# EmilioOlivastri/IPC

Measured on AMD Instinct MI355X. Metric: candidate-pairs/s (consistency matrix + set-max), higher is better.
Workload: dtype f64; 1 GPU; C2: INTEL-like SE2 synthetic (V=1228, 256 true loops) + 1000 injected outliers; N=1256 candidates, 789396 cells (i<=j), 531545 solved on rank 0, s=10, fast 6.251/50, slow 11.345/100; parallelism=1 GPU

## Files before the change

### include/ipc_amd.h

```cpp
#ifndef IPC_AMD_H
#define IPC_AMD_H

#include <stddef.h>
#include <stdint.h>

#ifdef __cplusplus
extern "C" {
#endif

typedef struct ipc_engine ipc_engine_t;

typedef enum {
    IPC_OK = 0,
    IPC_ERR_ARG = -1,
    IPC_ERR_HIP = -2,
    IPC_ERR_STATE = -3,
    IPC_ERR_LIMIT = -4
} ipc_status;

typedef struct {
    double fast_reject_th;
    int    fast_reject_iter_base;
    double slow_reject_th;
    int    slow_reject_iter_base;
    double s_factor;
} ipc_params_t;

typedef struct {
    int    i, j;
    int    lo, hi;
    double max_chi2;
    double chi2_total;
    int    iterations;
    int    tries;
    int    flags;
    int    evals;
} ipc_cell_info_t;

const char* ipc_last_error(void);

int ipc_create(int dim, int n_vertices, const double* odom_meas, const double* odom_info,
               const ipc_params_t* params, int device, ipc_engine_t** out);

int ipc_destroy(ipc_engine_t* h);

int ipc_set_candidates(ipc_engine_t* h, int n, const int* ids, const double* meas,
                       const double* info);

int ipc_append_candidate(ipc_engine_t* h, const int* ids, const double* meas, const double* info, int* index_out);

int ipc_append_odometry(ipc_engine_t* h, int n_edges, const double* meas, const double* info);
int ipc_reserve_vertices(ipc_engine_t* h, int capacity);
int ipc_vertex_count(ipc_engine_t* h, int* n_vertices);

int ipc_candidate_order(ipc_engine_t* h, int* order_out);

int ipc_initial_poses(ipc_engine_t* h, double* poses_out);


int ipc_rows_per_rank(int n, int world);

int ipc_row_assignment(int n, const int* ids, int world, int policy, int* slot_out);

int ipc_solve_rows(ipc_engine_t* h, int rank, int world, uint64_t* d_upper, void* stream);

typedef struct {
    int cells;
    int long_cells;
    int failed_cells;
    int capped_cells;
    int nan_cells;
    int damped_cells;
    int literal_cells;
} ipc_solve_report_t;
int ipc_solve_report(ipc_engine_t* h, ipc_solve_report_t* out);

int ipc_assemble_matrix(ipc_engine_t* h, const uint64_t* d_gathered, int world,
                        uint64_t* d_bits, void* stream);

int ipc_set_max(ipc_engine_t* h, const uint64_t* d_bits, uint8_t* d_accepted, void* stream);

int ipc_run(ipc_engine_t* h, uint64_t* bits_out, uint8_t* accepted_out);

int ipc_run_set_only(ipc_engine_t* h, uint8_t* accepted_out, int* solved_cells_out);

int ipc_run_sharded(ipc_engine_t** engines, int n_engines, uint64_t* bits_out, uint8_t* accepted_out);

typedef struct {
    int covered_before, covered_after;
    int cells;
    int long_cells, literal_cells, damped_cells;
    int set_max_resumed;
    int grew;
} ipc_online_report_t;
int ipc_run_online(ipc_engine_t* h, uint64_t* bits_out, uint8_t* accepted_out, ipc_online_report_t* report);
int ipc_online_covered(ipc_engine_t* h, int* m);
int ipc_online_reset(ipc_engine_t* h);
int ipc_reserve_candidates(ipc_engine_t* h, int capacity);

int ipc_cell_count(ipc_engine_t* h, int* n_cells);
int ipc_cell_info(ipc_engine_t* h, ipc_cell_info_t* out, int capacity);

int ipc_solver_time_ms(ipc_engine_t* h, double* ms, int* launches);

int ipc_synchronize(ipc_engine_t* h);


typedef struct {
    int    lo, hi;
    int    n_cluster_loops;
    int    iterations, tries, flags;
    double max_chi2;
    double chi2_total;
    double chi2_initial;
} ipc_check_info_t;

int ipc_incremental_reset(ipc_engine_t* h);

int ipc_incremental_prepare(ipc_engine_t* h);

int ipc_agreement_check(ipc_engine_t* h, int k, int* agrees, ipc_check_info_t* info);

typedef struct {
    long host_solver_fallbacks, lost_launches, relaunches, literal_band_solves;
} ipc_incremental_counters_t;
int ipc_incremental_counters(ipc_engine_t* h, ipc_incremental_counters_t* out);

int ipc_consensus_size(ipc_engine_t* h, int* n);
int ipc_consensus_set(ipc_engine_t* h, int* out);

int ipc_remove_from_consensus(ipc_engine_t* h, int k, int* removed);
int ipc_add_to_consensus(ipc_engine_t* h, int k);

int ipc_current_poses(ipc_engine_t* h, double* poses_out);

int ipc_incremental_set_state(ipc_engine_t* h, const double* poses, const int* cns, int n_cns, int resume_position);

int ipc_final_optimize(ipc_engine_t* h, const uint8_t* accepted, int iterations, double* poses_out,
                       ipc_check_info_t* info);

int ipc_debug_dense_solve(int n, const double* system, int mode, int workgroups, double* x_out, int* info_out);

int ipc_debug_band_solve(int nb, int m, int W, const double* system, int workgroups, double* x_out, int* info_out);
int ipc_debug_absorbed_edges(int klo, int khi, int n, const int* lo, const int* hi, int sweep, int* members_out, int* n_members_out,
                             int* lo_out, int* hi_out);
int ipc_debug_band_plan(int d, int nl, const int* a, const int* b, int min_n, int* use_out, int* nlb_out, int* bwb_out,
                        int* order_out);

#ifdef __cplusplus
}
#endif
#endif
```

### ipc_amd/capi.py

```python
import ctypes as C
import os

import numpy as np



def export_recommended_environment():
    os.environ.setdefault("GPU_MAX_HW_QUEUES", "24")


_HERE = os.path.dirname(os.path.abspath(__file__))
LIB_PATH = os.environ.get("IPC_AMD_LIB") or os.path.join(_HERE, "libipc_amd.so")

SYMBOLS = [
    "ipc_last_error", "ipc_create", "ipc_destroy", "ipc_set_candidates", "ipc_candidate_order",
    "ipc_initial_poses", "ipc_rows_per_rank", "ipc_solve_rows", "ipc_assemble_matrix", "ipc_set_max",
    "ipc_run", "ipc_cell_count", "ipc_cell_info", "ipc_solve_report", "ipc_solver_time_ms", "ipc_synchronize",
    "ipc_incremental_reset", "ipc_incremental_prepare", "ipc_agreement_check", "ipc_consensus_size", "ipc_consensus_set",
    "ipc_remove_from_consensus", "ipc_add_to_consensus", "ipc_current_poses", "ipc_final_optimize",
    "ipc_debug_dense_solve", "ipc_debug_band_solve", "ipc_debug_band_plan", "ipc_debug_absorbed_edges", "ipc_append_candidate", "ipc_incremental_set_state", "ipc_incremental_counters", "ipc_row_assignment", "ipc_run_sharded", "ipc_run_set_only",
    "ipc_append_odometry", "ipc_reserve_vertices", "ipc_vertex_count",
    "ipc_run_online", "ipc_online_covered", "ipc_online_reset", "ipc_reserve_candidates",
]


class Params(C.Structure):
    _fields_ = [("fast_reject_th", C.c_double), ("fast_reject_iter_base", C.c_int),
                ("slow_reject_th", C.c_double), ("slow_reject_iter_base", C.c_int),
                ("s_factor", C.c_double)]


class CellInfo(C.Structure):
    _fields_ = [("i", C.c_int), ("j", C.c_int), ("lo", C.c_int), ("hi", C.c_int),
                ("max_chi2", C.c_double), ("chi2_total", C.c_double),
                ("iterations", C.c_int), ("tries", C.c_int), ("flags", C.c_int), ("evals", C.c_int)]


class CheckInfo(C.Structure):
    _fields_ = [("lo", C.c_int), ("hi", C.c_int), ("n_cluster_loops", C.c_int), ("iterations", C.c_int),
                ("tries", C.c_int), ("flags", C.c_int), ("max_chi2", C.c_double), ("chi2_total", C.c_double),
                ("chi2_initial", C.c_double)]


class IncrementalCounters(C.Structure):
    _fields_ = [("host_solver_fallbacks", C.c_long), ("lost_launches", C.c_long), ("relaunches", C.c_long),
                ("literal_band_solves", C.c_long)]


class SolveReport(C.Structure):
    _fields_ = [("cells", C.c_int), ("long_cells", C.c_int), ("failed_cells", C.c_int), ("capped_cells", C.c_int),
                ("nan_cells", C.c_int), ("damped_cells", C.c_int), ("literal_cells", C.c_int)]


class OnlineReport(C.Structure):
    _fields_ = [("covered_before", C.c_int), ("covered_after", C.c_int), ("cells", C.c_int), ("long_cells", C.c_int),
                ("literal_cells", C.c_int), ("damped_cells", C.c_int), ("set_max_resumed", C.c_int), ("grew", C.c_int)]


CELL_DTYPE = np.dtype([("i", "<i4"), ("j", "<i4"), ("lo", "<i4"), ("hi", "<i4"), ("max_chi2", "<f8"),
                       ("chi2_total", "<f8"), ("iterations", "<i4"), ("tries", "<i4"), ("flags", "<i4"),
                       ("evals", "<i4")])

_lib = None


class IpcError(RuntimeError):
    pass


def load():
    global _lib
    if _lib is not None:
        return _lib
    if not os.path.exists(LIB_PATH):
        raise IpcError("libipc_amd.so is not built (%s); run `python -c 'import __graft_entry__ as g; "
                       "g.build()'` -- there is no CPU fallback" % LIB_PATH)
    try:
        import torch
    except ImportError:
        pass
    lib = C.CDLL(LIB_PATH)
    lib.ipc_last_error.restype = C.c_char_p
    vp, ip, dp = C.c_void_p, C.c_int, C.c_double
    lib.ipc_create.argtypes = [ip, ip, vp, vp, C.POINTER(Params), ip, C.POINTER(vp)]
    lib.ipc_destroy.argtypes = [vp]
    lib.ipc_set_candidates.argtypes = [vp, ip, vp, vp, vp]
    lib.ipc_append_candidate.argtypes = [vp, vp, vp, vp, C.POINTER(ip)]
    lib.ipc_append_odometry.argtypes = [vp, ip, vp, vp]
    lib.ipc_reserve_vertices.argtypes = [vp, ip]
    lib.ipc_vertex_count.argtypes = [vp, C.POINTER(ip)]
    lib.ipc_candidate_order.argtypes = [vp, vp]
    lib.ipc_initial_poses.argtypes = [vp, vp]
    lib.ipc_rows_per_rank.argtypes = [ip, ip]
    lib.ipc_row_assignment.argtypes = [ip, vp, ip, ip, vp]
    lib.ipc_solve_rows.argtypes = [vp, ip, ip, vp, vp]
    lib.ipc_assemble_matrix.argtypes = [vp, vp, ip, vp, vp]
    lib.ipc_set_max.argtypes = [vp, vp, vp, vp]
    lib.ipc_run.argtypes = [vp, vp, vp]
    lib.ipc_run_online.argtypes = [vp, vp, vp, C.POINTER(OnlineReport)]
    lib.ipc_online_covered.argtypes = [vp, C.POINTER(ip)]
    lib.ipc_online_reset.argtypes = [vp]
    lib.ipc_reserve_candidates.argtypes = [vp, ip]
    lib.ipc_run_sharded.argtypes = [C.POINTER(vp), ip, vp, vp]
    lib.ipc_run_set_only.argtypes = [vp, vp, C.POINTER(ip)]
    lib.ipc_cell_count.argtypes = [vp, C.POINTER(ip)]
    lib.ipc_cell_info.argtypes = [vp, vp, ip]
    lib.ipc_solve_report.argtypes = [vp, C.POINTER(SolveReport)]
    lib.ipc_solver_time_ms.argtypes = [vp, C.POINTER(dp), C.POINTER(ip)]
    lib.ipc_synchronize.argtypes = [vp]
    lib.ipc_incremental_reset.argtypes = [vp]
    lib.ipc_incremental_prepare.argtypes = [vp]
    lib.ipc_agreement_check.argtypes = [vp, ip, C.POINTER(ip), C.POINTER(CheckInfo)]
    lib.ipc_consensus_size.argtypes = [vp, C.POINTER(ip)]
    lib.ipc_consensus_set.argtypes = [vp, vp]
    lib.ipc_remove_from_consensus.argtypes = [vp, ip, C.POINTER(ip)]
    lib.ipc_add_to_consensus.argtypes = [vp, ip]
    lib.ipc_current_poses.argtypes = [vp, vp]
    lib.ipc_incremental_set_state.argtypes = [vp, vp, vp, ip, ip]
    lib.ipc_incremental_counters.argtypes = [vp, C.POINTER(IncrementalCounters)]
    lib.ipc_final_optimize.argtypes = [vp, vp, ip, vp, C.POINTER(CheckInfo)]
    lib.ipc_debug_dense_solve.argtypes = [ip, vp, ip, ip, vp, C.POINTER(ip)]
    lib.ipc_debug_band_solve.argtypes = [ip, ip, ip, vp, ip, vp, C.POINTER(ip)]
    lib.ipc_debug_absorbed_edges.argtypes = [ip, ip, ip, vp, vp, ip, vp, C.POINTER(ip), C.POINTER(ip), C.POINTER(ip)]
    lib.ipc_debug_band_plan.argtypes = [ip, ip, vp, vp, ip, C.POINTER(ip), C.POINTER(ip), C.POINTER(ip), vp]
    assert C.sizeof(CellInfo) == CELL_DTYPE.itemsize
    _lib = lib
    return lib


def check(rc):
    if rc != 0:
        raise IpcError("ipc_amd error %d: %s" % (rc, load().ipc_last_error().decode()))
```

### ipc_amd/csrc/cell_kernels.hpp

```cpp
#pragma once
#include <hip/hip_runtime.h>

#include "se2_cell.hpp"
#include "se3_cell.hpp"

namespace ipc {

struct CellOut {
    double* max_chi2;
    double* chi2_total;
    int4* meta;
};

struct Variant { int W, M; };
static const Variant kVariants[] = {
    {1, 1}, {2, 1}, {3, 1}, {4, 1}, {5, 1}, {6, 1}, {7, 1}, {8, 1}, {10, 1}, {12, 1}, {14, 1}, {16, 1},
    {4, 2}, {5, 2}, {6, 2}, {7, 2}, {8, 2}, {10, 2}, {12, 2}, {16, 2},
    {5, 3}, {6, 3}, {7, 3}, {8, 3},
    {4, 4}, {6, 4}, {8, 4}, {16, 4}, {16, 8}, {16, 16},
    {2, 3}, {2, 4}, {2, 5}, {2, 6},
    {3, 4}, {3, 5}, {3, 6}, {4, 3}, {4, 5},
};
constexpr int kNumVariants = sizeof(kVariants) / sizeof(kVariants[0]);
static const Variant kVariants3[] = { {1, 1}, {2, 1}, {4, 1}, {8, 1}, {16, 1}, {16, 2}, {16, 4},
                                      {4, 2}, {4, 4}, {8, 2}, {8, 4}, {4, 8}, {8, 5},
                                      {1, 2}, {2, 2}, {1, 4}, {2, 4}, {1, 3}, {2, 3} };
constexpr int kNumVariants3 = sizeof(kVariants3) / sizeof(kVariants3[0]);

hipError_t launch_se2_block(int nl, int variant, int n, hipStream_t st, const Se2View& P, const int2* cells,
                            SolveParams prm, CellOut out);
hipError_t launch_se3_block(int nl, int variant, int n, hipStream_t st, const Se3View& P, const int2* cells,
                            SolveParams prm, CellOut out);

struct LdsVariant { int W, M; };
static const LdsVariant kLdsVariants3[] = { {1, 1}, {1, 2}, {1, 3}, {1, 4}, {1, 6}, {1, 8},
                                            {4, 2}, {4, 3}, {4, 4}, {4, 5}, {4, 6}, {4, 7}, {4, 8}, {4, 9}, {4, 10} };
constexpr int kNumLdsVariants3 = sizeof(kLdsVariants3) / sizeof(kLdsVariants3[0]);
constexpr int kLdsVariantBase3 = 400;
#define IPC_SE3_LDS_DECL(WW, MM)                                                                                \
    hipError_t launch_se3_lds_##WW##_##MM(int nl, int n, hipStream_t st, const Se3View& P, const int2* cells,   \
                                          SolveParams prm, CellOut out, unsigned* counter, int n_cu);
IPC_SE3_LDS_DECL(1, 1) IPC_SE3_LDS_DECL(1, 2) IPC_SE3_LDS_DECL(1, 3) IPC_SE3_LDS_DECL(1, 4) IPC_SE3_LDS_DECL(1, 6)
IPC_SE3_LDS_DECL(1, 8) IPC_SE3_LDS_DECL(4, 2) IPC_SE3_LDS_DECL(4, 3) IPC_SE3_LDS_DECL(4, 4) IPC_SE3_LDS_DECL(4, 5)
IPC_SE3_LDS_DECL(4, 6) IPC_SE3_LDS_DECL(4, 7) IPC_SE3_LDS_DECL(4, 8) IPC_SE3_LDS_DECL(4, 9) IPC_SE3_LDS_DECL(4, 10)
#undef IPC_SE3_LDS_DECL

static const int kWaveM[] = {1, 3, 5, 7, 9, 11, 13};
constexpr int kNumWaveM = sizeof(kWaveM) / sizeof(kWaveM[0]);
constexpr int kWaveVariantBase = 100;

hipError_t launch_se2_wave(int nl, int M, int n, hipStream_t st, const Se2View& P, const int2* cells,
                           SolveParams prm, CellOut out, unsigned* counter, int n_cu);

static const int kPairM[] = {5, 7, 9, 11};
constexpr int kNumPairM = sizeof(kPairM) / sizeof(kPairM[0]);
constexpr int kPairVariantBase = 200;
hipError_t launch_se2_pair(int nl, int M, int n, hipStream_t st, const Se2View& P, const int2* cells,
                           SolveParams prm, CellOut out, unsigned* counter, int n_cu);

static const int kQuadM[] = {7, 9, 11, 13};
constexpr int kNumQuadM = sizeof(kQuadM) / sizeof(kQuadM[0]);
constexpr int kQuadVariantBase = 300;
hipError_t launch_se2_quad(int nl, int M, int n, hipStream_t st, const Se2View& P, const int2* cells,
                           SolveParams prm, CellOut out, unsigned* counter, int n_cu);

}
```

### ipc_amd/csrc/engine.hip

```cpp
#include <hip/hip_runtime.h>

#include <algorithm>
#include <cstdarg>
#include <cstdlib>
#include <utility>
#include <cstdio>
#include <cstring>
#include <numeric>
#include <map>
#include <mutex>
#include <string>
#include <chrono>
#include <thread>
#include <vector>

#include "../../include/ipc_amd.h"
#include "cell_kernels.hpp"
#include "cluster_se2.hpp"
#include "cluster_se3.hpp"
#include "cluster_persist.hpp"

using namespace ipc;

static thread_local std::string g_err;
// ... 334 lines not shown
        }
        if (vr) bits[(size_t)ir * words + w] = mine;
    }
}

__global__ __launch_bounds__(256) void k_assemble_delta(int N, int M, int stride, const int* lo, const int* hi,
                                                        const unsigned long long* upper, unsigned long long* bits)
{
    const int lane = threadIdx.x & 63, wave = threadIdx.x >> 6;
    const int w = blockIdx.x;
    auto U = [&](int a, int c) -> unsigned {
        const unsigned long long word = upper[(size_t)a * stride + (c >> 6)];
        return (unsigned)((word >> (c & 63)) & 1ull);
    };
    const int w0 = M >> 6, w1 = (N - 1) >> 6;
    const bool neww = w >= w0;
    const unsigned long long keep = (w == w0 && (M & 63)) ? (1ull << (M & 63)) - 1ull : 0ull;
    const int j = w * 64 + lane;
    const bool vj = j < N;
    const int loj = vj ? lo[j] : 0, hij = vj ? hi[j] : 0;
    const unsigned long long Dword = __ballot(vj && U(j, j));
    for (int rb = (neww ? 0 : w0) + blockIdx.y * 4 + wave; rb <= w1; rb += gridDim.y * 4) {
        const int ir = rb * 64 + lane;
        const bool vr = ir < N;
        const int lor = vr ? lo[ir] : 0, hir = vr ? hi[ir] : 0;
        const unsigned long long dmask = __ballot(vr && U(ir, ir));
        const int nrows = min(64, N - rb * 64);
        unsigned long long mine = 0ull;
        for (int r = 0; r < nrows; ++r) {
            const int i = rb * 64 + r;
            if (i < M && !neww) continue;
            const int loi = __builtin_amdgcn_readlane(lor, r), hii = __builtin_amdgcn_readlane(hir, r);
            unsigned long long word = ((dmask >> r) & 1ull) ? Dword : 0ull;
            const bool ov = vj && j != i && (min(hii, hij) - max(loi, loj) > 0);
            const unsigned long long ovmask = __ballot(ov);
            if (ovmask) {
                const bool bit = ov && U(min(i, j), max(i, j));
                word = (word & ~ovmask) | __ballot(bit);
            }
            if (lane == r) mine = word;
        }
        if (vr) {
            unsigned long long* dst = bits + (size_t)ir * stride + w;
            if (ir >= M) *dst = mine;
            else if (neww) *dst = keep ? ((*dst & keep) | (mine & ~keep)) : mine;
        }
    }
}

__global__ __launch_bounds__(1024) void k_set_max(int N, int words, int stride, const int* order,
                                                  const unsigned long long* bits, unsigned char* accepted, int* live,
                                                  int first = 0, unsigned long long* mask = nullptr, int* nlive_io = nullptr)
{
    constexpr int CPW = 4, RC = 16 * CPW;
    extern __shared__ unsigned long long acc[];
    __shared__ int okflag[RC];
    __shared__ unsigned long long conf[RC];
    __shared__ int kk[RC];
    __shared__ int wcount[16];
    __shared__ int nlive_s;
    const int tid = threadIdx.x, wave = tid >> 6, lane = tid & 63;
    for (int w = tid; w < words; w += blockDim.x) acc[w] = first ? mask[w] : 0ull;
    if (first) { for (int q = first + tid; q < N; q += blockDim.x) accepted[order[q]] = 0; }
    else { for (int k = tid; k < N; k += blockDim.x) accepted[k] = 0; }
    if (tid == 0) nlive_s = first ? *nlive_io : 0;
    __syncthreads();
    const int nlive0 = nlive_s;
    for (int base = first; base < N; base += 1024) {
        const int pos = base + tid;
        const int k = pos < N ? order[pos] : -1;
        const bool keep = k >= 0 && ((bits[(size_t)k * stride + (k >> 6)] >> (k & 63)) & 1ull);
        const unsigned long long m = __ballot(keep);
        if (lane == 0) wcount[wave] = __popcll(m);
        __syncthreads();
        int off = nlive_s;
        for (int v = 0; v < wave; ++v) off += wcount[v];
        if (keep) live[off + __popcll(m & ((1ull << lane) - 1ull))] = k;
        __syncthreads();
        if (tid == 0) { int t = 0; for (int v = 0; v < 16; ++v) t += wcount[v]; nlive_s += t; }
        __syncthreads();
    }
    __threadfence_block();
    const int nlive = nlive_s;
    for (int base = nlive0; base < nlive; base += RC) {
        int k[CPW];
        bool bad[CPW];
#pragma unroll
        for (int c = 0; c < CPW; ++c) {
            const int pos = base + c * 16 + wave;
            k[c] = pos < nlive ? live[pos] : -1;
            bad[c] = false;
        }
        for (int w = lane; w < words; w += 64) {
            const unsigned long long a = acc[w];
#pragma unroll
            for (int c = 0; c < CPW; ++c) {
                const unsigned long long r = k[c] >= 0 ? bits[(size_t)k[c] * stride + w] : ~0ull;
                bad[c] = bad[c] || (r & a) != a;
            }
        }
#pragma unroll
        for (int c = 0; c < CPW; ++c) {
            const bool ok = k[c] >= 0 && __ballot(bad[c]) == 0ull;
            if (lane == 0) { okflag[c * 16 + wave] = ok ? 1 : 0; kk[c * 16 + wave] = k[c]; }
        }
        __syncthreads();
#pragma unroll
        for (int c = 0; c < CPW; ++c) {
            if (k[c] < 0) continue;
            unsigned m = 0;
            if (lane < RC && kk[lane] >= 0) {
                const int o = kk[lane];
                m = (unsigned)((bits[(size_t)k[c] * stride + (o >> 6)] >> (o & 63)) & 1ull);
            }
            const unsigned long long bal = __ballot(m != 0);
            if (lane == 0) conf[c * 16 + wave] = bal;
        }
        __syncthreads();
        if (tid == 0) {
            unsigned long long taken = 0;
            for (int w = 0; w < RC; ++w) {
                if (kk[w] < 0 || !okflag[w]) continue;
                if ((conf[w] & taken) != taken) continue;
                taken |= 1ull << w;
                acc[kk[w] >> 6] |= 1ull << (kk[w] & 63);
                accepted[kk[w]] = 1;
            }
        }
        __syncthreads();
    }
    if (mask) {
        for (int w = tid; w < words; w += blockDim.x) mask[w] = acc[w];
        if (tid == 0) *nlive_io = nlive;
    }
}

struct BinPlan {
    BinCaps caps;
    int variant[kMaxBins];
    int latency_variant[kMaxBins];
    int latency_below[kMaxBins];
};
static const char* kDefaultPolicy = "w1,w3,w5,w7,w9,w11,w13,p7,p9,p11,q7,q9,q11,q13,16x4,16x8,16x16";
static const int kDefaultSideStreams2 = 7, kDefaultSideStreams3 = 7;
static const char* kDefaultPolicy3 = "w1,w2,w3,w4,w6,w8,g3,g4,g5,g6,g7,g8,g9,g10,16x4";
static const char* kBlockPolicy3 = "1x1,1x2,1x3,2x2,2x3,4x2,4x4,8x4,8x5,16x4";
static const char* kDefaultLatencyPolicy3 = "1x1,2x1,4x1,4x2,4x4,8x4,8x5,16x4";
static bool make_plan(BinPlan& bp, int dim, std::string& err)
{
    const char* env = getenv(dim == 2 ? "IPC_SE2_POLICY" : "IPC_SE3_POLICY");
    std::string pol = env && *env ? env : (dim == 2 ? kDefaultPolicy : kDefaultPolicy3);
    if (dim == 3 && pol == "block") pol = kBlockPolicy3;
    const Variant* table = dim == 2 ? kVariants : kVariants3;
    const int ntable = dim == 2 ? kNumVariants : kNumVariants3;
    std::vector<std::pair<int, int>> items;
    size_t pos = 0;
    while (pos < pol.size()) {
        size_t e = pol.find(',', pos);
        if (e == std::string::npos) e = pol.size();
        int w = 0, m = 0;
        const std::string tok = pol.substr(pos, e - pos);
        int v = -1;
        if (dim == 2 && sscanf(tok.c_str(), "w%d", &m) == 1) {
            w = 1;
            for (int k = 0; k < kNumWaveM; ++k) if (kWaveM[k] == m) v = kWaveVariantBase + m;
        } else if (dim == 2 && sscanf(tok.c_str(), "p%d", &m) == 1) {
            w = 2;
            for (int k = 0; k < kNumPairM; ++k) if (kPairM[k] == m) v = kPairVariantBase + m;
        } else if (dim == 2 && sscanf(tok.c_str(), "q%d", &m) == 1) {
            w = 4;
            for (int k = 0; k < kNumQuadM; ++k) if (kQuadM[k] == m) v = kQuadVariantBase + m;
        } else if (dim == 3 && (sscanf(tok.c_str(), "w%d", &m) == 1 || sscanf(tok.c_str(), "g%d", &m) == 1)) {
            w = tok[0] == 'w' ? 1 : 4;
            for (int k = 0; k < kNumLdsVariants3; ++k)
                if (kLdsVariants3[k].W == w && kLdsVariants3[k].M == m) v = kLdsVariantBase3 + k;
        } else {
            if (sscanf(tok.c_str(), "%dx%d", &w, &m) != 2) { err = "bad IPC_SE2_POLICY token"; return false; }
            for (int k = 0; k < ntable; ++k) if (table[k].W == w && table[k].M == m) v = k;
        }
        if (v < 0) { err = "IPC_SE*_POLICY names a variant that is not compiled: " + tok; return false; }
        items.push_back({64 * w * m, v});
        pos = e + 1;
    }
    std::sort(items.begin(), items.end());
    if (items.empty() || (int)items.size() > kMaxBins) { err = "IPC_SE2_POLICY: 1..32 variants"; return false; }
    bp.caps.n = (int)items.size();
    for (int b = 0; b < kMaxBins; ++b) {
        bp.caps.cap[b] = b < bp.caps.n ? items[b].first : 0;
        bp.variant[b] = b < bp.caps.n ? items[b].second : -1;
        bp.latency_variant[b] = -1;
        bp.latency_below[b] = 0;
    }
    if (dim == 3) {
        const char* lenv = getenv("IPC_SE3_LATENCY_POLICY");
        const std::string lpol = lenv && *lenv ? lenv : kDefaultLatencyPolicy3;
        if (lpol != "none") {
            size_t lp = 0;
            std::vector<std::pair<int, int>> lat;
            while (lp < lpol.size()) {
                size_t e = lpol.find(',', lp);
                if (e == std::string::npos) e = lpol.size();
                int w = 0, m = 0, v = -1;
                if (sscanf(lpol.substr(lp, e - lp).c_str(), "%dx%d", &w, &m) != 2) { err = "bad IPC_SE3_LATENCY_POLICY token"; return false; }
                for (int k = 0; k < ntable; ++k) if (table[k].W == w && table[k].M == m) v = k;
                if (v < 0) { err = "IPC_SE3_LATENCY_POLICY names a variant that is not compiled"; return false; }
                lat.push_back({64 * w * m, v});
                lp = e + 1;
            }
            std::sort(lat.begin(), lat.end());
            for (int b = 0; b < bp.caps.n; ++b) {
                if (bp.variant[b] >= kLdsVariantBase3) continue;
                const int wt = table[bp.variant[b]].W;
                for (const auto& lv : lat) {
                    if (lv.first < bp.caps.cap[b]) continue;
                    if (table[lv.second].W > wt) {
                        bp.latency_variant[b] = lv.second;
                        bp.latency_below[b] = wt <= 4 ? 4 / wt : 1;
                    }
                    break;
                }
            }
        }
    }
    return true;
}

static hipError_t launch_se3_lds(int nl, int idx, int n, hipStream_t st, const Se3View& P, const int2* cells,
                                 SolveParams prm, CellOut out, unsigned* counter, int n_cu)
{
#define IPC_LCASE(i, WW, MM) case i: return launch_se3_lds_##WW##_##MM(nl, n, st, P, cells, prm, out, counter, n_cu);
    switch (idx) {
        IPC_LCASE(0, 1, 1) IPC_LCASE(1, 1, 2) IPC_LCASE(2, 1, 3) IPC_LCASE(3, 1, 4) IPC_LCASE(4, 1, 6) IPC_LCASE(5, 1, 8)
        IPC_LCASE(6, 4, 2) IPC_LCASE(7, 4, 3) IPC_LCASE(8, 4, 4) IPC_LCASE(9, 4, 5) IPC_LCASE(10, 4, 6) IPC_LCASE(11, 4, 7)
        IPC_LCASE(12, 4, 8) IPC_LCASE(13, 4, 9) IPC_LCASE(14, 4, 10)
        default: return hipErrorInvalidValue;
    }
#undef IPC_LCASE
}

struct ipc_engine {
    int dim = 2, V = 0, N = 0, device = 0;
    int vcap = 0;
    double* h_stage = nullptr; double* d_stage = nullptr; size_t stage_cap = 0;
    hipEvent_t ev_stage = nullptr; bool stage_used = false;
    long chain_growths = 0;
    ipc_params_t prm{};
    double term_eps = 1e-13;
    BinPlan plan{};
    hipStream_t own_stream = nullptr;
    double* d_chain = nullptr; int estride = 0;
    double* d_chain_rec = nullptr;
    double2* d_chain_blk = nullptr;
    double* d_pose0 = nullptr;
    double* d_cand = nullptr; int cstride = 0;
    int *d_from = nullptr, *d_to = nullptr, *d_lo = nullptr, *d_hi = nullptr, *d_order = nullptr;
    int* d_live = nullptr;
    int* d_rowperm = nullptr;
    std::vector<int> row_group_off;
    bool order_stale = false;
    std::vector<void*> retired;
    hipEvent_t ev_cand = nullptr; bool cand_event = false;
    std::vector<int> order, h_lo, h_hi;
    std::vector<int> h_cand_ids; std::vector<double> h_cand_meas, h_cand_info;
    unsigned* d_counters = nullptr;
    unsigned* d_offsets = nullptr;
    unsigned* d_wave_ctr = nullptr;
    int n_cu = 256;
    int2* d_cells = nullptr; size_t cells_cap = 0;
    double *d_chi = nullptr, *d_chitot = nullptr; int4* d_meta = nullptr;
    bool plan_cached = false; int plan_rank = -1, plan_world = 0; size_t plan_total = 0;
    int slow_first_iterations = 96;
    std::vector<unsigned> plan_counts, plan_offsets;
    int2* d_lit_cells = nullptr; int* d_lit_idx = nullptr; double *d_lit_chi = nullptr, *d_lit_chitot = nullptr; int4* d_lit_meta = nullptr;
    unsigned* d_slot_off = nullptr;
    int* d_recount = nullptr; int* h_recount = nullptr;
    int last_cells = 0, last_long_cells = 0;
    hipEvent_t ev0 = nullptr, ev1 = nullptr; bool ev_valid = false; int last_launches = 0;
    static constexpr int kMaxSide = 7;
    int n_side = 0;
    bool side_forced = false;
    hipStream_t side[kMaxSide] = {};
    hipEvent_t ev_fork = nullptr, ev_join[kMaxSide] = {}, ev_join_own = nullptr;
    unsigned long long *d_upper = nullptr, *d_bits = nullptr; unsigned char* d_acc = nullptr; size_t run_cap = 0;
    int on_cov = 0, on_ccap = 0, on_wcap = 0, reserved_cands = 0;
    unsigned long long *d_on_upper = nullptr, *d_on_bits = nullptr;
    unsigned long long* d_on_mask = nullptr;
    unsigned char* d_on_acc = nullptr;
    int* d_on_live = nullptr;
    long online_growths = 0;
    std::vector<double> h_odom_meas, h_odom_info;
    std::vector<int> h_from, h_to, cns;
    double* d_chain1 = nullptr;
    double* d_open = nullptr;
    double* d_cur = nullptr;
    ClusterSolver2* cluster = nullptr;
    ClusterSolver3* cluster3 = nullptr;
    bool persist = true;
    bool last_persist = false;
    int* d_slot = nullptr; int slot_world = 0; int row_policy = 1;
    int* d_failed = nullptr; int failed_cap = 0; int last_lm_cells = 0;
    bool lm_retry = true;
    double borderline_band = -1.0;
    int last_literal_cells = 0;
    long lm_fallbacks = 0;
    long persist_timeouts = 0;
    long persist_relaunches = 0;
    bool cns_dups = false;
    PersistSolver<PersistSe2>* persist2 = nullptr;
    PersistSolver<PersistSe3>* persist3 = nullptr;
    unsigned long long* d_prof = nullptr;
    int max_helpers = -1;
    PersistKnobs knobs;
    int literal_band_min_n = 3072;
    struct SpecSlot {
        PersistSolver<PersistSe2>* s2 = nullptr;
        PersistSolver<PersistSe3>* s3 = nullptr;
        hipStream_t st = nullptr;
        hipEvent_t done = nullptr;
        int cand = -1, pos = -1;
        int state = -1;
        int launch_id = 0;
        int busy_wgs = 0;
        int expect = -1;
        std::chrono::steady_clock::time_point t_launch;
        int lo = 0, hi = 0, nclu = 0;
        double th = 0.0;
        double pred_ratio = -1.0;
    };
    struct SpecState {
        double* d_poses = nullptr;
        bool owned = false;
        hipEvent_t ready = nullptr;
        bool has_ready = false;
        std::vector<int> cns;
        int pos = -1;
        int users = 0;
        bool live = false;
        double* d_pred = nullptr; double* h_pred = nullptr; int pred_cap = 0, pred_n = 0;
        hipEvent_t pred_ev = nullptr; bool has_pred = false, pred_ready = false;
    };
    struct SpecResult {
        bool valid = false, agree = false, retry_host = false;
        int state = -1, child = -1;
        int lo = 0, hi = 0, nclu = 0;
        ClusterOut o;
    };
    std::vector<SpecSlot> slots;
    std::vector<SpecState> spec_states;
    std::vector<int> tent;
    std::vector<SpecResult> spec_res;
    int committed_state = -1;
    std::vector<int> porder, ppos;
    std::vector<char> handed;
    int spec_head = -1;
    int spec_window = 4, spec_ahead = 256;
    bool window_forced = false;
    int stream_concurrency = 0;
    int spec_active = 0;
    double accept_rate = 0.5;
    std::vector<char> pred_accept;
    double pred_k = 30.0;
    std::vector<double> pred_last;
    int spec_behind = 1;
    double uncertain_from = 0.0;
    int xcd_cus = 0;
    int spec_hedge = 0;
    int helper_limit_reject = 8;
    double gate_release_ms = 0.0;
    int helper_limit = 39;
    double st_acc_s = 0, st_rej_s = 0; long st_acc_it = 0, st_rej_it = 0, st_acc_n = 0, st_rej_n = 0;
    double st_acc_dev_s = 0, st_rej_dev_s = 0;
    unsigned long long commit_count = 0;
    hipEvent_t ev_commit = nullptr;
    int* h_abort = nullptr;
    int* d_abort = nullptr;
    int next_launch_id = 1;
    long spec_hits = 0, spec_launches = 0, spec_wasted = 0, spec_tentative = 0, spec_promoted = 0;
    double spec_t_launch = 0, spec_t_tent = 0, spec_t_total = 0;
    unsigned long long idle_why[5] = {0, 0, 0, 0, 0};
    hipStream_t pred_stream = nullptr;
    FILE* spec_log = nullptr;
    std::chrono::steady_clock::time_point spec_log_t0;
    long pred_conf[3][2] = {{0, 0}, {0, 0}, {0, 0}};
};

static int spec_quiesce(ipc_engine* h, bool state_changes);
static int spec_reset(ipc_engine* h);
struct DevicePipeline {
    ipc_engine* active = nullptr;
    std::vector<ipc_engine*> engines;
    std::recursive_mutex run_mu;
};
static std::mutex g_pipeline_mu;
static std::map<int, DevicePipeline*> g_device_pipeline;
static DevicePipeline& device_pipeline(int device)
{
    std::lock_guard<std::mutex> lk(g_pipeline_mu);
    DevicePipeline*& p = g_device_pipeline[device];
    if (!p) p = new DevicePipeline();
    return *p;
}
static std::map<int, std::vector<hipStream_t>> g_slot_streams;
static hipError_t pipeline_stream(int device, int q, hipStream_t* out)
{
    std::lock_guard<std::mutex> lk(g_pipeline_mu);
    std::vector<hipStream_t>& pool = g_slot_streams[device];
    while ((int)pool.size() <= q) {
        hipStream_t st = nullptr;
        const hipError_t e = hipStreamCreateWithFlags(&st, hipStreamNonBlocking);
        if (e != hipSuccess) return e;
        pool.push_back(st);
    }
    *out = pool[q];
    return hipSuccess;
}

static hipError_t copy_d2d_now(ipc_engine* h, void* dst, const void* src, size_t bytes)
{
    hipError_t e = hipMemcpyAsync(dst, src, bytes, hipMemcpyDeviceToDevice, h->own_stream);
    return e != hipSuccess ? e : hipStreamSynchronize(h->own_stream);
}
constexpr int kPoseTrail = 16;
static int reset_current(ipc_engine* h)
{
    const size_t n = (h->dim == 2 ? 5 : 12) * (size_t)h->vcap;
    HIPCHK(hipMemcpyAsync(h->d_cur, h->d_open, sizeof(double) * n, hipMemcpyDeviceToDevice, h->own_stream));
    HIPCHK(hipMemsetAsync(h->d_cur + n, 0, sizeof(double) * kPoseTrail, h->own_stream));
    HIPCHK(hipStreamSynchronize(h->own_stream));
    return IPC_OK;
}
extern "C" int ipc_rows_per_rank(int n, int world) { return world > 0 ? (n + world - 1) / world : 0; }

extern "C" int ipc_row_assignment(int n, const int* ids, int world, int policy, int* slot_out)
{
    if (n < 0 || world < 1 || (n > 0 && (!ids || !slot_out))) return fail(IPC_ERR_ARG, "ipc_row_assignment: bad argument");
    const int rpr = ipc_rows_per_rank(n, world);
    if (policy == 0 || world == 1) {
        for (int i = 0; i < n; ++i) slot_out[i] = (i % world) * rpr + i / world;
        return IPC_OK;
    }
    std::vector<int> lo(n), hi(n);
    for (int i = 0; i < n; ++i) { lo[i] = std::min(ids[2 * i], ids[2 * i + 1]); hi[i] = std::max(ids[2 * i], ids[2 * i + 1]); }
    std::vector<long long> cost(n);
    for (int i = 0; i < n; ++i) cost[i] = hi[i] - lo[i];
    {
        std::vector<int> ord(n);
        std::iota(ord.begin(), ord.end(), 0);
        std::sort(ord.begin(), ord.end(), [&](int a, int b) { return lo[a] != lo[b] ? lo[a] < lo[b] : a < b; });
        for (int p = 0; p < n; ++p) {
            const int a = ord[p], loa = lo[a], hia = hi[a];
            for (int q = p + 1; q < n && lo[ord[q]] < hia; ++q) {
                const int b = ord[q];
                if (std::min(hia, hi[b]) - lo[b] > 0) cost[std::min(a, b)] += std::max(hia, hi[b]) - loa;
            }
        }
    }
    std::vector<int> rows(n);
    std::iota(rows.begin(), rows.end(), 0);
    std::stable_sort(rows.begin(), rows.end(), [&](int a, int b) { return cost[a] > cost[b]; });
    std::vector<long long> load(world, 0);
    std::vector<int> used(world, 0);
    for (int i : rows) {
        int best = -1;
        for (int r = 0; r < world; ++r)
            if (used[r] < rpr && (best < 0 || load[r] < load[best])) best = r;
        slot_out[i] = best * rpr + used[best];
        ++used[best];
        load[best] += cost[i];
    }
    return IPC_OK;
}

extern "C" int ipc_create(int dim, int n_vertices, const double* odom_meas, const double* odom_info,
                          const ipc_params_t* params, int device, ipc_engine_t** out)
{
    if (!out) return fail(IPC_ERR_ARG, "ipc_create: out is NULL");
    *out = nullptr;
    if (dim != 2 && dim != 3) return fail(IPC_ERR_ARG, "ipc_create: dim must be 2 (SE2) or 3 (SE3), got %d", dim);
    if (n_vertices < 2 || !odom_meas || !odom_info || !params)
        return fail(IPC_ERR_ARG, "ipc_create: need >= 2 vertices and non-NULL arrays");
    if (!(params->s_factor > 0)) return fail(IPC_ERR_ARG, "ipc_create: s_factor must be > 0");
    int ndev = 0;
    HIPCHK(hipGetDeviceCount(&ndev));
    if (device < 0 || device >= ndev) return fail(IPC_ERR_ARG, "ipc_create: device %d of %d", device, ndev);
    HIPCHK(hipSetDevice(device));
    ipc_engine* h = new ipc_engine();
    h->dim = dim; h->V = h->vcap = n_vertices; h->prm = *params; h->device = device;
    {
        std::string perr;
        if (!make_plan(h->plan, dim, perr)) { delete h; return fail(IPC_ERR_ARG, "%s", perr.c_str()); }
    }
    if (const char* te = getenv("IPC_TERMINATE_EPS")) {
        if (*te) {
            char* end = nullptr;
            h->term_eps = strtod(te, &end);
            while (end && (*end == ' ' || *end == '\t')) ++end;
            if (end == te || (end && *end)) { delete h; return fail(IPC_ERR_ARG, "IPC_TERMINATE_EPS: '%s' is not a number", te); }
        }
        if (!(h->term_eps >= 0) || h->term_eps > 1e-6) { delete h; return fail(IPC_ERR_ARG, "IPC_TERMINATE_EPS must be in [0, 1e-6]"); }
    }
    if (const char* pp = getenv("IPC_PERSIST_PROF")) {
        if (*pp && strcmp(pp, "0")) {
            if (hipMalloc(&h->d_prof, sizeof(unsigned long long) * kProfN) != hipSuccess) h->d_prof = nullptr;
            else hipMemset(h->d_prof, 0, sizeof(unsigned long long) * kProfN);
            hipStreamSynchronize(nullptr);
        }
    }
    if (const char* mh = getenv("IPC_PERSIST_HELPERS")) { if (*mh) h->max_helpers = atoi(mh); }
    if (const char* lm = getenv("IPC_LM_RETRY")) { if (*lm) h->lm_retry = atoi(lm) != 0; }
    h->knobs = PersistKnobs::from_env();
    if (const char* e = getenv("IPC_LITERAL_BAND_MIN_N")) { if (*e) h->literal_band_min_n = atoi(e); }
    if (const char* bb = getenv("IPC_BORDERLINE_BAND")) {
        if (*bb) {
            char* end = nullptr;
            h->borderline_band = strtod(bb, &end);
            if (end == bb || *end || !(h->borderline_band >= 0) || h->borderline_band > 0.5) {
                delete h;
                return fail(IPC_ERR_ARG, "IPC_BORDERLINE_BAND must be a number in [0, 0.5]");
            }
        }
    }
    if (const char* sf = getenv("IPC_SLOW_FIRST")) { if (*sf) h->slow_first_iterations = std::max(0, atoi(sf)); }
    if (const char* rb = getenv("IPC_ROW_BALANCE")) {
        if (!strcmp(rb, "cyclic")) h->row_policy = 0;
        else if (*rb && strcmp(rb, "cost")) { delete h; return fail(IPC_ERR_ARG, "IPC_ROW_BALANCE must be 'cost' or 'cyclic'"); }
    }
    {
        const char* q = getenv("GPU_MAX_HW_QUEUES");
        const int nq = q ? atoi(q) : 4;
        h->spec_window = nq >= 24 ? 16 : (nq >= 13 ? 10 : (nq >= 9 ? 8 : 4));
    }
    if (const char* sw = getenv("IPC_SPEC_WINDOW")) { if (*sw) { h->spec_window = std::max(1, std::min(32, atoi(sw))); h->window_forced = true; } }
    if (const char* sa = getenv("IPC_SPEC_AHEAD")) { if (*sa) h->spec_ahead = std::max(1, std::min(1024, atoi(sa))); }
    if (const char* pk = getenv("IPC_SPEC_PREDICT")) { if (*pk) h->pred_k = std::max(0.0, atof(pk)); }
    if (const char* hr = getenv("IPC_PERSIST_HELPERS_REJECT")) { if (*hr) h->helper_limit_reject = std::max(0, atoi(hr)); }
    if (const char* sb = getenv("IPC_SPEC_BEHIND")) { if (*sb) h->spec_behind = std::max(0, std::min(64, atoi(sb))); }
    if (const char* lg = getenv("IPC_SPEC_LOG")) { if (*lg) { h->spec_log = fopen(lg, "w"); h->spec_log_t0 = std::chrono::steady_clock::now(); } }
    if (const char* un = getenv("IPC_SPEC_UNCERTAIN")) { if (*un) h->uncertain_from = std::max(0.0, atof(un)); }
    if (const char* xc = getenv("IPC_SPEC_XCD_CUS")) { if (*xc) h->xcd_cus = std::max(0, atoi(xc)); }
    if (const char* hg = getenv("IPC_SPEC_HEDGE")) { if (*hg) h->spec_hedge = std::max(-1, std::min(8, atoi(hg))); }
    if (const char* gr = getenv("IPC_SPEC_GATE_MS")) { if (*gr) h->gate_release_ms = std::max(0.0, atof(gr)); }
    if (const char* cm = getenv("IPC_CLUSTER_MODE")) {
        if (!strcmp(cm, "host")) h->persist = false;
        else if (*cm && strcmp(cm, "persist")) { delete h; return fail(IPC_ERR_ARG, "IPC_CLUSTER_MODE must be 'persist' or 'host'"); }
    }
    const int E = n_vertices - 1;
    const int ms = dim == 2 ? 3 : 7, is = dim == 2 ? 6 : 21, nf = dim == 2 ? (int)F_NFIELDS : (int)G_NFIELDS;
    const int ps = dim == 2 ? 3 : 12;
    h->estride = (E + 63) & ~63;
    HIPCHK(hipStreamCreateWithFlags(&h->own_stream, hipStreamNonBlocking));
    HIPCHK(hipEventCreate(&h->ev0));
    HIPCHK(hipEventCreate(&h->ev1));
    {
        const char* env = getenv("IPC_SIDE_STREAMS");
        h->n_side = env && *env ? atoi(env) : (h->dim == 2 ? kDefaultSideStreams2 : kDefaultSideStreams3);
        h->side_forced = env && *env;
        if (h->n_side < 0) h->n_side = 0;
        if (h->n_side > ipc_engine::kMaxSide) h->n_side = ipc_engine::kMaxSide;
        HIPCHK(hipEventCreateWithFlags(&h->ev_fork, hipEventDisableTiming));
        HIPCHK(hipEventCreateWithFlags(&h->ev_join_own, hipEventDisableTiming));
        for (int k = 0; k < h->n_side; ++k) {
            HIPCHK(pipeline_stream(device, k, &h->side[k]));
            HIPCHK(hipEventCreateWithFlags(&h->ev_join[k], hipEventDisableTiming));
        }
    }
    HIPCHK(hipMalloc(&h->d_chain, sizeof(double) * (nf * (size_t)h->estride + 64)));
    HIPCHK(hipMalloc(&h->d_pose0, sizeof(double) * ps * (size_t)n_vertices));
    HIPCHK(hipMalloc(&h->d_counters, sizeof(unsigned) * 2 * (kMaxBins + 1) * kPlanSub));
    HIPCHK(hipMalloc(&h->d_offsets, sizeof(unsigned) * 2 * (kMaxBins + 1) * kPlanSub));
    HIPCHK(hipMalloc(&h->d_wave_ctr, sizeof(unsigned) * 2 * (kMaxBins + 1)));
    {
        hipDeviceProp_t prop;
        HIPCHK(hipGetDeviceProperties(&prop, device));
        h->n_cu = prop.multiProcessorCount > 0 ? prop.multiProcessorCount : 256;
    }
    double *d_m = nullptr, *d_i = nullptr;
    HIPCHK(hipMalloc(&d_m, sizeof(double) * ms * E));
    HIPCHK(hipMalloc(&d_i, sizeof(double) * is * E));
    HIPCHK(hipMemcpy(d_m, odom_meas, sizeof(double) * ms * E, hipMemcpyHostToDevice));
    HIPCHK(hipMemcpy(d_i, odom_info, sizeof(double) * is * E, hipMemcpyHostToDevice));
    HIPCHK(hipStreamSynchronize(nullptr));
    HIPCHK(hipMemsetAsync(h->d_chain, 0, sizeof(double) * (nf * (size_t)h->estride + 64), h->own_stream));
    if (dim == 2) {
        hipLaunchKernelGGL(k_se2_prep, dim3((E + 255) / 256), dim3(256), 0, h->own_stream, E, d_m, d_i,
                           params->s_factor, h->d_chain, h->estride);
        hipLaunchKernelGGL(k_se2_propagate, dim3(1), dim3(64), 0, h->own_stream, n_vertices, h->d_chain, h->estride,
                           h->d_pose0, h->vcap);
        HIPCHK(hipMalloc(&h->d_chain_rec, sizeof(double) * (size_t)F_NFIELDS * (h->estride + 64)));
        HIPCHK(hipMemsetAsync(h->d_chain_rec, 0, sizeof(double) * (size_t)F_NFIELDS * (h->estride + 64), h->own_stream));
        hipLaunchKernelGGL(k_records, dim3((E + 255) / 256), dim3(256), 0, h->own_stream, E, (int)F_NFIELDS, h->d_chain,
                           h->estride, h->d_chain_rec);
    } else {
        hipLaunchKernelGGL(k_se3_prep, dim3((E + 63) / 64), dim3(64), 0, h->own_stream, E, d_m, d_i,
                           params->s_factor, h->d_chain, h->estride);
        hipLaunchKernelGGL(k_se3_propagate, dim3(1), dim3(64), 0, h->own_stream, n_vertices, h->d_chain, h->estride,
                           h->d_pose0, h->vcap);
        HIPCHK(hipMalloc(&h->d_chain_rec, sizeof(double) * (size_t)G_NFIELDS * (h->estride + 64)));
        HIPCHK(hipMemsetAsync(h->d_chain_rec, 0, sizeof(double) * (size_t)G_NFIELDS * (h->estride + 64), h->own_stream));
        hipLaunchKernelGGL(k_records, dim3((E + 255) / 256), dim3(256), 0, h->own_stream, E, (int)G_NFIELDS, h->d_chain,
                           h->estride, h->d_chain_rec);
        const size_t nblk = (size_t)h->estride / 64 + 2;
        HIPCHK(hipMalloc(&h->d_chain_blk, sizeof(double2) * nblk * kSe3BlkPairs * 64));
        HIPCHK(hipMemsetAsync(h->d_chain_blk, 0, sizeof(double2) * nblk * kSe3BlkPairs * 64, h->own_stream));
        hipLaunchKernelGGL(k_se3_blocks, dim3((E + 255) / 256), dim3(256), 0, h->own_stream, E, h->d_chain, h->estride,
                           h->d_chain_blk);
    }
    HIPCHK(hipGetLastError());
    HIPCHK(hipStreamSynchronize(h->own_stream));
    HIPCHK(hipFree(d_m));
    HIPCHK(hipFree(d_i));
    h->h_odom_meas.assign(odom_meas, odom_meas + (size_t)ms * E);
    h->h_odom_info.assign(odom_info, odom_info + (size_t)is * E);
    *out = h;
    return IPC_OK;
}

static void free_candidates(ipc_engine* h)
{
    hipFree(h->d_cand); hipFree(h->d_from); hipFree(h->d_to); hipFree(h->d_lo); hipFree(h->d_hi); hipFree(h->d_order); hipFree(h->d_live);
    hipFree(h->d_rowperm); h->d_rowperm = nullptr;
    hipFree(h->d_slot); h->d_slot = nullptr; h->slot_world = 0;
    for (void* q : h->retired) hipFree(q);
    h->retired.clear();
    h->d_cand = nullptr; h->d_from = h->d_to = h->d_lo = h->d_hi = h->d_order = h->d_live = nullptr;
    h->N = 0; h->cstride = 0; h->order_stale = false; h->cand_event = false;
    h->on_cov = 0;
}

static int alloc_candidates(ipc_engine* h, int cap)
{
    const int nf = h->dim == 2 ? (int)F_NFIELDS : (int)G_NFIELDS;
    HIPCHK(hipMalloc(&h->d_cand, sizeof(double) * nf * (size_t)cap));
    HIPCHK(hipMalloc(&h->d_from, sizeof(int) * cap));
    HIPCHK(hipMalloc(&h->d_to, sizeof(int) * cap));
    HIPCHK(hipMalloc(&h->d_lo, sizeof(int) * cap));
    HIPCHK(hipMalloc(&h->d_hi, sizeof(int) * cap));
    HIPCHK(hipMalloc(&h->d_order, sizeof(int) * cap));
    HIPCHK(hipMalloc(&h->d_live, sizeof(int) * cap));
    HIPCHK(hipMalloc(&h->d_rowperm, sizeof(int) * cap));
    HIPCHK(hipMemsetAsync(h->d_cand, 0, sizeof(double) * nf * (size_t)cap, h->own_stream));
    h->cstride = cap;
    return IPC_OK;
}

static int grow_candidates(ipc_engine* h, int need)
{
    const int nf = h->dim == 2 ? (int)F_NFIELDS : (int)G_NFIELDS;
    int cap = std::max(std::max(64, h->cstride), h->reserved_cands);
    while (cap < need) cap *= 2;
    double* o_cand = h->d_cand; const int o_stride = h->cstride;
    int *o_from = h->d_from, *o_to = h->d_to, *o_lo = h->d_lo, *o_hi = h->d_hi, *o_order = h->d_order, *o_live = h->d_live, *o_perm = h->d_rowperm;
    if (int rc = alloc_candidates(h, cap)) return rc;
    if (h->N > 0) {
        HIPCHK(hipMemcpy2DAsync(h->d_cand, sizeof(double) * cap, o_cand, sizeof(double) * o_stride, sizeof(double) * h->N, nf,
                                hipMemcpyDeviceToDevice, h->own_stream));
        HIPCHK(hipMemcpyAsync(h->d_from, o_from, sizeof(int) * h->N, hipMemcpyDeviceToDevice, h->own_stream));
        HIPCHK(hipMemcpyAsync(h->d_to, o_to, sizeof(int) * h->N, hipMemcpyDeviceToDevice, h->own_stream));
        HIPCHK(hipMemcpyAsync(h->d_lo, o_lo, sizeof(int) * h->N, hipMemcpyDeviceToDevice, h->own_stream));
        HIPCHK(hipMemcpyAsync(h->d_hi, o_hi, sizeof(int) * h->N, hipMemcpyDeviceToDevice, h->own_stream));
        if (!h->ev_cand) HIPCHK(hipEventCreateWithFlags(&h->ev_cand, hipEventDisableTiming));
        HIPCHK(hipEventRecord(h->ev_cand, h->own_stream));
        h->cand_event = true;
        h->slot_world = 0;
        h->plan_cached = false;
    }
    for (void* q : {(void*)o_cand, (void*)o_from, (void*)o_to, (void*)o_lo, (void*)o_hi, (void*)o_order, (void*)o_live, (void*)o_perm})
        if (q) h->retired.push_back(q);
    h->order_stale = true;
    return IPC_OK;
}

extern "C" int ipc_destroy(ipc_engine_t* h)
{
    if (!h) return IPC_OK;
    hipSetDevice(h->device);
    DevicePipeline& dp = device_pipeline(h->device);
    std::lock_guard<std::recursive_mutex> run_lk(dp.run_mu);
    spec_quiesce(h, true);
    {
        std::lock_guard<std::mutex> lk(g_pipeline_mu);
        if (dp.active == h) dp.active = nullptr;
        dp.engines.erase(std::remove(dp.engines.begin(), dp.engines.end(), h), dp.engines.end());
    }
    free_candidates(h);
    hipFree(h->d_chain); hipFree(h->d_chain_rec); hipFree(h->d_chain_blk); hipFree(h->d_pose0); hipFree(h->d_counters); hipFree(h->d_offsets); hipFree(h->d_wave_ctr);
    hipFree(h->d_cells); hipFree(h->d_chi); hipFree(h->d_chitot); hipFree(h->d_meta);
    hipFree(h->d_upper); hipFree(h->d_bits); hipFree(h->d_acc); hipFree(h->d_failed);
    hipFree(h->d_on_upper); hipFree(h->d_on_bits); hipFree(h->d_on_mask); hipFree(h->d_on_acc); hipFree(h->d_on_live);
    hipFree(h->d_lit_cells); hipFree(h->d_lit_idx); hipFree(h->d_lit_chi); hipFree(h->d_lit_chitot); hipFree(h->d_lit_meta);
    hipFree(h->d_slot_off); hipFree(h->d_recount); if (h->h_recount) hipHostFree(h->h_recount);
    if (h->h_stage) hipHostFree(h->h_stage);
    if (h->ev_stage) hipEventDestroy(h->ev_stage);
    hipFree(h->d_chain1); if (h->d_open != h->d_pose0) hipFree(h->d_open); hipFree(h->d_cur);
    delete h->cluster;
    delete h->cluster3;
    if (h->d_prof) {
        unsigned long long p[kProfN] = {};
        hipDeviceSynchronize();
        hipMemcpy(p, h->d_prof, sizeof(p), hipMemcpyDeviceToHost);
        static const char* names[kProfN] = {"total", "pre", "handoff", "assemble", "factor", "factor_work", "factor_wait", "backsolve",
                                            "post", "trial", "rest", "iterations", "steps", "help_dt", "help_solve", "help_update", "help_wait",
                                            "look_load", "look_solve", "look_fill", "look_potrf", "look_publish", "bs_dots", "bs_prefetch", "bs_sync", "bs_triangle",
                                            "start_skew", "start_skew_of_launches_over_1_ms", "band_launches", "tile_block", "tile_select", "tile_trsm", "tile_store"};
        fprintf(stderr, "{\"persist_profile_us\": {");
        for (int k = 0; k < kProfN; ++k)
            fprintf(stderr, "%s\"%s\": %.1f", k ? ", " : "", names[k], (k == kProfIterations || k == kProfSteps || k == kProfStartLaunches) ? (double)p[k] : p[k] * 0.01);
        fprintf(stderr, "}}\n");
        hipFree(h->d_prof);
    }
    for (auto& sl : h->slots) {
        if (sl.st) hipStreamSynchronize(sl.st);
        delete sl.s2; delete sl.s3;
        if (sl.done) hipEventDestroy(sl.done);
    }
    for (auto& stt : h->spec_states) {
        if (stt.owned) hipFree(stt.d_poses);
        if (stt.ready) hipEventDestroy(stt.ready);
        if (stt.h_pred) hipHostFree(stt.h_pred);
        if (stt.pred_ev) hipEventDestroy(stt.pred_ev);
    }
    if (h->d_prof || getenv("IPC_SPEC_STATS"))
        fprintf(stderr, "{\"speculation\": {\"window\": %d, \"slots_in_use\": %d, \"streams_abreast\": %d, \"persist_timeouts\": %ld, \"ahead\": %d, \"launches\": %ld, \"results_used\": %ld, \"discarded\": %ld, "
                        "\"tentative_states\": %ld, \"promoted\": %ld, \"host_s_in_checks\": %.3f, \"host_s_launching\": %.3f, "
                        "\"host_s_tentative\": %.3f, "
                        "\"accept_solves\": %ld, \"accept_us_per_iteration\": %.1f, \"accept_ms_per_solve\": %.2f, "
                        "\"reject_solves\": %ld, \"reject_us_per_iteration\": %.1f, \"reject_ms_per_solve\": %.2f, "
                        "\"accept_ms_per_solve_on_the_device\": %.2f, \"reject_ms_per_solve_on_the_device\": %.2f, "
                        "\"empty_slot_share\": {\"behind_an_expected_accept\": %.3f, \"no_candidate_within_the_look_ahead\": %.3f, \"cu_budget\": %.3f, \"cluster_too_large\": %.3f}, "
                        "\"kept_results_by_expectation\": {\"expected_accept\": {\"accepted\": %ld, \"rejected\": %ld}, \"expected_reject\": {\"accepted\": %ld, \"rejected\": %ld}, \"none\": {\"accepted\": %ld, \"rejected\": %ld}}}}\n",
                h->spec_window, h->spec_active, h->stream_concurrency, h->persist_timeouts, h->spec_ahead, h->spec_launches, h->spec_hits, h->spec_wasted, h->spec_tentative, h->spec_promoted,
                h->spec_t_total, h->spec_t_launch, h->spec_t_tent,
                h->st_acc_n, 1e6 * h->st_acc_s / std::max(1L, h->st_acc_it), 1e3 * h->st_acc_s / std::max(1L, h->st_acc_n),
                h->st_rej_n, 1e6 * h->st_rej_s / std::max(1L, h->st_rej_it), 1e3 * h->st_rej_s / std::max(1L, h->st_rej_n),
                1e3 * h->st_acc_dev_s / std::max(1L, h->st_acc_n), 1e3 * h->st_rej_dev_s / std::max(1L, h->st_rej_n),
                (double)h->idle_why[0] / std::max(1ull, h->idle_why[4]), (double)h->idle_why[1] / std::max(1ull, h->idle_why[4]),
                (double)h->idle_why[2] / std::max(1ull, h->idle_why[4]), (double)h->idle_why[3] / std::max(1ull, h->idle_why[4]),
                h->pred_conf[2][1], h->pred_conf[2][0], h->pred_conf[1][1], h->pred_conf[1][0], h->pred_conf[0][1], h->pred_conf[0][0]);
    if (h->spec_log) fclose(h->spec_log);
    if (h->ev_commit) hipEventDestroy(h->ev_commit);
    if (h->h_abort) hipHostFree(h->h_abort);
    delete h->persist2;
    delete h->persist3;
    if (h->ev0) hipEventDestroy(h->ev0);
    if (h->ev1) hipEventDestroy(h->ev1);
    if (h->ev_fork) hipEventDestroy(h->ev_fork);
    if (h->ev_join_own) hipEventDestroy(h->ev_join_own);
    for (int k = 0; k < h->n_side; ++k) {
        if (h->ev_join[k]) hipEventDestroy(h->ev_join[k]);
    }
    if (h->own_stream) hipStreamDestroy(h->own_stream);
    delete h;
    return IPC_OK;
}


static int upload_candidates(ipc_engine* h, int n, const int* ids, const double* meas, const double* info)
{
    for (int k = 0; k < n; ++k) {
        const int f = ids[2 * k], t = ids[2 * k + 1];
        if (f < 0 || t < 0 || f >= h->V || t >= h->V)
            return fail(IPC_ERR_ARG, "candidate %d joins vertex %d-%d outside 0..%d", k, f, t, h->V - 1);
        if (std::abs(f - t) < 2)
            return fail(IPC_ERR_ARG, "candidate %d joins adjacent vertices %d-%d (an odometry edge, "
                        "reference src/utils.cpp:184)", k, f, t);
    }
    HIPCHK(hipSetDevice(h->device));
    if (int rc = spec_quiesce(h, true)) return rc;
    free_candidates(h);
    h->last_cells = 0;
    h->plan_cached = false;
    h->ev_valid = false;
    h->cns.clear(); h->cns_dups = false;
    if (h->d_cur && h->d_open) { if (int rc = reset_current(h)) return rc; }
    const int ms = h->dim == 2 ? 3 : 7, is = h->dim == 2 ? 6 : 21;
    h->h_cand_ids.assign(ids, ids + 2 * (size_t)n);
    h->h_cand_meas.assign(meas, meas + (size_t)ms * n);
    h->h_cand_info.assign(info, info + (size_t)is * n);
    h->h_from.resize(n); h->h_to.resize(n); h->h_lo.resize(n); h->h_hi.resize(n);
    for (int k = 0; k < n; ++k) {
        h->h_from[k] = ids[2 * k]; h->h_to[k] = ids[2 * k + 1];
        h->h_lo[k] = std::min(h->h_from[k], h->h_to[k]); h->h_hi[k] = std::max(h->h_from[k], h->h_to[k]);
    }
    h->order.resize(n);
    std::iota(h->order.begin(), h->order.end(), 0);
    std::stable_sort(h->order.begin(), h->order.end(), [&](int a, int b) { return h->h_hi[a] < h->h_hi[b]; });
    h->porder = h->order;
    h->handed.assign(n, 0);
    h->ppos.assign(n, 0);
    for (int q = 0; q < n; ++q) h->ppos[h->porder[q]] = q;
    if (n == 0) return IPC_OK;
    if (int rc = alloc_candidates(h, std::max((n + 63) & ~63, h->reserved_cands))) return rc;
    h->N = n;
    HIPCHK(hipMemcpy(h->d_from, h->h_from.data(), sizeof(int) * n, hipMemcpyHostToDevice));
    HIPCHK(hipMemcpy(h->d_to, h->h_to.data(), sizeof(int) * n, hipMemcpyHostToDevice));
    HIPCHK(hipMemcpy(h->d_lo, h->h_lo.data(), sizeof(int) * n, hipMemcpyHostToDevice));
    HIPCHK(hipMemcpy(h->d_hi, h->h_hi.data(), sizeof(int) * n, hipMemcpyHostToDevice));
    HIPCHK(hipMemcpy(h->d_order, h->order.data(), sizeof(int) * n, hipMemcpyHostToDevice));
    double *d_m = nullptr, *d_i = nullptr;
    HIPCHK(hipMalloc(&d_m, sizeof(double) * ms * n));
    HIPCHK(hipMalloc(&d_i, sizeof(double) * is * n));
    HIPCHK(hipMemcpy(d_m, meas, sizeof(double) * ms * n, hipMemcpyHostToDevice));
    HIPCHK(hipMemcpy(d_i, info, sizeof(double) * is * n, hipMemcpyHostToDevice));
    HIPCHK(hipStreamSynchronize(nullptr));
    if (h->dim == 2)
        hipLaunchKernelGGL(k_se2_prep, dim3((n + 255) / 256), dim3(256), 0, h->own_stream, n, d_m, d_i, 1.0,
                           h->d_cand, h->cstride);
    else
        hipLaunchKernelGGL(k_se3_prep, dim3((n + 63) / 64), dim3(64), 0, h->own_stream, n, d_m, d_i, 1.0,
                           h->d_cand, h->cstride);
    HIPCHK(hipGetLastError());
    HIPCHK(hipStreamSynchronize(h->own_stream));
    HIPCHK(hipFree(d_m));
// ... 149 lines not shown
            } else {
                IPC_CL_CHK(h->persist2->launch(h->own_stream, chain, h->estride, h->d_cand, h->cstride, src, h->vcap, lo, hi, members,
                                               h->h_from.data(), h->h_to.data(), iters));
                IPC_CL_CHK(h->persist2->wait(o));
                lost = h->persist2->timed_out();
            }
            if (!lost) break;
            ++h->persist_timeouts;
            if (attempt < 2) ++h->persist_relaunches;
        }
        if (lost) o.flags |= 2;
        if (!lost && (!(o.flags & 2) || !h->lm_retry)) return hipSuccess;
        h->last_persist = false;
        ++h->lm_fallbacks;
    }
    if (h->dim == 3)
        return h->cluster3->solve(h->own_stream, chain, h->estride, h->d_cand, h->cstride, src, h->vcap, lo, hi, members,
                                  h->h_from.data(), h->h_to.data(), iters, o, nullptr);
    return h->cluster->solve(h->own_stream, chain, h->estride, h->d_cand, h->cstride, pose_arr(src, h->vcap), lo, hi, members,
                             h->h_from.data(), h->h_to.data(), iters, o, nullptr);
}
static PoseArr cluster_result2(const ipc_engine* h)
{
    if (!h->last_persist) return h->cluster->result();
    return h->persist2->result_in_second() ? h->persist2->dev().Xn : h->persist2->dev().X;
}
static const double* cluster_result3(const ipc_engine* h, int& ld)
{
    if (!h->last_persist) { ld = h->cluster3->ld(); return h->cluster3->result(); }
    ld = h->persist3->ld();
    return h->persist3->result_in_second() ? h->persist3->dev().Xn : h->persist3->dev().X;
}

static int solve_long_cells(ipc_engine* h, hipStream_t st, int nb, const unsigned* counts, const unsigned* offsets)
{
    if (int rc = ensure_incremental(h, "ipc_solve_rows")) return rc;
    HIPCHK(hipStreamSynchronize(st));
    for (int nl = 1; nl <= 2; ++nl) {
        const int s = (nl == 1 ? 0 : (kMaxBins + 1)) + nb;
        const unsigned n = counts[s];
        if (!n) continue;
        std::vector<int2> cells(n);
        HIPCHK(hipMemcpy(cells.data(), h->d_cells + offsets[s], sizeof(int2) * n, hipMemcpyDeviceToHost));
        std::vector<double> chi(n), tot(n);
        std::vector<int4> meta(n);
        for (unsigned c = 0; c < n; ++c) {
            const int i = cells[c].x, j = cells[c].y;
            const int lo = std::min(h->h_lo[i], h->h_lo[j]), hi = std::max(h->h_hi[i], h->h_hi[j]);
            std::vector<int> members{i};
            if (nl == 2) members.push_back(j);
            int iters = nl == 1 ? h->prm.fast_reject_iter_base : h->prm.slow_reject_iter_base;
            if ((hi - lo) + nl > 100) iters *= 5;
            ClusterOut o;
            HIPCHK(cluster_solve(h, h->d_chain, h->d_open, lo, hi, members, iters, o));
            chi[c] = o.max_chi2; tot[c] = o.chi2_total;
            meta[c] = make_int4(o.iterations, o.tries, o.flags, o.evals);
        }
        HIPCHK(hipStreamSynchronize(h->own_stream));
        HIPCHK(hipMemcpy(h->d_chi + offsets[s], chi.data(), sizeof(double) * n, hipMemcpyHostToDevice));
        HIPCHK(hipMemcpy(h->d_chitot + offsets[s], tot.data(), sizeof(double) * n, hipMemcpyHostToDevice));
        HIPCHK(hipMemcpy(h->d_meta + offsets[s], meta.data(), sizeof(int4) * n, hipMemcpyHostToDevice));
    }
    HIPCHK(hipStreamSynchronize(nullptr));
    return IPC_OK;
}

static int ensure_row_map(ipc_engine* h, int world)
{
    if (h->d_slot && h->slot_world == world) return IPC_OK;
    std::vector<int> slot(h->N);
    if (int rc = ipc_row_assignment(h->N, h->h_cand_ids.data(), world, h->row_policy, slot.data())) return rc;
    if (!h->d_slot) HIPCHK(hipMalloc(&h->d_slot, sizeof(int) * h->N));
    HIPCHK(hipMemcpy(h->d_slot, slot.data(), sizeof(int) * h->N, hipMemcpyHostToDevice));
    const int rpr = ipc_rows_per_rank(h->N, world);
    std::vector<int> perm(h->N);
    std::iota(perm.begin(), perm.end(), 0);
    std::stable_sort(perm.begin(), perm.end(), [&](int a, int b) {
        const int ra = slot[a] / rpr, rb = slot[b] / rpr;
        return ra != rb ? ra < rb : h->h_lo[a] < h->h_lo[b];
    });
    h->row_group_off.assign(world + 1, 0);
    for (int i = 0; i < h->N; ++i) ++h->row_group_off[slot[i] / rpr + 1];
    for (int r = 0; r < world; ++r) h->row_group_off[r + 1] += h->row_group_off[r];
    HIPCHK(hipMemcpy(h->d_rowperm, perm.data(), sizeof(int) * h->N, hipMemcpyHostToDevice));
    HIPCHK(hipStreamSynchronize(nullptr));
    h->slot_world = world;
    return IPC_OK;
}

__device__ __forceinline__ int slot_of_cell(const unsigned* slot_off, int nslots, int c)
{
    int lo = 0, hi = nslots;
    while (hi - lo > 1) { const int mid = (lo + hi) >> 1; if (slot_off[mid] <= (unsigned)c) lo = mid; else hi = mid; }
    return lo;
}
__global__ void k_collect_failed(int ncells, const int4* meta, const double* chi, const int2* cells, double fast_th,
                                 double slow_th, double band, bool want_failed, int cap, int* list, int* recount,
                                 const unsigned* slot_off, int nslots, int2* lit_cells, int* lit_idx, int long_bin)
{
    const int c = blockIdx.x * blockDim.x + threadIdx.x;
    if (c >= ncells) return;
    const bool failed = want_failed && (meta[c].z & 2);
    bool border = false;
    const int2 cc = cells[c];
    if (!failed && band > 0.0) {
        const double th = cc.x == cc.y ? fast_th : slow_th;
        border = fabs(chi[c] - th) <= band * th;
    }
    if (failed) {
        const int q = atomicAdd(recount + nslots, 1);
        if (q < cap) list[q] = c;
    } else if (border) {
        const int sl = slot_of_cell(slot_off, nslots, c);
        if (sl == long_bin || sl == (nslots >> 1) + long_bin) {
            const int q = atomicAdd(recount + nslots, 1);
            if (q < cap) list[q] = c;
            return;
        }
        const int q = atomicAdd(recount + sl, 1);
        lit_cells[slot_off[sl] + q] = cc;
        lit_idx[slot_off[sl] + q] = c;
    }
}
__global__ void k_slow_flags(int ncells, const int4* meta, int threshold, int* normal)
{
    const int c = blockIdx.x * blockDim.x + threadIdx.x;
    if (c <= ncells) normal[c] = (c < ncells && meta[c].x < threshold) ? 1 : 0;
}
__global__ __launch_bounds__(1024) void k_scan_int(int* a, int n)
{
    __shared__ int wsum[16];
    const int tid = threadIdx.x, wave = tid >> 6, lane = tid & 63;
    int carry = 0;
    for (int base = 0; base < n; base += 1024) {
        const int i = base + tid;
        const int v0 = i < n ? a[i] : 0;
        int v = v0;
#pragma unroll
        for (int o = 1; o < 64; o <<= 1) { const int t = __shfl_up(v, o, 64); if (lane >= o) v += t; }
        if (lane == 63) wsum[wave] = v;
        __syncthreads();
        int off = carry, tot = carry;
        for (int w = 0; w < 16; ++w) { if (w < wave) off += wsum[w]; tot += wsum[w]; }
        if (i < n) a[i] = off + v - v0;
        carry = tot;
        __syncthreads();
    }
}
__global__ void k_slow_first_permute(int ncells, const unsigned* slot_off, int nslots, const int* excl_normal, const int2* cells,
                                     const double* chi, const double* chitot, const int4* meta, int2* cells2, double* chi2,
                                     double* chitot2, int4* meta2)
{
    const int c = blockIdx.x * blockDim.x + threadIdx.x;
    if (c >= ncells) return;
    const int sl = slot_of_cell(slot_off, nslots, c);
    const int s0 = (int)slot_off[sl], s1 = (int)slot_off[sl + 1];
    const int n0 = excl_normal[s0], nc = excl_normal[c], n1 = excl_normal[s1];
    const bool normal = excl_normal[c + 1] != nc;
    const int nslow = (s1 - s0) - (n1 - n0);
    const int dst = normal ? s0 + nslow + (nc - n0) : s0 + ((c - s0) - (nc - n0));
    cells2[dst] = cells[c]; chi2[dst] = chi[c]; chitot2[dst] = chitot[c]; meta2[dst] = meta[c];
}

__global__ void k_scatter_literal(int ncells, const unsigned* slot_off, int nslots, const int* recount, const int* lit_idx,
                                  const double* lit_chi, const double* lit_chitot, const int4* lit_meta, double* chi, double* chitot, int4* meta)
{
    const int t = blockIdx.x * blockDim.x + threadIdx.x;
    if (t >= ncells) return;
    const int sl = slot_of_cell(slot_off, nslots, t);
    if ((int)(t - slot_off[sl]) >= recount[sl]) return;
    const int c = lit_idx[t];
    chi[c] = lit_chi[t]; chitot[c] = lit_chitot[t]; meta[c] = lit_meta[t];
}
static int resolve_failed_cells(ipc_engine* h, int n)
{
    h->last_lm_cells = 0;
    if (n == 0) return IPC_OK;
    n = std::min(n, h->failed_cap);
    if (int rc = ensure_incremental(h, "ipc_solve_rows")) return rc;
    std::vector<int> idx(n);
    HIPCHK(hipMemcpy(idx.data(), h->d_failed, sizeof(int) * n, hipMemcpyDeviceToHost));
    std::sort(idx.begin(), idx.end());
    for (int q = 0; q < n; ++q) {
        int2 cell;
        HIPCHK(hipMemcpy(&cell, h->d_cells + idx[q], sizeof(int2), hipMemcpyDeviceToHost));
        const int i = cell.x, j = cell.y, nl = i == j ? 1 : 2;
        const int lo = std::min(h->h_lo[i], h->h_lo[j]), hi = std::max(h->h_hi[i], h->h_hi[j]);
        std::vector<int> members{i};
        if (nl == 2) members.push_back(j);
        int iters = nl == 1 ? h->prm.fast_reject_iter_base : h->prm.slow_reject_iter_base;
        if ((hi - lo) + nl > 100) iters *= 5;
        ClusterOut o;
        int4 was;
        HIPCHK(hipMemcpy(&was, h->d_meta + idx[q], sizeof(int4), hipMemcpyDeviceToHost));
        if (was.z & 2) {
            HIPCHK(cluster_solve(h, h->d_chain, h->d_open, lo, hi, members, iters, o, true));
            ++h->last_lm_cells;
        } else {
            const double te = h->term_eps;
            auto set_eps = [&](double v) {
                if (h->cluster) h->cluster->term_eps = v;
                if (h->cluster3) h->cluster3->term_eps = v;
                if (h->persist2) h->persist2->term_eps = v;
                if (h->persist3) h->persist3->term_eps = v;
            };
            set_eps(0.0);
            const hipError_t e = cluster_solve(h, h->d_chain, h->d_open, lo, hi, members, iters, o);
            set_eps(te);
            HIPCHK(e);
            ++h->last_literal_cells;
        }
        const int4 meta = make_int4(o.iterations, o.tries, o.flags, o.evals);
        HIPCHK(hipMemcpy(h->d_chi + idx[q], &o.max_chi2, sizeof(double), hipMemcpyHostToDevice));
        HIPCHK(hipMemcpy(h->d_chitot + idx[q], &o.chi2_total, sizeof(double), hipMemcpyHostToDevice));
        HIPCHK(hipMemcpy(h->d_meta + idx[q], &meta, sizeof(int4), hipMemcpyHostToDevice));
    }
    HIPCHK(hipStreamSynchronize(nullptr));
    return IPC_OK;
}

static int solve_rows_impl(ipc_engine* h, int rank, int world, uint64_t* d_upper, void* stream, int phase);

constexpr int kPlanSlots = 2 * (kMaxBins + 1);
struct CellPlan { unsigned counts[kPlanSlots], offsets[kPlanSlots]; size_t total = 0; };

template <class LaunchPass>
static int plan_cells(ipc_engine* h, hipStream_t st, CellPlan& pl, size_t min_cap, LaunchPass&& launch_pass)
{
    constexpr int NS = kPlanSlots;
    unsigned* counts = pl.counts; unsigned* offsets = pl.offsets;
    size_t total = 0;
    h->plan_cached = false;
    HIPCHK(hipMemsetAsync(h->d_counters, 0, sizeof(unsigned) * NS * kPlanSub, st));
    launch_pass((int2*)nullptr, 0);
    HIPCHK(hipGetLastError());
    static thread_local unsigned subcounts[NS * kPlanSub], suboffsets[NS * kPlanSub];
    HIPCHK(hipMemcpyAsync(subcounts, h->d_counters, sizeof subcounts, hipMemcpyDeviceToHost, st));
    HIPCHK(hipStreamSynchronize(st));
    for (int s = 0; s < NS; ++s) {
        counts[s] = 0;
        for (int q = 0; q < kPlanSub; ++q) counts[s] += subcounts[s * kPlanSub + q];
    }
    for (int s = 0; s < NS; ++s) { offsets[s] = (unsigned)total; total += counts[s]; }
    for (int s = 0; s < NS; ++s) {
        unsigned o = offsets[s];
        for (int q = 0; q < kPlanSub; ++q) { suboffsets[s * kPlanSub + q] = o; o += subcounts[s * kPlanSub + q]; }
    }
    if (std::max(total, min_cap) > h->cells_cap) {
        hipFree(h->d_cells); hipFree(h->d_chi); hipFree(h->d_chitot); hipFree(h->d_meta);
        hipFree(h->d_lit_cells); hipFree(h->d_lit_idx); hipFree(h->d_lit_chi); hipFree(h->d_lit_chitot); hipFree(h->d_lit_meta);
        h->d_cells = h->d_lit_cells = nullptr; h->d_chi = h->d_chitot = h->d_lit_chi = h->d_lit_chitot = nullptr;
        h->d_meta = h->d_lit_meta = nullptr; h->d_lit_idx = nullptr;
        h->cells_cap = std::max(total + total / 8 + 1024, min_cap);
        HIPCHK(hipMalloc(&h->d_cells, sizeof(int2) * h->cells_cap));
        HIPCHK(hipMalloc(&h->d_chi, sizeof(double) * h->cells_cap));
        HIPCHK(hipMalloc(&h->d_chitot, sizeof(double) * h->cells_cap));
        HIPCHK(hipMalloc(&h->d_meta, sizeof(int4) * h->cells_cap));
        HIPCHK(hipMalloc(&h->d_lit_cells, sizeof(int2) * h->cells_cap));
        HIPCHK(hipMalloc(&h->d_lit_idx, sizeof(int) * (h->cells_cap + 1)));
        HIPCHK(hipMalloc(&h->d_lit_chi, sizeof(double) * h->cells_cap));
        HIPCHK(hipMalloc(&h->d_lit_chitot, sizeof(double) * h->cells_cap));
        HIPCHK(hipMalloc(&h->d_lit_meta, sizeof(int4) * h->cells_cap));
    }
    if (!h->d_slot_off) {
        HIPCHK(hipMalloc(&h->d_slot_off, sizeof(unsigned) * (NS + 1)));
        HIPCHK(hipMalloc(&h->d_recount, sizeof(int) * (NS + 1)));
        HIPCHK(hipHostMalloc(&h->h_recount, sizeof(int) * (NS + 1)));
    }
    static thread_local unsigned slot_off[NS + 1];
    for (int s = 0; s < NS; ++s) slot_off[s] = offsets[s];
    slot_off[NS] = (unsigned)total;
    HIPCHK(hipMemcpyAsync(h->d_slot_off, slot_off, sizeof slot_off, hipMemcpyHostToDevice, st));
    HIPCHK(hipMemcpyAsync(h->d_offsets, suboffsets, sizeof suboffsets, hipMemcpyHostToDevice, st));
    HIPCHK(hipMemsetAsync(h->d_counters, 0, sizeof(unsigned) * NS * kPlanSub, st));
    launch_pass(h->d_cells, 1);
    HIPCHK(hipGetLastError());
    pl.total = total;
    return IPC_OK;
}
static int solve_planned(ipc_engine* h, hipStream_t st, const CellPlan& pl);

extern "C" int ipc_solve_rows(ipc_engine_t* h, int rank, int world, uint64_t* d_upper, void* stream)
{
    if (!h) return fail(IPC_ERR_ARG, "ipc_solve_rows: NULL handle");
    if (h->N <= 0) return fail(IPC_ERR_STATE, "ipc_solve_rows: no candidates set");
    if (world < 1 || rank < 0 || rank >= world) return fail(IPC_ERR_ARG, "ipc_solve_rows: rank %d of %d", rank, world);
    if (!d_upper) return fail(IPC_ERR_ARG, "ipc_solve_rows: d_upper is NULL");
    return solve_rows_impl(h, rank, world, d_upper, stream, 0);
}

static int solve_planned(ipc_engine* h, hipStream_t st, const CellPlan& pl)
{
    constexpr int NS = kPlanSlots;
    const unsigned* counts = pl.counts; const unsigned* offsets = pl.offsets;
    const size_t total = pl.total;
    const int nb = h->plan.caps.n;
    const unsigned n_long = counts[nb] + counts[(kMaxBins + 1) + nb];
    Se2View P = make_view(h);
    Se3View P3 = make_view3(h);
    const SolveParams sp{h->prm.fast_reject_iter_base, h->prm.slow_reject_iter_base};
    auto launch_slot = [&](int b, int nl, int n, const int2* cells, const CellOut& out, hipStream_t ls, unsigned* ctr) -> hipError_t {
        int var = h->plan.variant[b];
        if (h->plan.latency_variant[b] >= 0 && n < h->plan.latency_below[b] * h->n_cu) var = h->plan.latency_variant[b];
        if (h->dim == 2)
            return var >= kQuadVariantBase   ? launch_se2_quad(nl, var - kQuadVariantBase, n, ls, P, cells, sp, out, ctr, h->n_cu)
                   : var >= kPairVariantBase ? launch_se2_pair(nl, var - kPairVariantBase, n, ls, P, cells, sp, out, ctr, h->n_cu)
                   : var >= kWaveVariantBase ? launch_se2_wave(nl, var - kWaveVariantBase, n, ls, P, cells, sp, out, ctr, h->n_cu)
                                             : launch_se2_block(nl, var, n, ls, P, cells, sp, out);
        if (var >= kLdsVariantBase3) return launch_se3_lds(nl, var - kLdsVariantBase3, n, ls, P3, cells, sp, out, ctr, h->n_cu);
        return launch_se3_block(nl, var, n, ls, P3, cells, sp, out);
    };
    int launches = 0;
    HIPCHK(hipMemsetAsync(h->d_wave_ctr, 0, sizeof(unsigned) * NS, st));
    HIPCHK(hipEventRecord(h->ev0, st));
    const int n_side = h->side_forced || total < 300000 ? h->n_side : std::min(h->n_side, h->dim == 2 ? 2 : 3);
    hipStream_t st0 = n_side ? h->own_stream : st;
    if (n_side) {
        HIPCHK(hipEventRecord(h->ev_fork, st));
        if (st0 != st) HIPCHK(hipStreamWaitEvent(st0, h->ev_fork, 0));
        for (int k = 0; k < n_side; ++k) HIPCHK(hipStreamWaitEvent(h->side[k], h->ev_fork, 0));
    }
    for (int b = nb - 1; b >= 0; --b) {
        for (int nl = 2; nl >= 1; --nl) {
            const int s = (nl == 1 ? 0 : (kMaxBins + 1)) + b;
            if (!counts[s]) continue;
            CellOut out{h->d_chi + offsets[s], h->d_chitot + offsets[s], h->d_meta + offsets[s]};
            const int lane_q = launches % (n_side + 1);
            hipStream_t ls = lane_q == 0 ? st0 : h->side[lane_q - 1];
            const hipError_t e = launch_slot(b, nl, (int)counts[s], h->d_cells + offsets[s], out, ls, h->d_wave_ctr + s);
            if (e != hipSuccess) return fail(IPC_ERR_HIP, "cell kernel launch failed: %s", hipGetErrorString(e));
            ++launches;
        }
    }
    if (st0 != st) {
        HIPCHK(hipEventRecord(h->ev_join_own, st0));
        HIPCHK(hipStreamWaitEvent(st, h->ev_join_own, 0));
    }
    for (int k = 0; k < n_side; ++k) {
        HIPCHK(hipEventRecord(h->ev_join[k], h->side[k]));
        HIPCHK(hipStreamWaitEvent(st, h->ev_join[k], 0));
    }
    if (n_long) {
        if (int rc = solve_long_cells(h, st, nb, counts, offsets)) return rc;
    }
    HIPCHK(hipEventRecord(h->ev1, st));
    h->ev_valid = true;
    h->last_launches = launches;
    h->last_cells = (int)total;
    h->last_long_cells = (int)n_long;
    h->last_lm_cells = h->last_literal_cells = 0;
    const double band = h->term_eps > 0 ? (h->borderline_band >= 0 ? h->borderline_band : 4.0 * std::sqrt(h->term_eps)) : 0.0;
    if (total && (h->lm_retry || band > 0.0)) {
        if ((int)total > h->failed_cap) {
            HIPCHK(hipFree(h->d_failed));
            h->d_failed = nullptr;
            h->failed_cap = std::max(16384, (int)(total + total / 8));
            HIPCHK(hipMalloc(&h->d_failed, sizeof(int) * ((size_t)h->failed_cap + 1)));
        }
        HIPCHK(hipMemsetAsync(h->d_recount, 0, sizeof(int) * (NS + 1), st));
        hipLaunchKernelGGL(k_collect_failed, dim3((unsigned)((total + 255) / 256)), dim3(256), 0, st, (int)total, (const int4*)h->d_meta,
                           (const double*)h->d_chi, (const int2*)h->d_cells, h->prm.fast_reject_th, h->prm.slow_reject_th, band,
                           h->lm_retry, h->failed_cap, h->d_failed, h->d_recount, (const unsigned*)h->d_slot_off, NS, h->d_lit_cells, h->d_lit_idx, nb);
        HIPCHK(hipGetLastError());
        HIPCHK(hipMemcpyAsync(h->h_recount, h->d_recount, sizeof(int) * (NS + 1), hipMemcpyDeviceToHost, st));
        HIPCHK(hipStreamSynchronize(st));
        int n_lit = 0;
        for (int s = 0; s < NS; ++s) n_lit += h->h_recount[s];
        if (n_lit) {
            P.term_eps = 0.0; P3.term_eps = 0.0;
            HIPCHK(hipMemsetAsync(h->d_wave_ctr, 0, sizeof(unsigned) * NS, st));
            for (int b = nb - 1; b >= 0; --b) {
                for (int nl = 2; nl >= 1; --nl) {
                    const int s = (nl == 1 ? 0 : (kMaxBins + 1)) + b;
                    const int n = h->h_recount[s];
                    if (!n) continue;
                    CellOut out{h->d_lit_chi + offsets[s], h->d_lit_chitot + offsets[s], h->d_lit_meta + offsets[s]};
                    const hipError_t e = launch_slot(b, nl, n, h->d_lit_cells + offsets[s], out, st, h->d_wave_ctr + s);
                    if (e != hipSuccess) return fail(IPC_ERR_HIP, "cell kernel launch failed: %s", hipGetErrorString(e));
                }
            }
            hipLaunchKernelGGL(k_scatter_literal, dim3((unsigned)((total + 255) / 256)), dim3(256), 0, st, (int)total,
                               (const unsigned*)h->d_slot_off, NS, (const int*)h->d_recount, (const int*)h->d_lit_idx, (const double*)h->d_lit_chi,
                               (const double*)h->d_lit_chitot, (const int4*)h->d_lit_meta, h->d_chi, h->d_chitot, h->d_meta);
            HIPCHK(hipGetLastError());
            h->last_literal_cells += n_lit;
        }
        if (h->h_recount[NS]) {
            if (int rc = resolve_failed_cells(h, h->h_recount[NS])) return rc;
        }
    }
    return IPC_OK;
}

static int solve_rows_impl(ipc_engine* h, int rank, int world, uint64_t* d_upper, void* stream, int phase)
{
    HIPCHK(hipSetDevice(h->device));
    hipStream_t st = stream ? (hipStream_t)stream : h->own_stream;
    const int N = h->N, words = (N + 63) / 64, rpr = ipc_rows_per_rank(N, world);
    if (int rc = matrix_mode_enter(h, st)) return rc;
    if (int rc = ensure_row_map(h, world)) return rc;
    const BinCaps bc = h->plan.caps;
    constexpr int NS = kPlanSlots;
    if (phase != 2) HIPCHK(hipMemsetAsync(d_upper, 0, sizeof(uint64_t) * (size_t)rpr * words, st));
    CellPlan pl;
    const bool cached = phase == 0 && h->plan_cached && h->plan_rank == rank && h->plan_world == world;
    if (cached) {
        std::copy(h->plan_counts.begin(), h->plan_counts.end(), pl.counts);
        std::copy(h->plan_offsets.begin(), h->plan_offsets.end(), pl.offsets);
        pl.total = h->plan_total;
    } else {
        const int nrows = h->row_group_off[rank + 1] - h->row_group_off[rank];
        const int* rows = h->d_rowperm + h->row_group_off[rank];
        const dim3 pgrid((N + 255) / 256, std::max(1, std::min(nrows, 2048))), pblock(256);
        if (int rc = plan_cells(h, st, pl, 0, [&](int2* cells, int fill) {
                hipLaunchKernelGGL(k_plan, pgrid, pblock, 0, st, N, h->d_lo, h->d_hi, rows, nrows, bc, h->d_counters,
                                   h->d_offsets, cells, fill, phase, (const unsigned long long*)d_upper, words);
            })) return rc;
        if (phase == 0) {
            h->plan_counts.assign(pl.counts, pl.counts + NS);
            h->plan_offsets.assign(pl.offsets, pl.offsets + NS);
            h->plan_total = pl.total; h->plan_rank = rank; h->plan_world = world;
            h->plan_cached = true;
        }
    }
    const size_t total = pl.total;
    if (int rc = solve_planned(h, st, pl)) return rc;
    if (total)
        hipLaunchKernelGGL(k_scatter_bits, dim3((unsigned)((total + 255) / 256)), dim3(256), 0, st, (int)total,
                           h->d_cells, h->d_chi, h->prm.fast_reject_th, h->prm.slow_reject_th, rpr, (const int*)h->d_slot, words,
                           (unsigned long long*)d_upper);
    HIPCHK(hipGetLastError());
    if (total && !cached && phase == 0 && h->slow_first_iterations > 0) {
        const unsigned nblk1 = (unsigned)((total + 1 + 255) / 256), nblk = (unsigned)((total + 255) / 256);
        hipLaunchKernelGGL(k_slow_flags, dim3(nblk1), dim3(256), 0, st, (int)total, (const int4*)h->d_meta, h->slow_first_iterations, h->d_lit_idx);
        hipLaunchKernelGGL(k_scan_int, dim3(1), dim3(1024), 0, st, h->d_lit_idx, (int)total + 1);
        hipLaunchKernelGGL(k_slow_first_permute, dim3(nblk), dim3(256), 0, st, (int)total, (const unsigned*)h->d_slot_off, NS, (const int*)h->d_lit_idx,
                           (const int2*)h->d_cells, (const double*)h->d_chi, (const double*)h->d_chitot, (const int4*)h->d_meta, h->d_lit_cells,
                           h->d_lit_chi, h->d_lit_chitot, h->d_lit_meta);
        HIPCHK(hipGetLastError());
        std::swap(h->d_cells, h->d_lit_cells); std::swap(h->d_chi, h->d_lit_chi);
        std::swap(h->d_chitot, h->d_lit_chitot); std::swap(h->d_meta, h->d_lit_meta);
    }
    return IPC_OK;
}

extern "C" int ipc_assemble_matrix(ipc_engine_t* h, const uint64_t* d_gathered, int world, uint64_t* d_bits,
                                   void* stream)
{
    if (!h || !d_gathered || !d_bits) return fail(IPC_ERR_ARG, "ipc_assemble_matrix: NULL argument");
    if (h->N <= 0) return fail(IPC_ERR_STATE, "ipc_assemble_matrix: no candidates set");
    if (world < 1) return fail(IPC_ERR_ARG, "ipc_assemble_matrix: world %d", world);
    HIPCHK(hipSetDevice(h->device));
    hipStream_t st = stream ? (hipStream_t)stream : h->own_stream;
    const int N = h->N, words = (N + 63) / 64, rpr = ipc_rows_per_rank(N, world);
    if (int rc = matrix_mode_enter(h, st)) return rc;
    if (int rc = ensure_row_map(h, world)) return rc;
    hipLaunchKernelGGL(k_assemble, dim3(words, std::min((N + 255) / 256, 1024)), dim3(256), 0, st, N, words, (const int*)h->d_slot, h->d_lo,
                       h->d_hi, (const unsigned long long*)d_gathered, (unsigned long long*)d_bits);
    HIPCHK(hipGetLastError());
    return IPC_OK;
}

extern "C" int ipc_set_max(ipc_engine_t* h, const uint64_t* d_bits, uint8_t* d_accepted, void* stream)
{
    if (!h || !d_bits || !d_accepted) return fail(IPC_ERR_ARG, "ipc_set_max: NULL argument");
    if (h->N <= 0) return fail(IPC_ERR_STATE, "ipc_set_max: no candidates set");
    HIPCHK(hipSetDevice(h->device));
    hipStream_t st = stream ? (hipStream_t)stream : h->own_stream;
    const int N = h->N, words = (N + 63) / 64;
    const size_t shmem = sizeof(unsigned long long) * words;
    if (shmem > 60 * 1024) return fail(IPC_ERR_LIMIT, "ipc_set_max: N=%d exceeds the LDS-resident mask", N);
    if (int rc = matrix_mode_enter(h, st)) return rc;
    hipLaunchKernelGGL(k_set_max, dim3(1), dim3(1024), shmem, st, N, words, words, (const int*)h->d_order,
                       (const unsigned long long*)d_bits, d_accepted, h->d_live, 0, (unsigned long long*)nullptr, (int*)nullptr);
    HIPCHK(hipGetLastError());
    return IPC_OK;
}

extern "C" int ipc_run(ipc_engine_t* h, uint64_t* bits_out, uint8_t* accepted_out)
{
    if (!h) return fail(IPC_ERR_ARG, "ipc_run: NULL handle");
    if (h->N <= 0) return fail(IPC_ERR_STATE, "ipc_run: no candidates set");
    HIPCHK(hipSetDevice(h->device));
    const int N = h->N, words = (N + 63) / 64;
    const size_t need = (size_t)N * words;
    if (need > h->run_cap) {
        hipFree(h->d_upper); hipFree(h->d_bits); hipFree(h->d_acc);
        h->d_upper = h->d_bits = nullptr; h->d_acc = nullptr;
        HIPCHK(hipMalloc(&h->d_upper, sizeof(uint64_t) * need));
        HIPCHK(hipMalloc(&h->d_bits, sizeof(uint64_t) * need));
        HIPCHK(hipMalloc(&h->d_acc, (size_t)N + 64));
        h->run_cap = need;
    }
    int rc = ipc_solve_rows(h, 0, 1, (uint64_t*)h->d_upper, h->own_stream);
    if (rc) return rc;
    rc = ipc_assemble_matrix(h, (const uint64_t*)h->d_upper, 1, (uint64_t*)h->d_bits, h->own_stream);
    if (rc) return rc;
    rc = ipc_set_max(h, (const uint64_t*)h->d_bits, h->d_acc, h->own_stream);
    if (rc) return rc;
    HIPCHK(hipStreamSynchronize(h->own_stream));
    if (bits_out) HIPCHK(hipMemcpy(bits_out, h->d_bits, sizeof(uint64_t) * need, hipMemcpyDeviceToHost));
    if (accepted_out) HIPCHK(hipMemcpy(accepted_out, h->d_acc, (size_t)N, hipMemcpyDeviceToHost));
    return IPC_OK;
}

static int grow_online(ipc_engine* h, int cap)
{
    const int wcap = cap / 64, M = h->on_cov;
    hipStream_t st = h->own_stream;
    unsigned long long *n_upper = nullptr, *n_bits = nullptr, *n_mask = nullptr;
    unsigned char* n_acc = nullptr; int* n_live = nullptr;
    const size_t mat = sizeof(unsigned long long) * (size_t)cap * wcap;
    size_t mem_free = 0, mem_total = 0;
    HIPCHK(hipMemGetInfo(&mem_free, &mem_total));
    if (2 * mat + 16 * (size_t)cap > mem_free)
        return fail(IPC_ERR_LIMIT, "online matrix for %d candidates needs %zu MB, the device has %zu MB free", cap, (2 * mat) >> 20, mem_free >> 20);
    HIPCHK(hipMalloc(&n_upper, mat));
    HIPCHK(hipMalloc(&n_bits, mat));
    HIPCHK(hipMalloc(&n_mask, sizeof(unsigned long long) * wcap));
    HIPCHK(hipMalloc(&n_acc, (size_t)cap));
    HIPCHK(hipMalloc(&n_live, sizeof(int) * ((size_t)cap + 1)));
    HIPCHK(hipMemsetAsync(n_upper, 0, mat, st));
    HIPCHK(hipMemsetAsync(n_bits, 0, mat, st));
    HIPCHK(hipMemsetAsync(n_mask, 0, sizeof(unsigned long long) * wcap, st));
    HIPCHK(hipMemsetAsync(n_acc, 0, (size_t)cap, st));
    HIPCHK(hipMemsetAsync(n_live, 0, sizeof(int) * ((size_t)cap + 1), st));
    if (M > 0) {
        const size_t opitch = sizeof(unsigned long long) * h->on_wcap, npitch = sizeof(unsigned long long) * wcap;
        HIPCHK(hipMemcpy2DAsync(n_upper, npitch, h->d_on_upper, opitch, opitch, M, hipMemcpyDeviceToDevice, st));
        HIPCHK(hipMemcpy2DAsync(n_bits, npitch, h->d_on_bits, opitch, opitch, M, hipMemcpyDeviceToDevice, st));
        HIPCHK(hipMemcpyAsync(n_mask, h->d_on_mask, opitch, hipMemcpyDeviceToDevice, st));
        HIPCHK(hipMemcpyAsync(n_acc, h->d_on_acc, (size_t)M, hipMemcpyDeviceToDevice, st));
        HIPCHK(hipMemcpyAsync(n_live, h->d_on_live, sizeof(int) * (size_t)M, hipMemcpyDeviceToDevice, st));
        HIPCHK(hipMemcpyAsync(n_live + cap, h->d_on_live + h->on_ccap, sizeof(int), hipMemcpyDeviceToDevice, st));
    }
    for (void* q : {(void*)h->d_on_upper, (void*)h->d_on_bits, (void*)h->d_on_mask, (void*)h->d_on_acc, (void*)h->d_on_live})
        if (q) h->retired.push_back(q);
    h->d_on_upper = n_upper; h->d_on_bits = n_bits; h->d_on_mask = n_mask; h->d_on_acc = n_acc; h->d_on_live = n_live;
    h->on_ccap = cap; h->on_wcap = wcap;
    ++h->online_growths;
    return IPC_OK;
}

extern "C" int ipc_reserve_candidates(ipc_engine_t* h, int capacity)
{
    if (!h) return fail(IPC_ERR_ARG, "ipc_reserve_candidates: NULL handle");
    if (capacity < 0 || capacity > (1 << 24)) return fail(IPC_ERR_ARG, "ipc_reserve_candidates: capacity %d (0 .. 2^24)", capacity);
    HIPCHK(hipSetDevice(h->device));
    const int cap = (capacity + 63) & ~63;
    if (cap > h->reserved_cands) h->reserved_cands = cap;
    if (cap > h->cstride) { if (int rc = grow_candidates(h, cap)) return rc; }
    if (cap > h->on_ccap && sizeof(unsigned long long) * (size_t)(cap / 64) <= 60 * 1024) { if (int rc = grow_online(h, cap)) return rc; }
    return IPC_OK;
}

extern "C" int ipc_online_covered(ipc_engine_t* h, int* m)
{
    if (!h || !m) return fail(IPC_ERR_ARG, "ipc_online_covered: NULL argument");
    *m = h->on_cov;
    return IPC_OK;
}

extern "C" int ipc_online_reset(ipc_engine_t* h)
{
    if (!h) return fail(IPC_ERR_ARG, "ipc_online_reset: NULL handle");
    h->on_cov = 0;
    return IPC_OK;
}

extern "C" int ipc_run_online(ipc_engine_t* h, uint64_t* bits_out, uint8_t* accepted_out, ipc_online_report_t* report)
{
    if (!h) return fail(IPC_ERR_ARG, "ipc_run_online: NULL handle");
    if (h->N <= 0) return fail(IPC_ERR_STATE, "ipc_run_online: no candidates set");
    HIPCHK(hipSetDevice(h->device));
    const int N = h->N, M = h->on_cov, words = (N + 63) / 64;
    if (sizeof(unsigned long long) * (size_t)words > 60 * 1024) return fail(IPC_ERR_LIMIT, "ipc_run_online: N=%d exceeds the LDS-resident mask", N);
    hipStream_t st = h->own_stream;
    if (int rc = matrix_mode_enter(h, st)) return rc;
    ipc_online_report_t rep{};
    rep.covered_before = M; rep.covered_after = N;
    if (N > h->on_ccap) {
        int cap = std::max(64, h->on_ccap);
        while (cap < N) cap *= 2;
        if (int rc = grow_online(h, cap)) return rc;
        rep.grew = 1;
    }
    const int stride = h->on_wcap;
    h->last_cells = 0; h->last_long_cells = 0; h->last_lm_cells = h->last_literal_cells = 0;
    if (M < N) {
        if (M == 0) {
            const size_t mat = sizeof(unsigned long long) * (size_t)h->on_ccap * stride;
            HIPCHK(hipMemsetAsync(h->d_on_upper, 0, mat, st));
            HIPCHK(hipMemsetAsync(h->d_on_bits, 0, mat, st));
            HIPCHK(hipMemsetAsync(h->d_on_mask, 0, sizeof(unsigned long long) * stride, st));
        }
        CellPlan pl;
        const BinCaps bc = h->plan.caps;
        const dim3 pgrid((N + 255) / 256, std::min(N - M, 2048)), pblock(256);
        if (int rc = plan_cells(h, st, pl, (size_t)h->on_ccap, [&](int2* cells, int fill) {
                hipLaunchKernelGGL(k_plan_delta, pgrid, pblock, 0, st, N, M, (const int*)h->d_lo, (const int*)h->d_hi, bc, h->d_counters,
                                   (const unsigned*)h->d_offsets, cells, fill);
            })) return rc;
        const size_t total = pl.total;
        if (int rc = solve_planned(h, st, pl)) return rc;
        if (total)
            hipLaunchKernelGGL(k_scatter_bits_delta, dim3((unsigned)((total + 255) / 256)), dim3(256), 0, st, (int)total, (const int2*)h->d_cells,
                               (const double*)h->d_chi, h->prm.fast_reject_th, h->prm.slow_reject_th, stride, h->d_on_upper);
        const int tiles = ((N - 1) >> 6) + 1;
        hipLaunchKernelGGL(k_assemble_delta, dim3(words, std::min((tiles + 3) / 4, 1024)), dim3(256), 0, st, N, M, stride, (const int*)h->d_lo,
                           (const int*)h->d_hi, (const unsigned long long*)h->d_on_upper, h->d_on_bits);
        bool resume = M > 0;
        for (int q = M; q < N && resume; ++q) resume = h->order[q] >= M;
        hipLaunchKernelGGL(k_set_max, dim3(1), dim3(1024), sizeof(unsigned long long) * words, st, N, words, stride, (const int*)h->d_order,
                           (const unsigned long long*)h->d_on_bits, h->d_on_acc, h->d_on_live, resume ? M : 0, h->d_on_mask,
                           h->d_on_live + h->on_ccap);
        HIPCHK(hipGetLastError());
        h->on_cov = N;
        rep.cells = (int)total;
        rep.long_cells = h->last_long_cells;
        rep.literal_cells = h->last_literal_cells;
        rep.damped_cells = h->last_lm_cells;
        rep.set_max_resumed = resume ? 1 : 0;
    }
    HIPCHK(hipStreamSynchronize(st));
    if (bits_out)
        HIPCHK(hipMemcpy2D(bits_out, sizeof(uint64_t) * words, h->d_on_bits, sizeof(uint64_t) * stride, sizeof(uint64_t) * words, N,
                           hipMemcpyDeviceToHost));
    if (accepted_out) HIPCHK(hipMemcpy(accepted_out, h->d_on_acc, (size_t)N, hipMemcpyDeviceToHost));
    if (report) *report = rep;
    return IPC_OK;
}

extern "C" int ipc_cell_count(ipc_engine_t* h, int* n_cells)
{
    if (!h || !n_cells) return fail(IPC_ERR_ARG, "ipc_cell_count: NULL argument");
    *n_cells = h->last_cells;
    return IPC_OK;
}

extern "C" int ipc_cell_info(ipc_engine_t* h, ipc_cell_info_t* out, int capacity)
{
    if (!h || !out) return fail(IPC_ERR_ARG, "ipc_cell_info: NULL argument");
    HIPCHK(hipSetDevice(h->device));
    HIPCHK(hipDeviceSynchronize());
    const int n = std::min(capacity, h->last_cells);
    if (n <= 0) return IPC_OK;
    std::vector<int2> cells(n);
    std::vector<double> chi(n), tot(n);
    std::vector<int4> meta(n);
    HIPCHK(hipMemcpy(cells.data(), h->d_cells, sizeof(int2) * n, hipMemcpyDeviceToHost));
    HIPCHK(hipMemcpy(chi.data(), h->d_chi, sizeof(double) * n, hipMemcpyDeviceToHost));
    HIPCHK(hipMemcpy(tot.data(), h->d_chitot, sizeof(double) * n, hipMemcpyDeviceToHost));
    HIPCHK(hipMemcpy(meta.data(), h->d_meta, sizeof(int4) * n, hipMemcpyDeviceToHost));
    for (int c = 0; c < n; ++c) {
        ipc_cell_info_t& o = out[c];
        o.i = cells[c].x; o.j = cells[c].y;
        o.lo = std::min(h->h_lo[o.i], h->h_lo[o.j]);
        o.hi = std::max(h->h_hi[o.i], h->h_hi[o.j]);
        o.max_chi2 = chi[c]; o.chi2_total = tot[c];
        o.iterations = meta[c].x; o.tries = meta[c].y; o.flags = meta[c].z; o.evals = meta[c].w;
    }
    return IPC_OK;
}

__global__ void k_report(int n, const int4* meta, const double* chi, unsigned* out)
{
    const int c = blockIdx.x * blockDim.x + threadIdx.x;
    if (c >= n) return;
    const int4 m = meta[c];
    if (m.z & 2) atomicAdd(&out[0], 1u);
    if (!(m.z & 1) && !(m.z & 2)) atomicAdd(&out[1], 1u);
    if (chi[c] != chi[c]) atomicAdd(&out[2], 1u);
}

extern "C" int ipc_solve_report(ipc_engine_t* h, ipc_solve_report_t* out)
{
    if (!h || !out) return fail(IPC_ERR_ARG, "ipc_solve_report: NULL argument");
    HIPCHK(hipSetDevice(h->device));
    HIPCHK(hipDeviceSynchronize());
    memset(out, 0, sizeof *out);
    out->cells = h->last_cells;
    out->long_cells = h->last_long_cells;
    if (h->last_cells <= 0) return IPC_OK;
    unsigned host[3] = {0, 0, 0};
    HIPCHK(hipMemsetAsync(h->d_counters, 0, sizeof(unsigned) * 3, h->own_stream));
    hipLaunchKernelGGL(k_report, dim3((h->last_cells + 255) / 256), dim3(256), 0, h->own_stream, h->last_cells, h->d_meta,
                       h->d_chi, h->d_counters);
    HIPCHK(hipGetLastError());
    HIPCHK(hipMemcpyAsync(host, h->d_counters, sizeof host, hipMemcpyDeviceToHost, h->own_stream));
    HIPCHK(hipStreamSynchronize(h->own_stream));
    out->failed_cells = (int)host[0];
    out->capped_cells = (int)host[1];
    out->nan_cells = (int)host[2];
    out->damped_cells = h->last_lm_cells;
    out->literal_cells = h->last_literal_cells;
    return IPC_OK;
}

extern "C" int ipc_solver_time_ms(ipc_engine_t* h, double* ms, int* launches)
{
    if (!h || !ms) return fail(IPC_ERR_ARG, "ipc_solver_time_ms: NULL argument");
    if (!h->ev_valid) return fail(IPC_ERR_STATE, "ipc_solver_time_ms: no solve recorded");
    HIPCHK(hipSetDevice(h->device));
    HIPCHK(hipEventSynchronize(h->ev1));
    float t = 0;
    HIPCHK(hipEventElapsedTime(&t, h->ev0, h->ev1));
    *ms = t;
    if (launches) *launches = h->last_launches;
    return IPC_OK;
}

#if defined(IPC_PHASE_TIMING)
extern "C" int ipc_dbg_read(ipc_engine_t* h, double* out, int n)
{
    Se2View P = make_view(h);
    hipDeviceSynchronize();
    hipMemcpy(out, P.dbg, sizeof(double) * n, hipMemcpyDeviceToHost);
    return 0;
}
#endif
extern "C" int ipc_synchronize(ipc_engine_t* h)
{
    if (!h) return fail(IPC_ERR_ARG, "ipc_synchronize: NULL handle");
    HIPCHK(hipSetDevice(h->device));
    HIPCHK(hipDeviceSynchronize());
    return IPC_OK;
}

__global__ void k_pose5_init(int V, const double* pose0, int is, double* out, int os, int first = 0)
{
    const int i = first + blockIdx.x * blockDim.x + threadIdx.x;
    if (i >= V) return;
    const double th = pose0[2 * (size_t)is + i];
    double s, c;
    sincos_pi(th, s, c);
    out[i] = pose0[i]; out[(size_t)os + i] = pose0[(size_t)is + i]; out[2 * (size_t)os + i] = th;
    out[3 * (size_t)os + i] = c; out[4 * (size_t)os + i] = s;
}

__global__ void k_se2_propagate_tail(int V, int start, const double* rec, int stride, double* cur)
{
    if (threadIdx.x != 0 || blockIdx.x != 0) return;
    double x = cur[start], y = cur[(size_t)V + start], th = cur[2 * (size_t)V + start];
    double c = cur[3 * (size_t)V + start], s = cur[4 * (size_t)V + start];
    for (int i = start + 1; i < V; ++i) {
        const double tx = rec[(size_t)F_TZX * stride + i - 1], ty = rec[(size_t)F_TZY * stride + i - 1];
        x += c * tx - s * ty;
        y += s * tx + c * ty;
        th = normalize_theta(th + rec[(size_t)F_THZ * stride + i - 1]);
        sincos_pi(th, s, c);
        cur[i] = x; cur[(size_t)V + i] = y; cur[2 * (size_t)V + i] = th;
        cur[3 * (size_t)V + i] = c; cur[4 * (size_t)V + i] = s;
    }
}

__global__ void k_se3_propagate_tail(int V, int start, const double* rec, int stride, double* cur)
{
    if (threadIdx.x != 0 || blockIdx.x != 0) return;
    double R[9], t[3];
    for (int q = 0; q < 9; ++q) R[q] = cur[(size_t)q * V + start];
    for (int q = 0; q < 3; ++q) t[q] = cur[(size_t)(9 + q) * V + start];
    for (int i = start + 1; i < V; ++i) {
        double Rz[9], tz[3], Rn[9], d[3];
        for (int q = 0; q < 9; ++q) Rz[q] = rec[(size_t)(G_RZ + q) * stride + i - 1];
        for (int q = 0; q < 3; ++q) tz[q] = rec[(size_t)(G_TZ + q) * stride + i - 1];
        m3_mul(R, Rz, Rn);
        m3_vec(R, tz, d);
        for (int q = 0; q < 3; ++q) t[q] += d[q];
        for (int q = 0; q < 9; ++q) R[q] = Rn[q];
        for (int q = 0; q < 9; ++q) cur[(size_t)q * V + i] = R[q];
        for (int q = 0; q < 3; ++q) cur[(size_t)(9 + q) * V + i] = t[q];
    }
}

__global__ void k_cand_own_chi2_se2(const double* poses, int V, const double* cand, int cstride, const int* from, const int* to,
                                    int n, double* out)
{
    const int c = blockIdx.x * blockDim.x + threadIdx.x;
    if (c >= n) return;
    const int ia = from[c], ib = to[c];
    const Pose2 a{poses[ia], poses[V + ia], poses[2 * (size_t)V + ia], poses[3 * (size_t)V + ia], poses[4 * (size_t)V + ia]};
    const Pose2 b{poses[ib], poses[V + ib], poses[2 * (size_t)V + ib], poses[3 * (size_t)V + ib], poses[4 * (size_t)V + ib]};
    double e0, e1, e2;
    se2_error(a, b, cand[(size_t)F_TZX * cstride + c], cand[(size_t)F_TZY * cstride + c], cand[(size_t)F_CZ * cstride + c],
              cand[(size_t)F_SZ * cstride + c], cand[(size_t)F_THZ * cstride + c], e0, e1, e2);
    out[c] = gk_sym(cand, cstride, F_OM, c).quad(e0, e1, e2);
}
__global__ void k_cand_own_chi2_se3(const double* poses, int V, const double* cand, int cstride, const int* from, const int* to,
                                    int n, double* out)
{
    const int c = blockIdx.x * blockDim.x + threadIdx.x;
    if (c >= n) return;
    double Rz[9], tz[3], om[21];
    gk3_rz(cand, cstride, c, Rz, tz);
    Edge3 E;
    se3_edge(gk3_pose(poses, V, from[c]), gk3_pose(poses, V, to[c]), Rz, tz, E);
    gk3_sym(cand, cstride, G_OM, c, om);
    out[c] = sym6_quad(om, E.e);
}

__device__ __forceinline__ void se2_tail_D(double xT, double yT, double thT, const double* open, size_t Vs, int hi, double* D)
{
    const double thP = open[2 * Vs + hi];
    const double thD = normalize_theta(thT - thP);
    double sD, cD;
    sincos_pi(thD, sD, cD);
    const double xP = open[hi], yP = open[Vs + hi];
    const double xD = xT - (cD * xP - sD * yP), yD = yT - (sD * xP + cD * yP);
    D[0] = xD; D[1] = yD; D[2] = thD; D[3] = cD; D[4] = sD;
}
__device__ __forceinline__ void se2_tail_apply(const double* D, const double* open, size_t Vs, double* dst, int i)
{
    const double xD = D[0], yD = D[1], thD = D[2], cD = D[3], sD = D[4];
    const double x = open[i], y = open[Vs + i];
    const double th = normalize_theta(thD + open[2 * Vs + i]);
    double sn, cs;
    sincos_pi(th, sn, cs);
    dst[i] = xD + (cD * x - sD * y);
    dst[Vs + i] = yD + (sD * x + cD * y);
    dst[2 * Vs + i] = th;
    dst[3 * Vs + i] = cs;
    dst[4 * Vs + i] = sn;
}
__device__ __forceinline__ void se3_tail_D(const double* T, size_t ldt, const double* open, size_t Vs, int hi, double* D)
{
    double RT[9], tT[3], RP[9], tP[3], d[3];
    double* RD = D;
    for (int q = 0; q < 9; ++q) { RT[q] = T[(size_t)q * ldt]; RP[q] = open[(size_t)q * Vs + hi]; }
    for (int q = 0; q < 3; ++q) { tT[q] = T[(size_t)(9 + q) * ldt]; tP[q] = open[(size_t)(9 + q) * Vs + hi]; }
    for (int r = 0; r < 3; ++r)
        for (int c = 0; c < 3; ++c) RD[3 * r + c] = RT[3 * r] * RP[3 * c] + RT[3 * r + 1] * RP[3 * c + 1] + RT[3 * r + 2] * RP[3 * c + 2];
    m3_vec(RD, tP, d);
    for (int q = 0; q < 3; ++q) D[9 + q] = tT[q] - d[q];
}
__device__ __forceinline__ void se3_tail_apply(const double* D, const double* open, size_t Vs, double* dst, int i)
{
    const double* RD = D;
    const double* tD = D + 9;
    double Ri[9], ti[3], Rn[9], d[3];
    for (int q = 0; q < 9; ++q) Ri[q] = open[(size_t)q * Vs + i];
    for (int q = 0; q < 3; ++q) ti[q] = open[(size_t)(9 + q) * Vs + i];
    m3_mul(RD, Ri, Rn);
    m3_vec(RD, ti, d);
    for (int q = 0; q < 9; ++q) dst[(size_t)q * Vs + i] = Rn[q];
    for (int q = 0; q < 3; ++q) dst[(size_t)(9 + q) * Vs + i] = tD[q] + d[q];
}
template <int NF>
__global__ __launch_bounds__(256) void k_apply_accept(int V, int vs, int lo, int hi, const double* parent, const double* X, int ldx,
                                                      const double* open, double* dst)
{
    const int tid = threadIdx.x;
    for (int q = tid; q < NF * V; q += 256) {
        const int f = q / V, i = q - f * V;
        const size_t a = (size_t)f * vs + i;
        if (i >= lo && i <= hi) dst[a] = X[(size_t)f * ldx + (i - lo)];
        else if (i < lo && dst != parent) dst[a] = parent[a];
    }
    const size_t Vs = (size_t)vs;
    double D[12];
    if (NF == 5) se2_tail_D(X[hi - lo], X[(size_t)ldx + (hi - lo)], X[2 * (size_t)ldx + (hi - lo)], open, Vs, hi, D);
    else se3_tail_D(X + (hi - lo), (size_t)ldx, open, Vs, hi, D);
    if (tid == 0) {
        double* tr = dst + (size_t)NF * Vs;
        for (int q = 0; q < NF; ++q) tr[q] = D[q];
        tr[kPoseTrail - 1] = 1.0;
    }
    for (int i = hi + 1 + tid; i < V; i += 256) {
        if (NF == 5) se2_tail_apply(D, open, Vs, dst, i);
        else se3_tail_apply(D, open, Vs, dst, i);
    }
}
template <int NF>
__global__ void k_state_D(int V, int vs, const double* open, double* cur)
{
    if (threadIdx.x != 0 || blockIdx.x != 0) return;
    const size_t Vs = (size_t)vs;
    double D[12];
    if (NF == 5) se2_tail_D(cur[V - 1], cur[Vs + V - 1], cur[2 * Vs + V - 1], open, Vs, V - 1, D);
    else se3_tail_D(cur + (V - 1), Vs, open, Vs, V - 1, D);
    double* tr = cur + (size_t)NF * Vs;
    for (int q = 0; q < NF; ++q) tr[q] = D[q];
    tr[kPoseTrail - 1] = 1.0;
}

struct ChainPtrs {
    double* chain; int estride;
    double* chain_rec;
    double2* chain_blk;
    double* chain1;
    double* pose0;
    double* open5;
    int vs;
};
struct RawOdometry { double meas[7]; double info[21]; };
template <int DIM>
__device__ __forceinline__ void append_edge_records(const double* m, const double* inf, double scale, const ChainPtrs& C, int k)
{
    constexpr int nf = DIM == 2 ? (int)F_NFIELDS : (int)G_NFIELDS;
    if (DIM == 2) se2_prep_record(m, inf, scale, 1.0, C.chain, C.estride, k);
    else se3_prep_record(m, inf, scale, 1.0, C.chain, C.estride, k);
    for (int f = 0; f < nf; ++f) C.chain_rec[(size_t)k * nf + f] = C.chain[(size_t)f * C.estride + k];
    if (DIM == 3) se3_block_record(C.chain, C.estride, C.chain_blk, k);
    if (C.chain1) {
        if (DIM == 2) se2_prep_record(m, inf, scale, scale, C.chain1, C.estride, k);
        else se3_prep_record(m, inf, scale, scale, C.chain1, C.estride, k);
    }
}
template <int DIM>
__device__ __forceinline__ void append_compose(int V0, int n, const ChainPtrs& C)
{
    const size_t vs = (size_t)C.vs;
    if (DIM == 2) {
        double x = C.pose0[V0 - 1], y = C.pose0[vs + V0 - 1], th = C.pose0[2 * vs + V0 - 1];
        for (int i = V0; i < V0 + n; ++i) {
            se2_compose_step(x, y, th, C.chain, C.estride, i);
            C.pose0[i] = x; C.pose0[vs + i] = y; C.pose0[2 * vs + i] = th;
            if (C.open5) {
                double s, c;
                sincos_pi(th, s, c);
                C.open5[i] = x; C.open5[vs + i] = y; C.open5[2 * vs + i] = th; C.open5[3 * vs + i] = c; C.open5[4 * vs + i] = s;
            }
        }
    } else {
        double R[9], t[3];
        for (int q = 0; q < 9; ++q) R[q] = C.pose0[(size_t)q * vs + V0 - 1];
        for (int q = 0; q < 3; ++q) t[q] = C.pose0[(size_t)(9 + q) * vs + V0 - 1];
        for (int i = V0; i < V0 + n; ++i) {
            se3_compose_step(R, t, C.chain, C.estride, i);
            for (int q = 0; q < 9; ++q) C.pose0[(size_t)q * vs + i] = R[q];
            for (int q = 0; q < 3; ++q) C.pose0[(size_t)(9 + q) * vs + i] = t[q];
        }
    }
}
template <int DIM>
__global__ void k_append_odometry_one(RawOdometry r, int k, double scale, ChainPtrs C)
{
    if (threadIdx.x != 0 || blockIdx.x != 0) return;
    double m[7], inf[21];
    for (int q = 0; q < 7; ++q) m[q] = r.meas[q];
    for (int q = 0; q < 21; ++q) inf[q] = r.info[q];
    append_edge_records<DIM>(m, inf, scale, C, k);
    append_compose<DIM>(k + 1, 1, C);
}
template <int DIM>
__global__ void k_append_odometry_prep(int n, int k0, const double* meas, const double* info, double scale, ChainPtrs C)
{
    const int j = blockIdx.x * blockDim.x + threadIdx.x;
    if (j >= n) return;
    constexpr int ms = DIM == 2 ? 3 : 7, is = DIM == 2 ? 6 : 21;
    double m[7], inf[21];
    for (int q = 0; q < ms; ++q) m[q] = meas[(size_t)ms * j + q];
    for (int q = 0; q < is; ++q) inf[q] = info[(size_t)is * j + q];
    append_edge_records<DIM>(m, inf, scale, C, k0 + j);
}
template <int DIM>
__global__ void k_append_odometry_compose(int V0, int n, ChainPtrs C)
{
    if (threadIdx.x != 0 || blockIdx.x != 0) return;
    append_compose<DIM>(V0, n, C);
}
constexpr int kMaxAppendStates = 12;
struct StateList { double* p[kMaxAppendStates]; };
template <int NF>
__global__ void k_append_state_tail(int V0, int n, const double* open, int vs, StateList L)
{
    const int i = V0 + blockIdx.x * blockDim.x + threadIdx.x;
    if (i >= V0 + n) return;
    const size_t Vs = (size_t)vs;
    double* dst = L.p[blockIdx.y];
    const double* D = dst + (size_t)NF * Vs;
    if (D[kPoseTrail - 1] == 0.0) {
        for (int f = 0; f < NF; ++f) dst[(size_t)f * Vs + i] = open[(size_t)f * Vs + i];
        return;
    }
    if (NF == 5) se2_tail_apply(D, open, Vs, dst, i);
    else se3_tail_apply(D, open, Vs, dst, i);
}

static PoseArr pose_arr(double* base, int V)
{
    return PoseArr{base, base + (size_t)V, base + 2 * (size_t)V, base + 3 * (size_t)V, base + 4 * (size_t)V};
}

static int ensure_incremental(ipc_engine* h, const char* who)
{
    (void)who;
    HIPCHK(hipSetDevice(h->device));
    if (h->dim == 3) {
        if (!h->d_cur) {
            h->d_open = h->d_pose0;
            HIPCHK(hipMalloc(&h->d_cur, sizeof(double) * (12 * (size_t)h->vcap + kPoseTrail)));
            if (int rc = reset_current(h)) return rc;
        }
        if (!h->cluster3) {
            h->cluster3 = new ClusterSolver3(); h->cluster3->term_eps = h->term_eps; h->cluster3->allow_damping = h->lm_retry;
            h->cluster3->literal_band_min_n = h->literal_band_min_n;
        }
        if (!h->persist3) {
// ... 1279 lines not shown
```

### ipc_amd/csrc/se2_group_kernel.hpp

```cpp
#pragma once
#include "cell_kernels.hpp"
#include "se2_wave_cell.hpp"

namespace ipc {

constexpr int kWavesPerGroup = 4;
#ifndef IPC_LDS_BUDGET
#define IPC_LDS_BUDGET (160 * 1024)
#endif
constexpr int kLdsBudget = IPC_LDS_BUDGET;

template <int W, int M, int NL, bool STAGED>
__global__ __launch_bounds__(64 * kWavesPerGroup, 1) void se2_group_kernel(Se2View P, const int2* cells, int ncells,
                                                                           unsigned* counter, SolveParams prm,
                                                                           CellOut out, int wlo, int wlen, int wstride)
{
    extern __shared__ double dyn_lds[];
    constexpr int kPairs = kWavesPerGroup / W;
    constexpr int kScratchDoubles = (sizeof(WaveScratch<NL>) + 7) / 8;
    constexpr int kBoxDoubles = (sizeof(PairBox) + 7) / 8;
    const int wave = threadIdx.x >> 6, lane = threadIdx.x & 63, pair = wave / W, wsub = wave & (W - 1);
    WaveScratch<NL>& sh = *reinterpret_cast<WaveScratch<NL>*>(dyn_lds + pair * kScratchDoubles);
    PairBox* box = reinterpret_cast<PairBox*>(dyn_lds + kPairs * kScratchDoubles + pair * kBoxDoubles);
    double* cst = dyn_lds + kPairs * (kScratchDoubles + kBoxDoubles);
    if (STAGED) {
        for (int f = 0; f < (int)F_SG; ++f)
            for (int i = threadIdx.x; i < wstride; i += 64 * kWavesPerGroup)
                cst[i * (int)F_SG + f] = i < wlen ? P.chain[(size_t)f * P.estride + wlo + i] : 0.0;
    }
    if (lane == 0) box->flag[wsub] = 0;
    __syncthreads();
    int seq = 0;
    for (;;) {
        ++seq;
        unsigned c = 0;
        if (wsub == 0 && lane == 0) {
            c = atomicAdd(counter, 1u);
            mb_store(&box->data[0][seq & 1][0], (double)c);
        }
        wave_sync();
        if (lane == 0) __hip_atomic_store(&box->flag[wsub], seq, __ATOMIC_RELEASE, __HIP_MEMORY_SCOPE_WORKGROUP);
#pragma unroll
        for (int o = 0; o < W; ++o) {
            if (o == wsub) continue;
            while (__hip_atomic_load(&box->flag[o], __ATOMIC_ACQUIRE, __HIP_MEMORY_SCOPE_WORKGROUP) - seq < 0)
                IPC_SPIN_WAIT();
        }
        wave_sync();
        c = (unsigned)mb_load(&box->data[0][seq & 1][0]);
        c = (unsigned)__builtin_amdgcn_readfirstlane((int)c);
        if (c >= (unsigned)ncells) break;
        const int2 cc = cells[c];
        int cand[2] = {cc.x, cc.y};
        int lo = min(P.cand_from[cc.x], P.cand_to[cc.x]), hi = max(P.cand_from[cc.x], P.cand_to[cc.x]);
        if (NL == 2) {
            lo = min(lo, min(P.cand_from[cc.y], P.cand_to[cc.y]));
            hi = max(hi, max(P.cand_from[cc.y], P.cand_to[cc.y]));
        }
        const int L = hi - lo;
        const int base = NL == 1 ? prm.fast_iter : prm.slow_iter;
        const int iterations = (L + NL > 100) ? base * 5 : base;
        CellResult r;
        se2_wave_solve<M, NL, STAGED, W>(P, lo, L, cand, iterations, sh, cst, wlo, wstride, r, box, seq, &seq);
        if (wsub == 0 && lane == 0) {
            out.max_chi2[c] = r.max_chi2;
            out.chi2_total[c] = r.chi2_total;
            out.meta[c] = make_int4(r.iterations, r.tries, r.flags, r.evals);
        }
        wave_sync();
    }
}

template <int W, int M, int NL>
static hipError_t launch_group(int n, hipStream_t st, const Se2View& P, const int2* cells, SolveParams prm, CellOut out,
                              unsigned* counter, int n_cu)
{
    const int E = P.V - 1;
    const int wstride = E + 32;
    constexpr int kPairs = kWavesPerGroup / W;
    const size_t scratch = kPairs * (((sizeof(WaveScratch<NL>) + 7) / 8) + ((sizeof(PairBox) + 7) / 8)) * sizeof(double);
    const size_t staged = scratch + sizeof(double) * (size_t)F_SG * wstride;
    const int groups = std::max(1, std::min(n_cu, (n + kPairs - 1) / kPairs));
    if (staged <= (size_t)kLdsBudget) {
        auto k = se2_group_kernel<W, M, NL, true>;
        hipError_t e = hipFuncSetAttribute(reinterpret_cast<const void*>(k), hipFuncAttributeMaxDynamicSharedMemorySize, (int)staged);
        if (e != hipSuccess) return e;
        hipLaunchKernelGGL(k, dim3(groups), dim3(64 * kWavesPerGroup), staged, st, P, cells, n, counter, prm, out, 0, E, wstride);
    } else {
        auto k = se2_group_kernel<W, M, NL, false>;
        hipLaunchKernelGGL(k, dim3(groups), dim3(64 * kWavesPerGroup), scratch, st, P, cells, n, counter, prm, out, 0, E, wstride);
    }
    return hipGetLastError();
}

}
```

### ipc_amd/csrc/se2_pair.hip

```cpp
#include "se2_group_kernel.hpp"

namespace ipc {
hipError_t launch_se2_pair(int nl, int M, int n, hipStream_t st, const Se2View& P, const int2* cells, SolveParams prm,
                           CellOut out, unsigned* counter, int n_cu)
{
#define IPC_PCASE(MM)                                                                              \
    case MM:                                                                                       \
        return nl == 1 ? launch_group<2, MM, 1>(n, st, P, cells, prm, out, counter, n_cu)          \
                       : launch_group<2, MM, 2>(n, st, P, cells, prm, out, counter, n_cu);
    switch (M) {
#ifdef IPC_PAIR_ONLY_M
        IPC_PCASE(IPC_PAIR_ONLY_M)
#else
        IPC_PCASE(5)
        IPC_PCASE(7)
        IPC_PCASE(9)
        IPC_PCASE(11)
#endif
        default: return hipErrorInvalidValue;
    }
#undef IPC_PCASE
}
}
```

### ipc_amd/csrc/se2_quad.hip

```cpp
#include "se2_group_kernel.hpp"

namespace ipc {
hipError_t launch_se2_quad(int nl, int M, int n, hipStream_t st, const Se2View& P, const int2* cells, SolveParams prm,
                           CellOut out, unsigned* counter, int n_cu)
{
#define IPC_PCASE(MM)                                                                              \
    case MM:                                                                                       \
        return nl == 1 ? launch_group<4, MM, 1>(n, st, P, cells, prm, out, counter, n_cu)          \
                       : launch_group<4, MM, 2>(n, st, P, cells, prm, out, counter, n_cu);
    switch (M) {
        IPC_PCASE(7)
        IPC_PCASE(9)
        IPC_PCASE(11)
        IPC_PCASE(13)
        default: return hipErrorInvalidValue;
    }
#undef IPC_PCASE
}
}
```

### ipc_amd/csrc/se2_wave.hip

```cpp
#include "cell_kernels.hpp"
#include "se2_wave_cell.hpp"

using namespace ipc;

#ifndef IPC_SE2_DENSE_MAXM
#define IPC_SE2_DENSE_MAXM 1
#endif
template <int M>
constexpr int se2_waves() { return M <= IPC_SE2_DENSE_MAXM ? 8 : 4; }

template <int M, int NL, bool STAGED>
__global__ __launch_bounds__((64 * se2_waves<M>()), 1) void se2_wave_kernel(Se2View P, const int2* cells, int ncells,
                                                                          unsigned* counter, SolveParams prm,
                                                                          CellOut out, int wlo, int wlen, int wstride)
{
    extern __shared__ double dyn_lds[];
    constexpr int kWavesPerGroup = se2_waves<M>();
    constexpr int kScratchDoubles = (sizeof(WaveScratch<NL>) + 7) / 8;
    const int wave = threadIdx.x >> 6, lane = threadIdx.x & 63;
    WaveScratch<NL>& sh = *reinterpret_cast<WaveScratch<NL>*>(dyn_lds + wave * kScratchDoubles);
    double* cst = dyn_lds + kWavesPerGroup * kScratchDoubles;
    if (STAGED) {
        for (int f = 0; f < (int)F_SG; ++f)
            for (int i = threadIdx.x; i < wstride; i += 64 * kWavesPerGroup)
                cst[i * (int)F_SG + f] = i < wlen ? P.chain[(size_t)f * P.estride + wlo + i] : 0.0;
    }
    __syncthreads();
    for (;;) {
        unsigned c = 0;
        if (lane == 0) c = atomicAdd(counter, 1u);
        c = (unsigned)__builtin_amdgcn_readfirstlane((int)c);
        if (c >= (unsigned)ncells) break;
        const int2 cc = cells[c];
        int cand[2] = {cc.x, cc.y};
        int lo = min(P.cand_from[cc.x], P.cand_to[cc.x]), hi = max(P.cand_from[cc.x], P.cand_to[cc.x]);
        if (NL == 2) {
            lo = min(lo, min(P.cand_from[cc.y], P.cand_to[cc.y]));
            hi = max(hi, max(P.cand_from[cc.y], P.cand_to[cc.y]));
        }
        const int L = hi - lo;
        const int base = NL == 1 ? prm.fast_iter : prm.slow_iter;
        const int iterations = (L + NL > 100) ? base * 5 : base;
        CellResult r;
        se2_wave_solve<M, NL, STAGED>(P, lo, L, cand, iterations, sh, cst, wlo, wstride, r);
        if (lane == 0) {
            out.max_chi2[c] = r.max_chi2;
            out.chi2_total[c] = r.chi2_total;
            out.meta[c] = make_int4(r.iterations, r.tries, r.flags, r.evals);
        }
        wave_sync();
    }
}

#ifndef IPC_LDS_BUDGET
#define IPC_LDS_BUDGET (160 * 1024)
#endif
constexpr int kLdsBudget = IPC_LDS_BUDGET;

template <int M, int NL>
static hipError_t launch_one(int n, hipStream_t st, const Se2View& P, const int2* cells, SolveParams prm, CellOut out,
                             unsigned* counter, int n_cu)
{
    constexpr int kWavesPerGroup = se2_waves<M>();
    const int E = P.V - 1;
    const int wstride = E + 32;
    const size_t scratch = kWavesPerGroup * ((sizeof(WaveScratch<NL>) + 7) / 8) * sizeof(double);
    const size_t staged = scratch + sizeof(double) * (size_t)F_SG * wstride;
    const int groups = std::max(1, std::min(n_cu, (n + kWavesPerGroup - 1) / kWavesPerGroup));
    if (staged <= (size_t)kLdsBudget) {
        auto k = se2_wave_kernel<M, NL, true>;
        hipError_t e = hipFuncSetAttribute(reinterpret_cast<const void*>(k), hipFuncAttributeMaxDynamicSharedMemorySize, (int)staged);
        if (e != hipSuccess) return e;
        hipLaunchKernelGGL(k, dim3(groups), dim3(64 * kWavesPerGroup), staged, st, P, cells, n, counter, prm, out, 0, E, wstride);
    } else {
        auto k = se2_wave_kernel<M, NL, false>;
        hipLaunchKernelGGL(k, dim3(groups), dim3(64 * kWavesPerGroup), scratch, st, P, cells, n, counter, prm, out, 0, E, wstride);
    }
    return hipGetLastError();
}

namespace ipc {
hipError_t launch_se2_wave(int nl, int M, int n, hipStream_t st, const Se2View& P, const int2* cells, SolveParams prm,
                           CellOut out, unsigned* counter, int n_cu)
{
#define IPC_WCASE(MM)                                                                              \
    case MM:                                                                                       \
        return nl == 1 ? launch_one<MM, 1>(n, st, P, cells, prm, out, counter, n_cu)               \
                       : launch_one<MM, 2>(n, st, P, cells, prm, out, counter, n_cu);
    switch (M) {
#ifdef IPC_WAVE_ONLY_M
        IPC_WCASE(IPC_WAVE_ONLY_M)
#else
        IPC_WCASE(1)
        IPC_WCASE(3)
        IPC_WCASE(5)
        IPC_WCASE(7)
        IPC_WCASE(9)
        IPC_WCASE(11)
        IPC_WCASE(13)
#endif
        default: return hipErrorInvalidValue;
    }
#undef IPC_WCASE
}

}
```

### ipc_amd/csrc/se2_wave_cell.hpp

```cpp
#pragma once
#include "se2_cell.hpp"

namespace ipc {

template <int NL>
struct WaveScratch {
    LoopConst lc[NL];
    LoopState ls[2][NL];
    double lvec[NL][2][3];
    double red[4][32];
    double gam[4][NL * 9];
};

struct PairBox {
    double data[4][2][8];
    int flag[4];
};
__device__ __forceinline__ void mb_store(double* p, double v)
{
#ifdef IPC_MAILBOX_PLAIN
    *p = v;
#else
    __hip_atomic_store(p, v, __ATOMIC_RELAXED, __HIP_MEMORY_SCOPE_WORKGROUP);
#endif
}
__device__ __forceinline__ double mb_load(const double* p)
{
#ifdef IPC_MAILBOX_PLAIN
    return *p;
#else
    return __hip_atomic_load(p, __ATOMIC_RELAXED, __HIP_MEMORY_SCOPE_WORKGROUP);
#endif
}

#ifndef IPC_SPIN_SLEEP
#define IPC_SPIN_SLEEP 1
#endif
#if IPC_SPIN_SLEEP > 0
#define IPC_SPIN_WAIT() __builtin_amdgcn_s_sleep(IPC_SPIN_SLEEP)
#else
#define IPC_SPIN_WAIT() asm volatile("s_nop 0")
#endif

__device__ __forceinline__ void wave_sync()
{
    __builtin_amdgcn_fence(__ATOMIC_ACQ_REL, "wavefront");
    __builtin_amdgcn_wave_barrier();
}

template <int N>
__device__ __forceinline__ bool ldl_solve(double (&A)[N][N], double (&b)[N])
{
    bool ok = true;
    double inv[N];
#pragma unroll
    for (int j = 0; j < N; ++j) {
        double d = A[j][j];
#pragma unroll
        for (int k = 0; k < j; ++k) d -= A[j][k] * A[j][k] * A[k][k];
        ok = ok && (d > 0);
        double r = __builtin_amdgcn_rcp(d);
        r = fma(fma(-d, r, 1.0), r, r);
        r = fma(fma(-d, r, 1.0), r, r);
        inv[j] = r;
        A[j][j] = d;
#pragma unroll
        for (int i = j + 1; i < N; ++i) {
            double v = A[i][j];
#pragma unroll
            for (int k = 0; k < j; ++k) v -= A[i][k] * A[j][k] * A[k][k];
            A[i][j] = v * r;
        }
    }
#pragma unroll
    for (int i = 0; i < N; ++i) {
        double v = b[i];
#pragma unroll
        for (int k = 0; k < i; ++k) v -= A[i][k] * b[k];
        b[i] = v;
    }
#pragma unroll
    for (int i = 0; i < N; ++i) b[i] *= inv[i];
#pragma unroll
    for (int i = N - 1; i >= 0; --i) {
        double v = b[i];
#pragma unroll
        for (int k = i + 1; k < N; ++k) v -= A[k][i] * b[k];
        b[i] = v;
    }
    return ok;
}

template <int V> struct IntC { static constexpr int value = V; };

#define IPC_SLOT_FENCE() __builtin_amdgcn_sched_barrier(0)
#define IPC_PIN1(a) asm volatile("" : "+v"(a) : : "memory")
#define IPC_PIN2(a, b) asm volatile("" : "+v"(a), "+v"(b) : : "memory")
#define IPC_PIN3(a, b, c) asm volatile("" : "+v"(a), "+v"(b), "+v"(c) : : "memory")

#ifndef IPC_KEEPE_MAX
#define IPC_KEEPE_MAX 8
#endif
#ifndef IPC_PF_MAX
#define IPC_PF_MAX 9
#endif
template <int M, int NL, bool STAGED, int W = 1, bool KEEP_E = (M <= IPC_KEEPE_MAX)>
__device__ __forceinline__ void se2_wave_solve(const Se2View& P, int lo_abs, int L, const int (&cand)[2], int iterations,
                               WaveScratch<NL>& sh, const double* cst, int wlo, int wstride, CellResult& res,
                               PairBox* box = nullptr, int seq0 = 0, int* seq_out = nullptr)
{
    static_assert(W == 1 || W == 2 || W == 4, "one, two or four cooperating waves per cell");
    constexpr int NS = NL * 3;
    const double term_scale = P.term_eps / (double)(L + NL);
    bool lastGN = false;
    const int lane = threadIdx.x & 63;
    const int wsub = W > 1 ? (__builtin_amdgcn_readfirstlane((int)(threadIdx.x >> 6)) & (W - 1)) : 0;
    const int gl = wsub * 64 + lane;
    int j0 = gl * M + 1;

#ifdef IPC_PHASE_TIMING
    unsigned long long gnEvals = 0, gnRejected = 0, nBig = 0, tmBig = 0, tmSmall = 0;
    unsigned long long tmA = 0, tmB1 = 0, tmB2 = 0, tmC = 0, tmT = 0, tmW = 0, tmK = 0, tm0 = __builtin_amdgcn_s_memtime();
#define IPC_WTICK(acc) { const unsigned long long t_ = __builtin_amdgcn_s_memtime(); acc += t_ - tm0; tm0 = t_; }
#else
#define IPC_WTICK(acc)
#endif
    int seq = seq0;
    auto post_wait = [&](const double (&mine)[8], int n) {
        if constexpr (W > 1) {
            ++seq;
            double* my = box->data[wsub][seq & 1];
            if (lane == 0) {
#pragma unroll
                for (int k = 0; k < 8; ++k) if (k < n) mb_store(&my[k], mine[k]);
            }
            wave_sync();
            if (lane == 0) __hip_atomic_store(&box->flag[wsub], seq, __ATOMIC_RELEASE, __HIP_MEMORY_SCOPE_WORKGROUP);
#ifdef IPC_PHASE_TIMING
            const unsigned long long tw0 = __builtin_amdgcn_s_memtime();
#endif
#pragma unroll
            for (int o = 0; o < W; ++o) {
                if (o == wsub) continue;
                while (__hip_atomic_load(&box->flag[o], __ATOMIC_ACQUIRE, __HIP_MEMORY_SCOPE_WORKGROUP) - seq < 0)
                    IPC_SPIN_WAIT();
            }
#ifdef IPC_PHASE_TIMING
            tmW += __builtin_amdgcn_s_memtime() - tw0;
#endif
#ifdef IPC_MB_DELAY_WAVE
            if (wsub == IPC_MB_DELAY_WAVE) { __builtin_amdgcn_s_sleep(127); __builtin_amdgcn_s_sleep(127); }
#endif
            __builtin_amdgcn_fence(__ATOMIC_ACQUIRE, "workgroup", "local");
            wave_sync();
        }
    };
    auto peer = [&](int o, int k) -> double { return mb_load(&box->data[o][seq & 1][k]); };
    auto pair_barrier = [&]() {
        if constexpr (W > 1) { double a[8] = {0, 0, 0, 0, 0, 0, 0, 0}; post_wait(a, 0); }
    };
    auto cell_sum2 = [&](double v0, double v1, double& s0, double& s1) {
        const double t0 = wave_sum(v0), t1 = wave_sum(v1);
        if constexpr (W > 1) {
            double a[8] = {t0, t1, 0, 0, 0, 0, 0, 0};
            post_wait(a, 2);
#if defined(IPC_MAILBOX_PLAIN) && defined(IPC_DBG_SUM_SIDE)
            auto rdx = [&](int o, int k) -> double {
                return ((IPC_DBG_SUM_SIDE >> o) & 1) ? __hip_atomic_load(&box->data[o][seq & 1][k], __ATOMIC_RELAXED, __HIP_MEMORY_SCOPE_WORKGROUP) : peer(o, k);
            };
#else
            auto rdx = [&](int o, int k) -> double { return peer(o, k); };
#endif
            s0 = wsub == 0 ? t0 : rdx(0, 0);
            s1 = wsub == 0 ? t1 : rdx(0, 1);
#pragma unroll
            for (int o = 1; o < W; ++o) { s0 += o == wsub ? t0 : rdx(o, 0); s1 += o == wsub ? t1 : rdx(o, 1); }
        } else { s0 = t0; s1 = t1; }
    };
    auto cell_excl = [&](double run) -> double {
        const double inc = wave_inclusive_scan(run);
        double off = inc - run;
        if constexpr (W > 1) {
            double a[8] = {read_lane(inc, 63), 0, 0, 0, 0, 0, 0, 0};
            post_wait(a, 1);
            double lower = 0.0;
#pragma unroll
            for (int o = 0; o < W - 1; ++o) if (o < wsub) lower += peer(o, 0);
            off += lower;
        }
        return off;
    };
    auto cell_excl2 = [&](double r0, double r1, double& o0, double& o1) {
        const double i0 = wave_inclusive_scan(r0), i1 = wave_inclusive_scan(r1);
        o0 = i0 - r0; o1 = i1 - r1;
        if constexpr (W > 1) {
            double a[8] = {read_lane(i0, 63), read_lane(i1, 63), 0, 0, 0, 0, 0, 0};
            post_wait(a, 2);
            double l0 = 0.0, l1 = 0.0;
#pragma unroll
            for (int o = 0; o < W - 1; ++o) if (o < wsub) { l0 += peer(o, 0); l1 += peer(o, 1); }
            o0 += l0; o1 += l1;
        }
    };

    if (lane < NL && wsub == 0) {
        const int l = lane, c = cand[l];
        LoopConst& q = sh.lc[l];
        q.f = P.cand_from[c] - lo_abs;
        q.t = P.cand_to[c] - lo_abs;
        q.lo = min(q.f, q.t);
        q.hi = max(q.f, q.t);
        q.sigma = q.t > q.f ? 1.0 : -1.0;
        q.tzx = P.cand[(size_t)F_TZX * P.cstride + c];
        q.tzy = P.cand[(size_t)F_TZY * P.cstride + c];
        q.cz = P.cand[(size_t)F_CZ * P.cstride + c];
        q.sz = P.cand[(size_t)F_SZ * P.cstride + c];
        q.thz = P.cand[(size_t)F_THZ * P.cstride + c];
#pragma unroll
        for (int k = 0; k < 6; ++k) {
            q.om[k] = P.cand[(size_t)(F_OM + k) * P.cstride + c];
            q.sg[k] = P.cand[(size_t)(F_SG + k) * P.cstride + c];
        }
    }

    Pose2 X[M];
    double ex[KEEP_E ? M : 1], ey[KEEP_E ? M : 1], eth[KEEP_E ? M : 1];
    double bx[M], by[M], bth[M];
    double hx[M], hy[M], hth[M];
    Pose2 gauge;
    gauge.x = P.pose0[lo_abs];
    gauge.y = P.pose0[(size_t)P.VS + lo_abs];
    gauge.th = P.pose0[(size_t)2 * P.VS + lo_abs];
    sincos_pi(gauge.th, gauge.s, gauge.c);
#pragma unroll
    for (int s = 0; s < M; ++s) {
        const int j = j0 + s;
        const int ja = j <= L ? lo_abs + j : lo_abs;
        X[s].x = P.pose0[ja];
        X[s].y = P.pose0[(size_t)P.VS + ja];
        X[s].th = P.pose0[(size_t)2 * P.VS + ja];
        sincos_pi(X[s].th, X[s].s, X[s].c);
        if (KEEP_E) ex[s] = ey[s] = eth[s] = 0.0;
        bx[s] = by[s] = bth[s] = 0.0;
        hx[s] = hy[s] = hth[s] = 0.0;
    }
    wave_sync();
    pair_barrier();
    int lf[NL], lt[NL], of[NL], sf[NL], ot[NL], st_[NL], llo[NL], lhi[NL];
#pragma unroll
    for (int l = 0; l < NL; ++l) {
        lf[l] = __builtin_amdgcn_readfirstlane(sh.lc[l].f);
        lt[l] = __builtin_amdgcn_readfirstlane(sh.lc[l].t);
        llo[l] = min(lf[l], lt[l]); lhi[l] = max(lf[l], lt[l]);
        of[l] = lf[l] > 0 ? (lf[l] - 1) / M : -1; sf[l] = lf[l] > 0 ? (lf[l] - 1) % M : -1;
        ot[l] = lt[l] > 0 ? (lt[l] - 1) / M : -1; st_[l] = lt[l] > 0 ? (lt[l] - 1) % M : -1;
    }
    unsigned ownSlots = 0;
#pragma unroll
    for (int l = 0; l < NL; ++l) {
        if (of[l] >= 0 && (of[l] >> 6) == wsub) ownSlots |= 1u << sf[l];
        if (ot[l] >= 0 && (ot[l] >> 6) == wsub) ownSlots |= 1u << st_[l];
    }
    if (gl == 0) {
#pragma unroll
        for (int l = 0; l < NL; ++l)
#pragma unroll
            for (int bsel = 0; bsel < 2; ++bsel) {
                double* pf = sh.ls[bsel][l].pf;
                double* pt = sh.ls[bsel][l].pt;
                if (lf[l] == 0) { pf[0] = gauge.x; pf[1] = gauge.y; pf[2] = gauge.th; pf[3] = gauge.c; pf[4] = gauge.s; }
                if (lt[l] == 0) { pt[0] = gauge.x; pt[1] = gauge.y; pt[2] = gauge.th; pt[3] = gauge.c; pt[4] = gauge.s; }
            }
    }

    int eloc = gl * M < L ? gl * M : 0;
    typedef const __attribute__((address_space(3))) double* LdsRec;
    LdsRec crec = nullptr;
    auto opaque = [&]() {
        asm volatile("" : "+v"(eloc), "+v"(j0));
        if (STAGED) { crec = (LdsRec)(cst + (lo_abs - wlo + eloc) * (int)F_SG); asm volatile("" : "+v"(crec)); }
    };
    auto ldc = [&](int field, int s) -> double {
        if (STAGED && field < (int)F_SG) return crec[s * (int)F_SG + field];
        return P.chain_rec[((size_t)(lo_abs + eloc) + s) * (int)F_NFIELDS + field];
    };
    auto ldsym = [&](int field0, int s) -> Sym3 {
        Sym3 m;
        m.a00 = ldc(field0 + 0, s); m.a01 = ldc(field0 + 1, s); m.a02 = ldc(field0 + 2, s);
        m.a11 = ldc(field0 + 3, s); m.a12 = ldc(field0 + 4, s); m.a22 = ldc(field0 + 5, s);
        return m;
    };
    struct SlotConst { double tzx, tzy, thz, cz, sz; Sym3 om, sg; };
    auto ld_slot = [&](int s, SlotConst& c, auto want_c) {
        constexpr int WANT = decltype(want_c)::value;
        if (WANT & 1) { c.tzx = ldc(F_TZX, s); c.tzy = ldc(F_TZY, s); c.thz = ldc(F_THZ, s); }
        if (WANT & 2) { c.cz = ldc(F_CZ, s); c.sz = ldc(F_SZ, s); }
        if (WANT & 4) c.om = ldsym(F_OM, s);
        if (WANT & 8) c.sg = ldsym(F_SG, s);
    };
    constexpr int kErrWant = KEEP_E ? 0 : 3;
    constexpr bool PF = M <= IPC_PF_MAX;

    auto prev0 = [&](const Pose2& last) -> Pose2 {
        Pose2 cr = gauge;
        if constexpr (W > 1) {
            double a[8] = {read_lane(last.x, 63), read_lane(last.y, 63), read_lane(last.th, 63), read_lane(last.c, 63),
                           read_lane(last.s, 63), 0, 0, 0};
            post_wait(a, 5);
            if (wsub > 0) { cr.x = peer(wsub - 1, 0); cr.y = peer(wsub - 1, 1); cr.th = peer(wsub - 1, 2); cr.c = peer(wsub - 1, 3); cr.s = peer(wsub - 1, 4); }
        }
        Pose2 p;
        p.x = lane_prev(last.x, cr.x); p.y = lane_prev(last.y, cr.y); p.th = lane_prev(last.th, cr.th);
        p.c = lane_prev(last.c, cr.c); p.s = lane_prev(last.s, cr.s);
        return p;
    };
    auto prev3 = [&](double vx, double vy, double vth, double& ox, double& oy, double& oth) {
        double c0 = 0.0, c1 = 0.0, c2 = 0.0;
        if constexpr (W > 1) {
            double a[8] = {read_lane(vx, 63), read_lane(vy, 63), read_lane(vth, 63), 0, 0, 0, 0, 0};
            post_wait(a, 3);
            if (wsub > 0) { c0 = peer(wsub - 1, 0); c1 = peer(wsub - 1, 1); c2 = peer(wsub - 1, 2); }
        }
        ox = lane_prev(vx, c0); oy = lane_prev(vy, c1); oth = lane_prev(vth, c2);
    };
    auto next3 = [&](double vx, double vy, double vth, double& ox, double& oy, double& oth) {
        double c0 = 0.0, c1 = 0.0, c2 = 0.0;
        if constexpr (W > 1) {
            double a[8] = {read_lane(vx, 0), read_lane(vy, 0), read_lane(vth, 0), 0, 0, 0, 0, 0};
            post_wait(a, 3);
            if (wsub < W - 1) { c0 = peer(wsub + 1, 0); c1 = peer(wsub + 1, 1); c2 = peer(wsub + 1, 2); }
        }
        ox = lane_next(vx, c0); oy = lane_next(vy, c1); oth = lane_next(vth, c2);
    };

    auto loop_eval = [&](int l, int bsel) -> double {
        const LoopConst& q = sh.lc[l];
        LoopState& st = sh.ls[bsel][l];
        Pose2 a{st.pf[0], st.pf[1], st.pf[2], st.pf[3], st.pf[4]};
        Pose2 b{st.pt[0], st.pt[1], st.pt[2], st.pt[3], st.pt[4]};
        double e0, e1, e2;
        se2_error(a, b, q.tzx, q.tzy, q.cz, q.sz, q.thz, e0, e1, e2);
        Sym3 om{q.om[0], q.om[1], q.om[2], q.om[3], q.om[4], q.om[5]};
        double q0, q1, q2;
        om.mul(e0, e1, e2, q0, q1, q2);
        const double chi = e0 * q0 + e1 * q1 + e2 * q2;
        st.e[0] = e0; st.e[1] = e1; st.e[2] = e2;
        st.chi = chi;
        return chi;
    };
    int cur = 0;
    auto loop_force = [&](int l) {
        const LoopConst& q = sh.lc[l];
        LoopState& st = sh.ls[cur][l];
        Sym3 om{q.om[0], q.om[1], q.om[2], q.om[3], q.om[4], q.om[5]};
        double q0, q1, q2;
        om.mul(st.e[0], st.e[1], st.e[2], q0, q1, q2);
        const double cP = st.pf[3] * q.cz - st.pf[4] * q.sz, sP = st.pf[4] * q.cz + st.pf[3] * q.sz;
        st.g[0] = cP * q0 - sP * q1; st.g[1] = sP * q0 + cP * q1; st.g[2] = q2;
    };
    auto loop_quad = [&](int l) -> double {
        const LoopConst& q = sh.lc[l];
        const LoopState& st = sh.ls[cur][l];
        Pose2 a{st.pf[0], st.pf[1], st.pf[2], st.pf[3], st.pf[4]};
        Pose2 b{st.pt[0], st.pt[1], st.pt[2], st.pt[3], st.pt[4]};
        double wx, wy, wth;
        se2_apply_J(a, b, q.cz, q.sz, sh.lvec[l][0][0], sh.lvec[l][0][1], sh.lvec[l][0][2], sh.lvec[l][1][0],
                    sh.lvec[l][1][1], sh.lvec[l][1][2], wx, wy, wth);
        Sym3 om{q.om[0], q.om[1], q.om[2], q.om[3], q.om[4], q.om[5]};
        return om.quad(wx, wy, wth);
    };

    bool sweepChanged = false;
    auto launder = [&]() {
#pragma unroll
        for (int s = 0; s < M; ++s) {
            asm volatile("" : "+v"(X[s].x), "+v"(X[s].y), "+v"(X[s].c), "+v"(X[s].s));
            if (KEEP_E) asm volatile("" : "+v"(ex[s]), "+v"(ey[s]), "+v"(eth[s]));
        }
    };
    auto err_of = [&](int s, const Pose2& a, const SlotConst& K, double& e0, double& e1, double& e2) {
        if (KEEP_E) { e0 = ex[s]; e1 = ey[s]; e2 = eth[s]; return; }
        se2_error(a, X[s], K.tzx, K.tzy, K.cz, K.sz, K.thz, e0, e1, e2);
        if (!(j0 + s <= L)) { e0 = 0.0; e1 = 0.0; e2 = 0.0; }
    };
    auto sweep = [&](auto mode_c, bool big, double p, double q, int bsel, bool gn = false, bool wantChanged = true) -> double {
        constexpr int MODE = decltype(mode_c)::value;
        opaque();
        launder();
        asm volatile("" : "+v"(p), "+v"(q));
        auto stepped = [&](int s) -> Pose2 {
            Pose2 Y;
            double dx, dy, dth;
            if (gn) { dx = hx[s]; dy = hy[s]; dth = hth[s]; }
            else { dx = fma(p, bx[s], q * hx[s]); dy = fma(p, by[s], q * hy[s]); dth = fma(p, bth[s], q * hth[s]); }
            Y.x = X[s].x + dx;
            Y.y = X[s].y + dy;
            Y.th = wrap_pi(X[s].th + dth);
            if (big) sincos_pi(Y.th, Y.s, Y.c);
            else rotate_small(X[s].c, X[s].s, Y.th - X[s].th, Y.c, Y.s);
            return Y;
        };
        const Pose2 last = MODE == 0 ? X[M - 1] : stepped(M - 1);
        Pose2 prev = last;
        if (MODE != 2 || KEEP_E) prev = prev0(last);
        double part = 0.0;
        bool changed = false;
        constexpr int kWant = (MODE != 2 || KEEP_E) ? (MODE != 2 ? 7 : 3) : 0;
        SlotConst Kn;
        if (PF) ld_slot(0, Kn, IntC<kWant>{});
#pragma unroll
        for (int s = 0; s < M; ++s) {
            SlotConst K;
            if (PF) { K = Kn; if (s + 1 < M) ld_slot(s + 1, Kn, IntC<kWant>{}); }
            else ld_slot(s, K, IntC<kWant>{});
            const Pose2 Y = MODE == 0 ? X[s] : (s == M - 1 ? last : stepped(s));
            const bool v = j0 + s <= L;
            if (MODE == 1 && wantChanged) changed |= v && ((Y.x != X[s].x) || (Y.y != X[s].y) || (Y.th != X[s].th));
            double e0 = 0.0, e1 = 0.0, e2 = 0.0;
            if (MODE != 2 || KEEP_E) se2_error(prev, Y, K.tzx, K.tzy, K.cz, K.sz, K.thz, e0, e1, e2);
            if (MODE != 2) {
                const double c2 = K.om.quad(e0, e1, e2);
                part += v ? c2 : 0.0;
            }
            if (MODE != 1 && KEEP_E) { ex[s] = v ? e0 : 0.0; ey[s] = v ? e1 : 0.0; eth[s] = v ? e2 : 0.0; }
            if (MODE != 2 && ((ownSlots >> s) & 1u)) {
#pragma unroll
                for (int l = 0; l < NL; ++l) {
                    if (sf[l] == s && gl == of[l]) {
                        double* w = sh.ls[bsel][l].pf;
                        w[0] = Y.x; w[1] = Y.y; w[2] = Y.th; w[3] = Y.c; w[4] = Y.s;
                    }
                    if (st_[l] == s && gl == ot[l]) {
                        double* w = sh.ls[bsel][l].pt;
                        w[0] = Y.x; w[1] = Y.y; w[2] = Y.th; w[3] = Y.c; w[4] = Y.s;
                    }
                }
            }
            if (MODE == 2) X[s] = Y;
            prev = Y;
            if (MODE != 2) IPC_PIN1(part);
            if (MODE != 1 && KEEP_E) IPC_PIN3(ex[s], ey[s], eth[s]);
            if (MODE == 2) IPC_PIN3(X[s].x, X[s].y, X[s].th);
            IPC_PIN3(prev.x, prev.y, prev.th);
            IPC_PIN2(prev.c, prev.s);
            IPC_SLOT_FENCE();
        }
        if (MODE == 2) return 0.0;
        wave_sync();
        if constexpr (W > 1) {
            double tot, chg;
            cell_sum2(part, (MODE == 1 && changed) ? 1.0 : 0.0, tot, chg);
            const double lc = lane < NL ? loop_eval(lane, bsel) : 0.0;
#pragma unroll
            for (int l = 0; l < NL; ++l) tot += read_lane(lc, l);
            if (MODE == 1) sweepChanged = chg != 0.0;
            return tot;
        } else {
            if (lane < NL) part += loop_eval(lane, bsel);
            double tot, chg;
            cell_sum2(part, (MODE == 1 && changed) ? 1.0 : 0.0, tot, chg);
            if (MODE == 1) sweepChanged = chg != 0.0;
            return tot;
        }
    };

    int evals = 1;
    double currentChi = sweep(IntC<0>{}, false, 0.0, 0.0, cur);

    double delta = 1e4;
    const int maxTrials = 100;
    int it_done = 0, tries_total = 0, flags = 0;

    IPC_WTICK(tmT)
    for (int it = 0; it < iterations; ++it) {
        opaque();
        launder();
        if (gl < NL) loop_force(gl);
        wave_sync();
        const Pose2 a0 = prev0(X[M - 1]);
        constexpr int kWantA = 2 | 4 | kErrWant;
        auto force = [&](int s, const Pose2& a, const SlotConst& K, double& gx, double& gy, double& gth, double& mx,
                         double& my, double& mth) {
            const double cz = K.cz, sz = K.sz;
            const double cP = a.c * cz - a.s * sz, sP = a.s * cz + a.c * sz;
            double e0, e1, e2, qx, qy, qth;
            err_of(s, a, K, e0, e1, e2);
            K.om.mul(e0, e1, e2, qx, qy, qth);
            gx = cP * qx - sP * qy;
            gy = sP * qx + cP * qy;
            gth = qth;
            const double dx = X[s].x - a.x, dy = X[s].y - a.y;
            mx = gx; my = gy;
            mth = gth + (-dy * gx + dx * gy);
        };
        double bbp = 0.0;
        {
            double g0x, g0y, g0th, m0x, m0y, m0th;
            SlotConst Kn;
            {
                SlotConst K0;
                ld_slot(0, K0, IntC<kWantA>{});
                if (PF && M > 1) ld_slot(M - 1, Kn, IntC<kWantA>{});
                force(0, a0, K0, g0x, g0y, g0th, m0x, m0y, m0th);
            }
            double nx, ny, nth;
            next3(m0x, m0y, m0th, nx, ny, nth);
#pragma unroll
            for (int s = M - 1; s >= 0; --s) {
                double gx, gy, gth, mx, my, mth;
                if (s == 0) { gx = g0x; gy = g0y; gth = g0th; mx = m0x; my = m0y; mth = m0th; }
                else {
                    SlotConst K;
                    if (PF) { K = Kn; if (s - 1 > 0) ld_slot(s - 1, Kn, IntC<kWantA>{}); }
                    else ld_slot(s, K, IntC<kWantA>{});
                    force(s, X[s - 1], K, gx, gy, gth, mx, my, mth);
                }
                const bool v = j0 + s <= L;
                double tx = nx - gx, ty = ny - gy, tth = nth - gth;
                if ((ownSlots >> s) & 1u) {
#pragma unroll
                for (int l = 0; l < NL; ++l) {
                    const LoopState& st = sh.ls[cur][l];
                    if (st_[l] == s && gl == ot[l]) { tx -= st.g[0]; ty -= st.g[1]; tth -= st.g[2]; }
                    if (sf[l] == s && gl == of[l]) {
                        const double dx = st.pt[0] - st.pf[0], dy = st.pt[1] - st.pf[1];
                        tx += st.g[0]; ty += st.g[1];
                        tth += st.g[2] + (-dy * st.g[0] + dx * st.g[1]);
                    }
                }
                }
                bx[s] = v ? tx : 0.0; by[s] = v ? ty : 0.0; bth[s] = v ? tth : 0.0;
                bbp += bx[s] * bx[s] + by[s] * by[s] + bth[s] * bth[s];
                nx = mx; ny = my; nth = mth;
                IPC_PIN3(bx[s], by[s], bth[s]);
                IPC_PIN3(nx, ny, nth);
                IPC_PIN1(bbp);
                IPC_SLOT_FENCE();
            }
        }
        IPC_WTICK(tmA)
        double bb, bHb, alpha, hsdNorm;
        double nu[NL][3];
        opaque();
        launder();
        {
#pragma unroll
            for (int l = 0; l < NL; ++l) {
                if (gl == 0) {
                    if (lf[l] == 0) { sh.lvec[l][0][0] = 0.0; sh.lvec[l][0][1] = 0.0; sh.lvec[l][0][2] = 0.0; }
                    if (lt[l] == 0) { sh.lvec[l][1][0] = 0.0; sh.lvec[l][1][1] = 0.0; sh.lvec[l][1][2] = 0.0; }
                }
#pragma unroll
                for (int s = 0; s < M; ++s) {
                    if (!((ownSlots >> s) & 1u)) continue;
                    if (sf[l] == s && gl == of[l]) { sh.lvec[l][0][0] = bx[s]; sh.lvec[l][0][1] = by[s]; sh.lvec[l][0][2] = bth[s]; }
                    if (st_[l] == s && gl == ot[l]) { sh.lvec[l][1][0] = bx[s]; sh.lvec[l][1][1] = by[s]; sh.lvec[l][1][2] = bth[s]; }
                }
            }
            double v1[16], v2[16];
#pragma unroll
            for (int k = 0; k < 16; ++k) { v1[k] = 0.0; v2[k] = 0.0; }
            v1[0] = bbp;
            double qbx, qby, qbth;
            prev3(bx[M - 1], by[M - 1], bth[M - 1], qbx, qby, qbth);
            constexpr int kWantB = 2 | 4 | 8 | kErrWant;
            SlotConst Kn;
            if (PF) ld_slot(0, Kn, IntC<kWantB>{});
#pragma unroll
            for (int s = 0; s < M; ++s) {
                SlotConst K;
                if (PF) { K = Kn; if (s + 1 < M) ld_slot(s + 1, Kn, IntC<kWantB>{}); }
                else ld_slot(s, K, IntC<kWantB>{});
                const Pose2& a = s == 0 ? a0 : X[s - 1];
                const bool v = j0 + s <= L;
                const double cz = K.cz, sz = K.sz;
                double wx, wy, wth;
                se2_apply_J(a, X[s], cz, sz, qbx, qby, qbth, bx[s], by[s], bth[s], wx, wy, wth);
                const double hq = K.om.quad(wx, wy, wth);
                v1[1] += v ? hq : 0.0;
                const Sym3 sg = K.sg;
                const double c = a.c * cz - a.s * sz, sn = a.s * cz + a.c * sz;
                const double kx = -(X[s].y - gauge.y), ky = X[s].x - gauge.x;
                const double cc = c * c, ss = sn * sn, cs = c * sn;
                const double C00 = cc * sg.a00 - 2 * cs * sg.a01 + ss * sg.a11;
                const double C01 = cs * (sg.a00 - sg.a11) + (cc - ss) * sg.a01;
                const double C11 = ss * sg.a00 + 2 * cs * sg.a01 + cc * sg.a11;
                const double c0 = c * sg.a02 - sn * sg.a12, c1 = sn * sg.a02 + c * sg.a12;
                const double sth = sg.a22;
                double psi[6];
                psi[2] = c0 - sth * kx;
                psi[4] = c1 - sth * ky;
                psi[0] = C00 - kx * c0 - kx * psi[2];
                psi[1] = C01 - kx * c1 - ky * psi[2];
                psi[3] = C11 - ky * c1 - ky * psi[4];
                psi[5] = sth;
                double e0, e1, e2;
                err_of(s, a, K, e0, e1, e2);
                const double w0 = c * e0 - sn * e1 - kx * e2;
                const double w1 = sn * e0 + c * e1 - ky * e2;
                const double w2 = e2;
                const int j = j0 + s;
                const double m1 = (v && j > llo[0] && j <= lhi[0]) ? 1.0 : 0.0;
                v1[2] += m1 * w0; v1[3] += m1 * w1; v1[4] += m1 * w2;
#pragma unroll
                for (int k = 0; k < 6; ++k) v1[5 + k] += m1 * psi[k];
                if constexpr (NL == 2) {
                    const double m2 = (v && j > llo[1] && j <= lhi[1]) ? 1.0 : 0.0;
                    const double m12 = m1 * m2;
                    v2[0] += m2 * w0; v2[1] += m2 * w1; v2[2] += m2 * w2;
#pragma unroll
                    for (int k = 0; k < 6; ++k) { v2[3 + k] += m2 * psi[k]; v2[9 + k] += m12 * psi[k]; }
                }
                qbx = bx[s]; qby = by[s]; qbth = bth[s];
                asm volatile("" : "+v"(v1[0]), "+v"(v1[1]), "+v"(v1[2]), "+v"(v1[3]), "+v"(v1[4]), "+v"(v1[5]),
                             "+v"(v1[6]), "+v"(v1[7]), "+v"(v1[8]), "+v"(v1[9]), "+v"(v1[10]) : : "memory");
                if constexpr (NL == 2)
                    asm volatile("" : "+v"(v2[0]), "+v"(v2[1]), "+v"(v2[2]), "+v"(v2[3]), "+v"(v2[4]), "+v"(v2[5]),
                                 "+v"(v2[6]), "+v"(v2[7]), "+v"(v2[8]), "+v"(v2[9]), "+v"(v2[10]), "+v"(v2[11]),
                                 "+v"(v2[12]), "+v"(v2[13]), "+v"(v2[14]) : : "memory");
                IPC_SLOT_FENCE();
            }
            wave_sum16_store(v1, &sh.red[wsub][0]);
            if constexpr (NL == 2) wave_sum16_store(v2, &sh.red[wsub][16]);
            wave_sync();
            pair_barrier();
            IPC_WTICK(tmB1)
            auto wtv = [&](int k) -> double {
                double t = sh.red[0][k];
#pragma unroll
                for (int o = 1; o < W; ++o) t += sh.red[o][k];
                return t;
            };
            double* gamw = sh.gam[wsub];
            if (lane < NL * 9) {
                const int l = lane / 9, i = (lane % 9) / 3, a = lane % 3;
                const LoopConst& q = sh.lc[l];
                const LoopState& st = sh.ls[cur][l];
                const double Aq = st.pf[3] * q.cz - st.pf[4] * q.sz, Bq = st.pf[4] * q.cz + st.pf[3] * q.sz;
                const double Kx = -(st.pt[1] - gauge.y), Ky = st.pt[0] - gauge.x;
                double g;
                if (i == 0) g = a == 0 ? Aq : (a == 1 ? Bq : Aq * Kx + Bq * Ky);
                else if (i == 1) g = a == 0 ? -Bq : (a == 1 ? Aq : -Bq * Kx + Aq * Ky);
                else g = a == 2 ? 1.0 : 0.0;
                gamw[lane] = q.sigma * g;
            }
            wave_sync();
            constexpr int RS = NS + 1;
            double val = 0.0;
            const int r = lane / RS, c = lane % RS;
            if (lane < NS * RS) {
                const int l1 = r / 3, i = r % 3;
                const double g10 = gamw[l1 * 9 + i * 3], g11 = gamw[l1 * 9 + i * 3 + 1], g12 = gamw[l1 * 9 + i * 3 + 2];
                if (c < NS) {
                    const int l2 = c / 3, k = c % 3;
                    const int mb = l1 == l2 ? (l1 == 0 ? 5 : 19) : 25;
                    const double m00 = wtv(mb), m01 = wtv(mb + 1), m02 = wtv(mb + 2), m11 = wtv(mb + 3), m12 = wtv(mb + 4), m22 = wtv(mb + 5);
                    const double t0 = g10 * m00 + g11 * m01 + g12 * m02;
                    const double t1 = g10 * m01 + g11 * m11 + g12 * m12;
                    const double t2 = g10 * m02 + g11 * m12 + g12 * m22;
                    val = t0 * gamw[l2 * 9 + k * 3] + t1 * gamw[l2 * 9 + k * 3 + 1] + t2 * gamw[l2 * 9 + k * 3 + 2];
                    if (l1 == l2) {
                        const int lo_ = i < k ? i : k, hi_ = i < k ? k : i;
                        val += sh.lc[l1].sg[lo_ * 3 - lo_ * (lo_ - 1) / 2 + (hi_ - lo_)];
                    }
                } else {
                    const int wb = l1 == 0 ? 2 : 16;
                    val = sh.ls[cur][l1].e[i] - (g10 * wtv(wb) + g11 * wtv(wb + 1) + g12 * wtv(wb + 2));
                }
            }
            bool okS = true;
#pragma unroll
            for (int k = 0; k < NS; ++k) {
                const double piv = read_lane(val, k * RS + k);
                okS = okS && (piv > 0);
                double inv = __builtin_amdgcn_rcp(piv);
                inv = fma(fma(-piv, inv, 1.0), inv, inv);
                inv = fma(fma(-piv, inv, 1.0), inv, inv);
                const double rowk = __shfl(val, k * RS + c, 64);
                const double colk = __shfl(val, r * RS + k, 64);
                val = (r == k) ? rowk * inv : fma(-(colk * rowk), inv, val);
            }
            {
                const int l = (lane < NS) ? lane / 3 : 0, cc = lane % 3;
                double nv = 0.0;
#pragma unroll
                for (int rr = 0; rr < 3; ++rr) {
                    const double mu_r = __shfl(val, (3 * l + rr) * RS + NS, 64);
                    nv += gamw[l * 9 + rr * 3 + cc] * mu_r;
                }
#pragma unroll
                for (int l2 = 0; l2 < NL; ++l2)
#pragma unroll
                    for (int k = 0; k < 3; ++k) nu[l2][k] = read_lane(nv, 3 * l2 + k);
            }
            bb = wtv(0);
            bHb = wtv(1);
            {
                const double lq = lane < NL ? loop_quad(lane) : 0.0;
#pragma unroll
                for (int l = 0; l < NL; ++l) bHb += read_lane(lq, l);
            }
            if (!okS) { flags |= 2; break; }
            alpha = bb / bHb;
            hsdNorm = sqrt(alpha * alpha * bb);
        }
        IPC_WTICK(tmB2)
        double hgnNorm, bh, hHh;
        opaque();
        launder();
        {
            double run = 0.0;
            constexpr int kWantC = 2 | 8 | kErrWant;
            SlotConst Kn;
            if (PF) ld_slot(0, Kn, IntC<kWantC>{});
#pragma unroll
            for (int s = 0; s < M; ++s) {
                SlotConst K;
                if (PF) { K = Kn; if (s + 1 < M) ld_slot(s + 1, Kn, IntC<kWantC>{}); }
                else ld_slot(s, K, IntC<kWantC>{});
                const Pose2& a = s == 0 ? a0 : X[s - 1];
                const int j = j0 + s;
                const bool v = j <= L;
                const double m1 = (v && j > llo[0] && j <= lhi[0]) ? 1.0 : 0.0;
                double n0 = m1 * nu[0][0], n1 = m1 * nu[0][1], n2 = m1 * nu[0][2];
                if constexpr (NL == 2) {
                    const double m2 = (v && j > llo[1] && j <= lhi[1]) ? 1.0 : 0.0;
                    n0 += m2 * nu[1][0]; n1 += m2 * nu[1][1]; n2 += m2 * nu[1][2];
                }
                const double cz = K.cz, sz = K.sz;
                const double c = a.c * cz - a.s * sz, sn = a.s * cz + a.c * sz;
                const double kx = -(X[s].y - gauge.y), ky = X[s].x - gauge.x;
                const double wx = c * n0 + sn * n1, wy = -sn * n0 + c * n1, wth = -(kx * n0 + ky * n1) + n2;
                double vx, vy, vth;
                K.sg.mul(wx, wy, wth, vx, vy, vth);
                double e0, e1, e2;
                err_of(s, a, K, e0, e1, e2);
                const double ux = -vx - e0, uy = -vy - e1, uth = -vth - e2;
                hx[s] = v ? c * ux - sn * uy : 0.0;
                hy[s] = v ? sn * ux + c * uy : 0.0;
                run += v ? uth : 0.0;
                hth[s] = run;
                IPC_PIN3(hx[s], hy[s], hth[s]);
                IPC_SLOT_FENCE();
            }
            const double offT = cell_excl(run);
            double rx = 0.0, ry = 0.0, thPrev = offT;
#pragma unroll
            for (int s = 0; s < M; ++s) {
                const Pose2& a = s == 0 ? a0 : X[s - 1];
                const bool v = j0 + s <= L;
                hth[s] += offT;
                const double dx = X[s].x - a.x, dy = X[s].y - a.y;
                rx += v ? hx[s] - dy * thPrev : 0.0;
                ry += v ? hy[s] + dx * thPrev : 0.0;
                hx[s] = rx; hy[s] = ry;
                thPrev = hth[s];
                IPC_PIN3(hx[s], hy[s], hth[s]);
                IPC_SLOT_FENCE();
            }
            double offX, offY;
            cell_excl2(rx, ry, offX, offY);
            double p0 = 0.0, p1 = 0.0;
#pragma unroll
            for (int s = 0; s < M; ++s) {
                const bool v = j0 + s <= L;
                hx[s] = v ? hx[s] + offX : 0.0;
                hy[s] = v ? hy[s] + offY : 0.0;
                hth[s] = v ? hth[s] : 0.0;
                p0 += hx[s] * hx[s] + hy[s] * hy[s] + hth[s] * hth[s];
                p1 += bx[s] * hx[s] + by[s] * hy[s] + bth[s] * hth[s];
            }
            double hh;
            cell_sum2(p0, p1, hh, bh);
            hgnNorm = sqrt(hh);
            hHh = bh;
        }
        IPC_WTICK(tmC)
        if (lastGN && hgnNorm < delta && fabs(bh) < term_scale * currentChi) { it_done = it + 1; tries_total += maxTrials; flags |= 1; break; }
        const double deltaAtEntry = delta;
        bool goodStep = false, dlReady = false;
        double dlC = 0.0, dlBma = 0.0;
        int numTries = 0;
        do {
            ++numTries;
            int stepType;
            double beta = 0.0, sdScale = 0.0;
            if (hgnNorm < delta) stepType = 0;
            else if (hsdNorm > delta) { stepType = 1; sdScale = delta / hsdNorm; }
            else {
                stepType = 2;
                if (!dlReady) {
                    double p0 = 0.0, p1 = 0.0;
#pragma unroll
                    for (int s = 0; s < M; ++s) {
                        const double sx = alpha * bx[s], sy = alpha * by[s], sth = alpha * bth[s];
                        const double ax = hx[s] - sx, ay = hy[s] - sy, ath = hth[s] - sth;
                        p0 += sx * ax + sy * ay + sth * ath;
                        p1 += ax * ax + ay * ay + ath * ath;
                    }
                    cell_sum2(p0, p1, dlC, dlBma);
                    dlReady = true;
                }
                const double c = dlC, bma = dlBma;
                const double hsdSq = alpha * alpha * bb;
                if (c <= 0.) beta = (-c + sqrt(c * c + bma * (delta * delta - hsdSq))) / bma;
                else beta = (delta * delta - hsdSq) / (c + sqrt(c * c + bma * (delta * delta - hsdSq)));
            }
            double pcoef, qcoef, hdlNorm;
            if (stepType == 0) { pcoef = 0.0; qcoef = 1.0; hdlNorm = hgnNorm; }
            else if (stepType == 1) { pcoef = sdScale * alpha; qcoef = 0.0; hdlNorm = delta; }
            else { pcoef = alpha - beta * alpha; qcoef = beta; hdlNorm = delta; }
            const double hdlHhdl = pcoef * pcoef * bHb + 2 * pcoef * qcoef * bb + qcoef * qcoef * hHh;
            const double bhdl = pcoef * bb + qcoef * bh;
            double linearGain = -1 * hdlHhdl + 2 * bhdl;
            bool big = false;
            double pc2 = pcoef, qc2 = qcoef;
            asm volatile("" : "+v"(pc2), "+v"(qc2));
#pragma unroll
            for (int s = 0; s < M; ++s) {
                const double thn = wrap_pi(X[s].th + (stepType == 0 ? hth[s] : fma(pc2, bth[s], qc2 * hth[s])));
                big |= fabs(thn - X[s].th) >= 0.015625;
            }
            const bool anyBig = __ballot(big) != 0ull;
            const int trial = cur ^ 1;
#ifdef IPC_PHASE_TIMING
            const unsigned long long tb0 = __builtin_amdgcn_s_memtime();
#endif
            const double newChi = sweep(IntC<1>{}, anyBig, pcoef, qcoef, trial, stepType == 0, stepType == 1);
#ifdef IPC_PHASE_TIMING
            if (anyBig) { ++nBig; tmBig += __builtin_amdgcn_s_memtime() - tb0; } else { tmSmall += __builtin_amdgcn_s_memtime() - tb0; }
#endif
            const bool anyChanged = stepType == 1 ? sweepChanged : true;
            ++evals;
            const double nonLinearGain = currentChi - newChi;
#ifdef IPC_PHASE_TIMING
            if (stepType == 0) { ++gnEvals; if (!(linearGain > 0 ? nonLinearGain > 0 : nonLinearGain < 0)) ++gnRejected; }
#endif
            if (fabs(linearGain) < 1e-12) linearGain = 1e-12;
            const bool linPos = linearGain > 0;
            auto rho_gt = [&](double t) { return linPos ? nonLinearGain > t * linearGain : nonLinearGain < t * linearGain; };
            auto rho_lt = [&](double t) { return linPos ? nonLinearGain < t * linearGain : nonLinearGain > t * linearGain; };
            if (rho_gt(0.0)) {
                goodStep = true;
                currentChi = newChi;
                cur = trial;
                IPC_WTICK(tmT)
                sweep(IntC<2>{}, anyBig, pcoef, qcoef, trial, stepType == 0, false);
                IPC_WTICK(tmK)
            }
            if (rho_gt(0.75)) delta = fmax(delta, 3 * hdlNorm);
            else if (rho_lt(0.25)) delta *= 0.5;
            if (!goodStep) {
                if (nonLinearGain != nonLinearGain) {
                    numTries = maxTrials;
                } else if (stepType == 0) {
                    while (numTries < maxTrials && hgnNorm < delta) { ++numTries; delta *= 0.5; }
                } else if (stepType == 1 && !anyChanged) {
                    numTries = maxTrials;
                }
            }
        } while (!goodStep && numTries < maxTrials);
        lastGN = goodStep && numTries == 1 && hgnNorm < deltaAtEntry;
        it_done = it + 1;
        tries_total += numTries;
        IPC_WTICK(tmT)
        if (numTries == maxTrials || !goodStep) { flags |= 1; break; }
    }
#ifdef IPC_PHASE_TIMING
    if (lane == 0 && wsub == 0 && P.dbg) {
        unsigned long long* d = reinterpret_cast<unsigned long long*>(P.dbg) + 64 + 16 * (M + 16 * (W - 1));
        atomicAdd(d + 0, tmA); atomicAdd(d + 1, tmB1); atomicAdd(d + 2, tmB2); atomicAdd(d + 3, tmC);
        atomicAdd(d + 4, tmT); atomicAdd(d + 5, tmW);
        atomicAdd(d + 6, (unsigned long long)it_done); atomicAdd(d + 7, (unsigned long long)evals);
        atomicAdd(d + 8, (unsigned long long)it_done * (unsigned long long)L);
        atomicAdd(d + 9, 1ull); atomicAdd(d + 10, tmK); atomicAdd(d + 11, (unsigned long long)(evals - 1 - it_done)); atomicAdd(d + 12, gnEvals); atomicAdd(d + 13, gnRejected); atomicAdd(d + 14, nBig); atomicAdd(d + 15, tmBig); atomicAdd(d + 1024, tmSmall);
    }
#endif

    double mx = 0.0;
    bool nan = false;
    opaque();
    {
        const Pose2 a0 = prev0(X[M - 1]);
#pragma unroll
        for (int s = 0; s < M; ++s) {
            SlotConst K;
            ld_slot(s, K, IntC<(4 | kErrWant)>{});
            double e0, e1, e2;
            err_of(s, s == 0 ? a0 : X[s - 1], K, e0, e1, e2);
            if (j0 + s > L) continue;
            const double c = K.om.quad(e0, e1, e2);
            if (c != c) nan = true;
            else mx = fmax(mx, c);
        }
    }
    mx = wave_max(mx);
    nan = __ballot(nan) != 0ull;
    if constexpr (W > 1) {
        double a[8] = {mx, nan ? 1.0 : 0.0, 0, 0, 0, 0, 0, 0};
        post_wait(a, 2);
#pragma unroll
        for (int o = 0; o < W; ++o) {
            if (o == wsub) continue;
            mx = fmax(mx, peer(o, 0));
            nan = nan || peer(o, 1) != 0.0;
        }
    }
    wave_sync();
#pragma unroll
    for (int l = 0; l < NL; ++l) {
        const double c = sh.ls[cur][l].chi;
        if (c != c) nan = true;
        else mx = fmax(mx, c);
    }
    if (nan && !(mx > 0.0)) mx = __longlong_as_double(0x7ff8000000000000ll);
    res.max_chi2 = mx;
    res.chi2_total = currentChi;
    res.iterations = it_done;
    res.tries = tries_total;
    res.flags = flags;
    res.evals = evals;
    if (seq_out) *seq_out = seq;
}

}
```

Measured before the change: 1.901 million candidate-pairs/s.

## Park per-slot SE2 residuals in LDS instead of recomputing them

```diff
diff --git a/include/ipc_amd.h b/include/ipc_amd.h
--- a/include/ipc_amd.h
+++ b/include/ipc_amd.h
@@ -72,8 +72,12 @@
     int nan_cells;
     int damped_cells;
     int literal_cells;
+    int park_launches;
+    int park_cells;
 } ipc_solve_report_t;
 int ipc_solve_report(ipc_engine_t* h, ipc_solve_report_t* out);
+
+int ipc_se2_lds_plan(int W, int M, int nl, int V, int allow_park, long long* out4);
 
 int ipc_assemble_matrix(ipc_engine_t* h, const uint64_t* d_gathered, int world,
                         uint64_t* d_bits, void* stream);
diff --git a/ipc_amd/capi.py b/ipc_amd/capi.py
--- a/ipc_amd/capi.py
+++ b/ipc_amd/capi.py
@@ -21,6 +21,7 @@
     "ipc_debug_dense_solve", "ipc_debug_band_solve", "ipc_debug_band_plan", "ipc_debug_absorbed_edges", "ipc_append_candidate", "ipc_incremental_set_state", "ipc_incremental_counters", "ipc_row_assignment", "ipc_run_sharded", "ipc_run_set_only",
     "ipc_append_odometry", "ipc_reserve_vertices", "ipc_vertex_count",
     "ipc_run_online", "ipc_online_covered", "ipc_online_reset", "ipc_reserve_candidates",
+    "ipc_se2_lds_plan",
 ]
 
 
@@ -49,7 +50,8 @@
 
 class SolveReport(C.Structure):
     _fields_ = [("cells", C.c_int), ("long_cells", C.c_int), ("failed_cells", C.c_int), ("capped_cells", C.c_int),
-                ("nan_cells", C.c_int), ("damped_cells", C.c_int), ("literal_cells", C.c_int)]
+                ("nan_cells", C.c_int), ("damped_cells", C.c_int), ("literal_cells", C.c_int),
+                ("park_launches", C.c_int), ("park_cells", C.c_int)]
 
 
 class OnlineReport(C.Structure):
@@ -106,6 +108,8 @@
     lib.ipc_cell_count.argtypes = [vp, C.POINTER(ip)]
     lib.ipc_cell_info.argtypes = [vp, vp, ip]
     lib.ipc_solve_report.argtypes = [vp, C.POINTER(SolveReport)]
+    if hasattr(lib, "ipc_se2_lds_plan"):
+        lib.ipc_se2_lds_plan.argtypes = [ip, ip, ip, ip, ip, C.POINTER(C.c_longlong)]
     lib.ipc_solver_time_ms.argtypes = [vp, C.POINTER(dp), C.POINTER(ip)]
     lib.ipc_synchronize.argtypes = [vp]
     lib.ipc_incremental_reset.argtypes = [vp]
diff --git a/ipc_amd/csrc/cell_kernels.hpp b/ipc_amd/csrc/cell_kernels.hpp
--- a/ipc_amd/csrc/cell_kernels.hpp
+++ b/ipc_amd/csrc/cell_kernels.hpp
@@ -50,18 +50,18 @@
 constexpr int kWaveVariantBase = 100;
 
 hipError_t launch_se2_wave(int nl, int M, int n, hipStream_t st, const Se2View& P, const int2* cells,
-                           SolveParams prm, CellOut out, unsigned* counter, int n_cu);
+                           SolveParams prm, CellOut out, unsigned* counter, int n_cu, int* park = nullptr);
 
 static const int kPairM[] = {5, 7, 9, 11};
 constexpr int kNumPairM = sizeof(kPairM) / sizeof(kPairM[0]);
 constexpr int kPairVariantBase = 200;
 hipError_t launch_se2_pair(int nl, int M, int n, hipStream_t st, const Se2View& P, const int2* cells,
-                           SolveParams prm, CellOut out, unsigned* counter, int n_cu);
+                           SolveParams prm, CellOut out, unsigned* counter, int n_cu, int* park = nullptr);
 
 static const int kQuadM[] = {7, 9, 11, 13};
 constexpr int kNumQuadM = sizeof(kQuadM) / sizeof(kQuadM[0]);
 constexpr int kQuadVariantBase = 300;
 hipError_t launch_se2_quad(int nl, int M, int n, hipStream_t st, const Se2View& P, const int2* cells,
-                           SolveParams prm, CellOut out, unsigned* counter, int n_cu);
+                           SolveParams prm, CellOut out, unsigned* counter, int n_cu, int* park = nullptr);
 
 }
diff --git a/ipc_amd/csrc/engine.hip b/ipc_amd/csrc/engine.hip
--- a/ipc_amd/csrc/engine.hip
+++ b/ipc_amd/csrc/engine.hip
@@ -660,6 +660,8 @@
     bool lm_retry = true;
     double borderline_band = -1.0;
     int last_literal_cells = 0;
+    bool se2_err_park = true;
+    int last_park_launches = 0, last_park_cells = 0;
     long lm_fallbacks = 0;
     long persist_timeouts = 0;
     long persist_relaunches = 0;
@@ -866,6 +868,7 @@
     }
     if (const char* mh = getenv("IPC_PERSIST_HELPERS")) { if (*mh) h->max_helpers = atoi(mh); }
     if (const char* lm = getenv("IPC_LM_RETRY")) { if (*lm) h->lm_retry = atoi(lm) != 0; }
+    if (const char* ep = getenv("IPC_SE2_ERR_PARK")) { if (*ep) h->se2_err_park = atoi(ep) != 0; }
     h->knobs = PersistKnobs::from_env();
     if (const char* e = getenv("IPC_LITERAL_BAND_MIN_N")) { if (*e) h->literal_band_min_n = atoi(e); }
     if (const char* bb = getenv("IPC_BORDERLINE_BAND")) {
@@ -1621,15 +1624,21 @@
     auto launch_slot = [&](int b, int nl, int n, const int2* cells, const CellOut& out, hipStream_t ls, unsigned* ctr) -> hipError_t {
         int var = h->plan.variant[b];
         if (h->plan.latency_variant[b] >= 0 && n < h->plan.latency_below[b] * h->n_cu) var = h->plan.latency_variant[b];
-        if (h->dim == 2)
-            return var >= kQuadVariantBase   ? launch_se2_quad(nl, var - kQuadVariantBase, n, ls, P, cells, sp, out, ctr, h->n_cu)
-                   : var >= kPairVariantBase ? launch_se2_pair(nl, var - kPairVariantBase, n, ls, P, cells, sp, out, ctr, h->n_cu)
-                   : var >= kWaveVariantBase ? launch_se2_wave(nl, var - kWaveVariantBase, n, ls, P, cells, sp, out, ctr, h->n_cu)
-                                             : launch_se2_block(nl, var, n, ls, P, cells, sp, out);
+        if (h->dim == 2) {
+            int park = h->se2_err_park ? 1 : 0;
+            hipError_t e;
+            if (var >= kQuadVariantBase) e = launch_se2_quad(nl, var - kQuadVariantBase, n, ls, P, cells, sp, out, ctr, h->n_cu, &park);
+            else if (var >= kPairVariantBase) e = launch_se2_pair(nl, var - kPairVariantBase, n, ls, P, cells, sp, out, ctr, h->n_cu, &park);
+            else if (var >= kWaveVariantBase) e = launch_se2_wave(nl, var - kWaveVariantBase, n, ls, P, cells, sp, out, ctr, h->n_cu, &park);
+            else { park = 0; e = launch_se2_block(nl, var, n, ls, P, cells, sp, out); }
+            if (park) { ++h->last_park_launches; h->last_park_cells += n; }
+            return e;
+        }
         if (var >= kLdsVariantBase3) return launch_se3_lds(nl, var - kLdsVariantBase3, n, ls, P3, cells, sp, out, ctr, h->n_cu);
         return launch_se3_block(nl, var, n, ls, P3, cells, sp, out);
     };
     int launches = 0;
+    h->last_park_launches = h->last_park_cells = 0;
     HIPCHK(hipMemsetAsync(h->d_wave_ctr, 0, sizeof(unsigned) * NS, st));
     HIPCHK(hipEventRecord(h->ev0, st));
     const int n_side = h->side_forced || total < 300000 ? h->n_side : std::min(h->n_side, h->dim == 2 ? 2 : 3);
@@ -2013,6 +2022,8 @@
     out->nan_cells = (int)host[2];
     out->damped_cells = h->last_lm_cells;
     out->literal_cells = h->last_literal_cells;
+    out->park_launches = h->last_park_launches;
+    out->park_cells = h->last_park_cells;
     return IPC_OK;
 }
 
diff --git a/ipc_amd/csrc/se2_group_kernel.hpp b/ipc_amd/csrc/se2_group_kernel.hpp
--- a/ipc_amd/csrc/se2_group_kernel.hpp
+++ b/ipc_amd/csrc/se2_group_kernel.hpp
@@ -5,12 +5,8 @@
 namespace ipc {
 
 constexpr int kWavesPerGroup = 4;
-#ifndef IPC_LDS_BUDGET
-#define IPC_LDS_BUDGET (160 * 1024)
-#endif
-constexpr int kLdsBudget = IPC_LDS_BUDGET;
 
-template <int W, int M, int NL, bool STAGED>
+template <int W, int M, int NL, bool STAGED, int PARK = 0>
 __global__ __launch_bounds__(64 * kWavesPerGroup, 1) void se2_group_kernel(Se2View P, const int2* cells, int ncells,
                                                                            unsigned* counter, SolveParams prm,
                                                                            CellOut out, int wlo, int wlen, int wstride)
@@ -23,6 +19,7 @@
     WaveScratch<NL>& sh = *reinterpret_cast<WaveScratch<NL>*>(dyn_lds + pair * kScratchDoubles);
     PairBox* box = reinterpret_cast<PairBox*>(dyn_lds + kPairs * kScratchDoubles + pair * kBoxDoubles);
     double* cst = dyn_lds + kPairs * (kScratchDoubles + kBoxDoubles);
+    double* park = cst + (STAGED ? (int)F_SG * wstride : 0) + wave * se2_park_wave_doubles(PARK);
     if (STAGED) {
         for (int f = 0; f < (int)F_SG; ++f)
             for (int i = threadIdx.x; i < wstride; i += 64 * kWavesPerGroup)
@@ -61,7 +58,7 @@
         const int base = NL == 1 ? prm.fast_iter : prm.slow_iter;
         const int iterations = (L + NL > 100) ? base * 5 : base;
         CellResult r;
-        se2_wave_solve<M, NL, STAGED, W>(P, lo, L, cand, iterations, sh, cst, wlo, wstride, r, box, seq, &seq);
+        se2_wave_solve<M, NL, STAGED, W, PARK>(P, lo, L, cand, iterations, sh, cst, wlo, wstride, r, box, seq, &seq, park);
         if (wsub == 0 && lane == 0) {
             out.max_chi2[c] = r.max_chi2;
             out.chi2_total[c] = r.chi2_total;
@@ -73,24 +70,25 @@
 
 template <int W, int M, int NL>
 static hipError_t launch_group(int n, hipStream_t st, const Se2View& P, const int2* cells, SolveParams prm, CellOut out,
-                              unsigned* counter, int n_cu)
+                              unsigned* counter, int n_cu, int* park)
 {
     const int E = P.V - 1;
     const int wstride = E + 32;
     constexpr int kPairs = kWavesPerGroup / W;
-    const size_t scratch = kPairs * (((sizeof(WaveScratch<NL>) + 7) / 8) + ((sizeof(PairBox) + 7) / 8)) * sizeof(double);
-    const size_t staged = scratch + sizeof(double) * (size_t)F_SG * wstride;
+    constexpr int PS = se2_park_slots<W, M, true>(), PU = se2_park_slots<W, M, false>();
+    const Se2LdsPlan pl = se2_lds_plan(se2_scratch_bytes<W, NL>(kWavesPerGroup), P.V, kWavesPerGroup, PS, PU, park && *park);
+    if (park) *park = pl.park > 0;
     const int groups = std::max(1, std::min(n_cu, (n + kPairs - 1) / kPairs));
-    if (staged <= (size_t)kLdsBudget) {
-        auto k = se2_group_kernel<W, M, NL, true>;
-        hipError_t e = hipFuncSetAttribute(reinterpret_cast<const void*>(k), hipFuncAttributeMaxDynamicSharedMemorySize, (int)staged);
-        if (e != hipSuccess) return e;
-        hipLaunchKernelGGL(k, dim3(groups), dim3(64 * kWavesPerGroup), staged, st, P, cells, n, counter, prm, out, 0, E, wstride);
-    } else {
-        auto k = se2_group_kernel<W, M, NL, false>;
-        hipLaunchKernelGGL(k, dim3(groups), dim3(64 * kWavesPerGroup), scratch, st, P, cells, n, counter, prm, out, 0, E, wstride);
-    }
-    return hipGetLastError();
+    auto go = [&](auto k) -> hipError_t {
+        if (pl.bytes > 48 * 1024) {
+            hipError_t e = hipFuncSetAttribute(reinterpret_cast<const void*>(k), hipFuncAttributeMaxDynamicSharedMemorySize, (int)pl.bytes);
+            if (e != hipSuccess) return e;
+        }
+        hipLaunchKernelGGL(k, dim3(groups), dim3(64 * kWavesPerGroup), pl.bytes, st, P, cells, n, counter, prm, out, 0, E, wstride);
+        return hipGetLastError();
+    };
+    if (pl.staged) return pl.park ? go(se2_group_kernel<W, M, NL, true, PS>) : go(se2_group_kernel<W, M, NL, true, 0>);
+    return pl.park ? go(se2_group_kernel<W, M, NL, false, PU>) : go(se2_group_kernel<W, M, NL, false, 0>);
 }
 
 }
diff --git a/ipc_amd/csrc/se2_pair.hip b/ipc_amd/csrc/se2_pair.hip
--- a/ipc_amd/csrc/se2_pair.hip
+++ b/ipc_amd/csrc/se2_pair.hip
@@ -2,12 +2,12 @@
 
 namespace ipc {
 hipError_t launch_se2_pair(int nl, int M, int n, hipStream_t st, const Se2View& P, const int2* cells, SolveParams prm,
-                           CellOut out, unsigned* counter, int n_cu)
+                           CellOut out, unsigned* counter, int n_cu, int* park)
 {
 #define IPC_PCASE(MM)                                                                              \
     case MM:                                                                                       \
-        return nl == 1 ? launch_group<2, MM, 1>(n, st, P, cells, prm, out, counter, n_cu)          \
-                       : launch_group<2, MM, 2>(n, st, P, cells, prm, out, counter, n_cu);
+        return nl == 1 ? launch_group<2, MM, 1>(n, st, P, cells, prm, out, counter, n_cu, park)    \
+                       : launch_group<2, MM, 2>(n, st, P, cells, prm, out, counter, n_cu, park);
     switch (M) {
 #ifdef IPC_PAIR_ONLY_M
         IPC_PCASE(IPC_PAIR_ONLY_M)
diff --git a/ipc_amd/csrc/se2_quad.hip b/ipc_amd/csrc/se2_quad.hip
--- a/ipc_amd/csrc/se2_quad.hip
+++ b/ipc_amd/csrc/se2_quad.hip
@@ -2,12 +2,12 @@
 
 namespace ipc {
 hipError_t launch_se2_quad(int nl, int M, int n, hipStream_t st, const Se2View& P, const int2* cells, SolveParams prm,
-                           CellOut out, unsigned* counter, int n_cu)
+                           CellOut out, unsigned* counter, int n_cu, int* park)
 {
 #define IPC_PCASE(MM)                                                                              \
     case MM:                                                                                       \
-        return nl == 1 ? launch_group<4, MM, 1>(n, st, P, cells, prm, out, counter, n_cu)          \
-                       : launch_group<4, MM, 2>(n, st, P, cells, prm, out, counter, n_cu);
+        return nl == 1 ? launch_group<4, MM, 1>(n, st, P, cells, prm, out, counter, n_cu, park)    \
+                       : launch_group<4, MM, 2>(n, st, P, cells, prm, out, counter, n_cu, park);
     switch (M) {
         IPC_PCASE(7)
         IPC_PCASE(9)
diff --git a/ipc_amd/csrc/se2_wave.hip b/ipc_amd/csrc/se2_wave.hip
--- a/ipc_amd/csrc/se2_wave.hip
+++ b/ipc_amd/csrc/se2_wave.hip
@@ -9,7 +9,7 @@
 template <int M>
 constexpr int se2_waves() { return M <= IPC_SE2_DENSE_MAXM ? 8 : 4; }
 
-template <int M, int NL, bool STAGED>
+template <int M, int NL, bool STAGED, int PARK = 0>
 __global__ __launch_bounds__((64 * se2_waves<M>()), 1) void se2_wave_kernel(Se2View P, const int2* cells, int ncells,
                                                                           unsigned* counter, SolveParams prm,
                                                                           CellOut out, int wlo, int wlen, int wstride)
@@ -20,6 +20,7 @@
     const int wave = threadIdx.x >> 6, lane = threadIdx.x & 63;
     WaveScratch<NL>& sh = *reinterpret_cast<WaveScratch<NL>*>(dyn_lds + wave * kScratchDoubles);
     double* cst = dyn_lds + kWavesPerGroup * kScratchDoubles;
+    double* park = cst + (STAGED ? (int)F_SG * wstride : 0) + wave * se2_park_wave_doubles(PARK);
     if (STAGED) {
         for (int f = 0; f < (int)F_SG; ++f)
             for (int i = threadIdx.x; i < wstride; i += 64 * kWavesPerGroup)
@@ -42,7 +43,7 @@
         const int base = NL == 1 ? prm.fast_iter : prm.slow_iter;
         const int iterations = (L + NL > 100) ? base * 5 : base;
         CellResult r;
-        se2_wave_solve<M, NL, STAGED>(P, lo, L, cand, iterations, sh, cst, wlo, wstride, r);
+        se2_wave_solve<M, NL, STAGED, 1, PARK>(P, lo, L, cand, iterations, sh, cst, wlo, wstride, r, nullptr, 0, nullptr, park);
         if (lane == 0) {
             out.max_chi2[c] = r.max_chi2;
             out.chi2_total[c] = r.chi2_total;
@@ -52,41 +53,37 @@
     }
 }
 
-#ifndef IPC_LDS_BUDGET
-#define IPC_LDS_BUDGET (160 * 1024)
-#endif
-constexpr int kLdsBudget = IPC_LDS_BUDGET;
-
 template <int M, int NL>
 static hipError_t launch_one(int n, hipStream_t st, const Se2View& P, const int2* cells, SolveParams prm, CellOut out,
-                             unsigned* counter, int n_cu)
+                             unsigned* counter, int n_cu, int* park)
 {
     constexpr int kWavesPerGroup = se2_waves<M>();
+    constexpr int PS = se2_park_slots<1, M, true>(), PU = se2_park_slots<1, M, false>();
     const int E = P.V - 1;
     const int wstride = E + 32;
-    const size_t scratch = kWavesPerGroup * ((sizeof(WaveScratch<NL>) + 7) / 8) * sizeof(double);
-    const size_t staged = scratch + sizeof(double) * (size_t)F_SG * wstride;
+    const Se2LdsPlan pl = se2_lds_plan(se2_scratch_bytes<1, NL>(kWavesPerGroup), P.V, kWavesPerGroup, PS, PU, park && *park);
+    if (park) *park = pl.park > 0;
     const int groups = std::max(1, std::min(n_cu, (n + kWavesPerGroup - 1) / kWavesPerGroup));
-    if (staged <= (size_t)kLdsBudget) {
-        auto k = se2_wave_kernel<M, NL, true>;
-        hipError_t e = hipFuncSetAttribute(reinterpret_cast<const void*>(k), hipFuncAttributeMaxDynamicSharedMemorySize, (int)staged);
-        if (e != hipSuccess) return e;
-        hipLaunchKernelGGL(k, dim3(groups), dim3(64 * kWavesPerGroup), staged, st, P, cells, n, counter, prm, out, 0, E, wstride);
-    } else {
-        auto k = se2_wave_kernel<M, NL, false>;
-        hipLaunchKernelGGL(k, dim3(groups), dim3(64 * kWavesPerGroup), scratch, st, P, cells, n, counter, prm, out, 0, E, wstride);
-    }
-    return hipGetLastError();
+    auto go = [&](auto k) -> hipError_t {
+        if (pl.bytes > 48 * 1024) {
+            hipError_t e = hipFuncSetAttribute(reinterpret_cast<const void*>(k), hipFuncAttributeMaxDynamicSharedMemorySize, (int)pl.bytes);
+            if (e != hipSuccess) return e;
+        }
+        hipLaunchKernelGGL(k, dim3(groups), dim3(64 * kWavesPerGroup), pl.bytes, st, P, cells, n, counter, prm, out, 0, E, wstride);
+        return hipGetLastError();
+    };
+    if (pl.staged) return pl.park ? go(se2_wave_kernel<M, NL, true, PS>) : go(se2_wave_kernel<M, NL, true, 0>);
+    return pl.park ? go(se2_wave_kernel<M, NL, false, PU>) : go(se2_wave_kernel<M, NL, false, 0>);
 }
 
 namespace ipc {
 hipError_t launch_se2_wave(int nl, int M, int n, hipStream_t st, const Se2View& P, const int2* cells, SolveParams prm,
-                           CellOut out, unsigned* counter, int n_cu)
+                           CellOut out, unsigned* counter, int n_cu, int* park)
 {
 #define IPC_WCASE(MM)                                                                              \
     case MM:                                                                                       \
-        return nl == 1 ? launch_one<MM, 1>(n, st, P, cells, prm, out, counter, n_cu)               \
-                       : launch_one<MM, 2>(n, st, P, cells, prm, out, counter, n_cu);
+        return nl == 1 ? launch_one<MM, 1>(n, st, P, cells, prm, out, counter, n_cu, park)         \
+                       : launch_one<MM, 2>(n, st, P, cells, prm, out, counter, n_cu, park);
     switch (M) {
 #ifdef IPC_WAVE_ONLY_M
         IPC_WCASE(IPC_WAVE_ONLY_M)
@@ -104,4 +101,23 @@
 #undef IPC_WCASE
 }
 
+extern "C" int ipc_se2_lds_plan(int W, int M, int nl, int V, int allow_park, long long* out4)
+{
+    Se2LdsPlan pl;
+    bool found = false;
+#define IPC_PLAN(WW, MM)                                                                                              \
+    if (W == WW && M == MM && (nl == 1 || nl == 2)) {                                                                  \
+        const int waves = WW == 1 ? se2_waves<MM>() : 4;                                                              \
+        const size_t scratch = nl == 1 ? se2_scratch_bytes<WW, 1>(waves) : se2_scratch_bytes<WW, 2>(waves);           \
+        pl = se2_lds_plan(scratch, V, waves, se2_park_slots<WW, MM, true>(), se2_park_slots<WW, MM, false>(), allow_park != 0); \
+        found = true;                                                                                                 \
+    }
+    IPC_PLAN(1, 1) IPC_PLAN(1, 3) IPC_PLAN(1, 5) IPC_PLAN(1, 7) IPC_PLAN(1, 9) IPC_PLAN(1, 11) IPC_PLAN(1, 13)
+    IPC_PLAN(2, 5) IPC_PLAN(2, 7) IPC_PLAN(2, 9) IPC_PLAN(2, 11)
+#undef IPC_PLAN
+    if (!found || !out4 || V < 2) return -1;
+    out4[0] = pl.staged; out4[1] = pl.park; out4[2] = (long long)pl.bytes; out4[3] = IPC_LDS_BUDGET;
+    return 0;
 }
+
+}
diff --git a/ipc_amd/csrc/se2_wave_cell.hpp b/ipc_amd/csrc/se2_wave_cell.hpp
--- a/ipc_amd/csrc/se2_wave_cell.hpp
+++ b/ipc_amd/csrc/se2_wave_cell.hpp
@@ -104,12 +104,61 @@
 #ifndef IPC_PF_MAX
 #define IPC_PF_MAX 9
 #endif
-template <int M, int NL, bool STAGED, int W = 1, bool KEEP_E = (M <= IPC_KEEPE_MAX)>
+#ifndef IPC_LDS_BUDGET
+#define IPC_LDS_BUDGET (160 * 1024)
+#endif
+
+constexpr int se2_park_stride(int park) { return park * 3 + ((park * 3) & 1 ? 0 : 1); }
+constexpr int se2_park_wave_doubles(int park) { return park > 0 ? 64 * se2_park_stride(park) : 0; }
+#ifndef IPC_PARK_WAVE
+#define IPC_PARK_WAVE 6
+#endif
+#ifndef IPC_PARK_PAIR
+#define IPC_PARK_PAIR 7
+#endif
+#ifndef IPC_PARK_W9
+#define IPC_PARK_W9 0
+#endif
+#ifndef IPC_PARK_W9U
+#define IPC_PARK_W9U 6
+#endif
+template <int W, int M, bool STAGED>
+constexpr int se2_park_slots()
+{
+    if (M <= IPC_KEEPE_MAX || W > 2) return 0;
+    if (W == 1 && M == 9) return STAGED ? IPC_PARK_W9 : IPC_PARK_W9U;
+    if (!STAGED) return M;
+    const int p = W == 1 ? IPC_PARK_WAVE : IPC_PARK_PAIR;
+    return p < M ? p : M;
+}
+struct Se2LdsPlan { bool staged; int park; size_t bytes; };
+inline Se2LdsPlan se2_lds_plan(size_t scratch, int V, int waves, int park_staged, int park_unstaged, bool allow_park)
+{
+    const size_t budget = (size_t)IPC_LDS_BUDGET;
+    const size_t window = sizeof(double) * (size_t)F_SG * (size_t)(V - 1 + 32);
+    Se2LdsPlan pl;
+    pl.staged = scratch + window <= budget;
+    pl.bytes = scratch + (pl.staged ? window : 0);
+    pl.park = 0;
+    const int park = pl.staged ? park_staged : park_unstaged;
+    const size_t pbytes = sizeof(double) * (size_t)waves * se2_park_wave_doubles(park);
+    if (allow_park && park > 0 && pl.bytes + pbytes <= budget) { pl.park = park; pl.bytes += pbytes; }
+    return pl;
+}
+template <int W, int NL>
+constexpr size_t se2_scratch_bytes(int waves)
+{
+    return W == 1 ? waves * ((sizeof(WaveScratch<NL>) + 7) / 8) * sizeof(double)
+                  : (waves / W) * (((sizeof(WaveScratch<NL>) + 7) / 8) + ((sizeof(PairBox) + 7) / 8)) * sizeof(double);
+}
+
+template <int M, int NL, bool STAGED, int W = 1, int PARK = 0, bool KEEP_E = (M <= IPC_KEEPE_MAX)>
 __device__ __forceinline__ void se2_wave_solve(const Se2View& P, int lo_abs, int L, const int (&cand)[2], int iterations,
                                WaveScratch<NL>& sh, const double* cst, int wlo, int wstride, CellResult& res,
-                               PairBox* box = nullptr, int seq0 = 0, int* seq_out = nullptr)
+                               PairBox* box = nullptr, int seq0 = 0, int* seq_out = nullptr, double* park = nullptr)
 {
     static_assert(W == 1 || W == 2 || W == 4, "one, two or four cooperating waves per cell");
+    static_assert(PARK >= 0 && PARK <= M && (PARK == 0 || !KEEP_E), "the park replaces recomputed errors only");
     constexpr int NS = NL * 3;
     const double term_scale = P.term_eps / (double)(L + NL);
     bool lastGN = false;
@@ -276,9 +325,12 @@
     int eloc = gl * M < L ? gl * M : 0;
     typedef const __attribute__((address_space(3))) double* LdsRec;
     LdsRec crec = nullptr;
+    typedef __attribute__((address_space(3))) double* LdsPark;
+    LdsPark pk = nullptr;
     auto opaque = [&]() {
         asm volatile("" : "+v"(eloc), "+v"(j0));
         if (STAGED) { crec = (LdsRec)(cst + (lo_abs - wlo + eloc) * (int)F_SG); asm volatile("" : "+v"(crec)); }
+        if (PARK > 0) { pk = (LdsPark)(park + lane * se2_park_stride(PARK)); asm volatile("" : "+v"(pk)); }
     };
     auto ldc = [&](int field, int s) -> double {
         if (STAGED && field < (int)F_SG) return crec[s * (int)F_SG + field];
@@ -293,12 +345,14 @@
     struct SlotConst { double tzx, tzy, thz, cz, sz; Sym3 om, sg; };
     auto ld_slot = [&](int s, SlotConst& c, auto want_c) {
         constexpr int WANT = decltype(want_c)::value;
-        if (WANT & 1) { c.tzx = ldc(F_TZX, s); c.tzy = ldc(F_TZY, s); c.thz = ldc(F_THZ, s); }
+        if ((WANT & 16) && s < PARK) { c.tzx = pk[s * 3 + 0]; c.tzy = pk[s * 3 + 1]; c.thz = pk[s * 3 + 2]; }
+        else if (WANT & 1) { c.tzx = ldc(F_TZX, s); c.tzy = ldc(F_TZY, s); c.thz = ldc(F_THZ, s); }
         if (WANT & 2) { c.cz = ldc(F_CZ, s); c.sz = ldc(F_SZ, s); }
         if (WANT & 4) c.om = ldsym(F_OM, s);
         if (WANT & 8) c.sg = ldsym(F_SG, s);
     };
     constexpr int kErrWant = KEEP_E ? 0 : 3;
+    constexpr int kErrWantP = KEEP_E ? 0 : (PARK > 0 ? 16 | 3 : 3);
     constexpr bool PF = M <= IPC_PF_MAX;
 
     auto prev0 = [&](const Pose2& last) -> Pose2 {
@@ -378,10 +432,13 @@
             if (KEEP_E) asm volatile("" : "+v"(ex[s]), "+v"(ey[s]), "+v"(eth[s]));
         }
     };
-    auto err_of = [&](int s, const Pose2& a, const SlotConst& K, double& e0, double& e1, double& e2) {
+    auto err_of = [&](int s, const Pose2& a, const SlotConst& K, double& e0, double& e1, double& e2, auto how_c) {
+        constexpr int HOW = decltype(how_c)::value;
         if (KEEP_E) { e0 = ex[s]; e1 = ey[s]; e2 = eth[s]; return; }
+        if (HOW == 2 && s < PARK) { e0 = K.tzx; e1 = K.tzy; e2 = K.thz; return; }
         se2_error(a, X[s], K.tzx, K.tzy, K.cz, K.sz, K.thz, e0, e1, e2);
         if (!(j0 + s <= L)) { e0 = 0.0; e1 = 0.0; e2 = 0.0; }
+        if (HOW == 1 && s < PARK) { pk[s * 3 + 0] = e0; pk[s * 3 + 1] = e1; pk[s * 3 + 2] = e2; }
     };
     auto sweep = [&](auto mode_c, bool big, double p, double q, int bsel, bool gn = false, bool wantChanged = true) -> double {
         constexpr int MODE = decltype(mode_c)::value;
@@ -484,7 +541,7 @@
             const double cz = K.cz, sz = K.sz;
             const double cP = a.c * cz - a.s * sz, sP = a.s * cz + a.c * sz;
             double e0, e1, e2, qx, qy, qth;
-            err_of(s, a, K, e0, e1, e2);
+            err_of(s, a, K, e0, e1, e2, IntC<1>{});
             K.om.mul(e0, e1, e2, qx, qy, qth);
             gx = cP * qx - sP * qy;
             gy = sP * qx + cP * qy;
@@ -563,7 +620,7 @@
             v1[0] = bbp;
             double qbx, qby, qbth;
             prev3(bx[M - 1], by[M - 1], bth[M - 1], qbx, qby, qbth);
-            constexpr int kWantB = 2 | 4 | 8 | kErrWant;
+            constexpr int kWantB = 2 | 4 | 8 | kErrWantP;
             SlotConst Kn;
             if (PF) ld_slot(0, Kn, IntC<kWantB>{});
 #pragma unroll
@@ -595,7 +652,7 @@
                 psi[3] = C11 - ky * c1 - ky * psi[4];
                 psi[5] = sth;
                 double e0, e1, e2;
-                err_of(s, a, K, e0, e1, e2);
+                err_of(s, a, K, e0, e1, e2, IntC<2>{});
                 const double w0 = c * e0 - sn * e1 - kx * e2;
                 const double w1 = sn * e0 + c * e1 - ky * e2;
                 const double w2 = e2;
@@ -710,7 +767,7 @@
         launder();
         {
             double run = 0.0;
-            constexpr int kWantC = 2 | 8 | kErrWant;
+            constexpr int kWantC = 2 | 8 | kErrWantP;
             SlotConst Kn;
             if (PF) ld_slot(0, Kn, IntC<kWantC>{});
 #pragma unroll
@@ -734,7 +791,7 @@
                 double vx, vy, vth;
                 K.sg.mul(wx, wy, wth, vx, vy, vth);
                 double e0, e1, e2;
-                err_of(s, a, K, e0, e1, e2);
+                err_of(s, a, K, e0, e1, e2, IntC<2>{});
                 const double ux = -vx - e0, uy = -vy - e1, uth = -vth - e2;
                 hx[s] = v ? c * ux - sn * uy : 0.0;
                 hy[s] = v ? sn * ux + c * uy : 0.0;
@@ -887,7 +944,7 @@
             SlotConst K;
             ld_slot(s, K, IntC<(4 | kErrWant)>{});
             double e0, e1, e2;
-            err_of(s, s == 0 ? a0 : X[s - 1], K, e0, e1, e2);
+            err_of(s, s == 0 ? a0 : X[s - 1], K, e0, e1, e2, IntC<0>{});
             if (j0 + s > L) continue;
             const double c = K.om.quad(e0, e1, e2);
             if (c != c) nan = true;
```

Result: faster. 1.928 million candidate-pairs/s (median of 6 runs) (+1.4%).
